# Hi-PACE/hipace

Measured on AMD Instinct MI355X. Metric: transverse slices/s at 1024^2 x 4ppc (explicit solver), higher is better.
Workload: dtype f64

## Files before the change

hipace_amd/_lib.py:

```python
import ctypes as C
import os
import subprocess


def hip_already_started():
    import sys
    if _LIB is not None:
        return True
    t = sys.modules.get("torch")
    try:
        return bool(t is not None and t.cuda.is_initialized())
    except Exception:
        return False


_LIB = None
_HWQ_PRESET = "GPU_MAX_HW_QUEUES" in os.environ
_HIP_STARTED_AT_IMPORT = hip_already_started()
_HERE = os.path.dirname(os.path.abspath(__file__))
CSRC = os.path.join(_HERE, "csrc")
SO = os.environ.get("HPS_LIB") or os.path.join(CSRC, "libhpslice.so")


class Slab(C.Structure):
# ... 54 lines not shown
                ("lo", C.c_double * 3), ("hi", C.c_double * 3),
                ("order", C.c_int), ("deriv_type", C.c_int),
                ("plasma_ppc", C.c_int * 2), ("plasma_density", C.c_double), ("plasma_radius", C.c_double),
                ("plasma_charge", C.c_double), ("plasma_mass", C.c_double), ("max_qsa", C.c_double),
                ("n_subcycles", C.c_int),
                ("beam_profile", C.c_int), ("beam_zmin", C.c_double), ("beam_zmax", C.c_double),
                ("beam_radius", C.c_double), ("beam_density", C.c_double),
                ("beam_umean", C.c_double * 3), ("beam_pos_mean", C.c_double * 3),
                ("beam_pos_std", C.c_double * 3), ("beam_ppc", C.c_int * 3), ("beam_charge", C.c_double),
                ("bc", C.c_int), ("mg_tol_rel", C.c_double), ("mg_tol_abs", C.c_double),
                ("deposit_rho", C.c_int), ("n_steps", C.c_int),
                ("dt", C.c_double), ("beam_n_subcycles", C.c_int), ("beam_mass", C.c_double), ("ext_E_slope", C.c_double * 2),
                ("bxby_solver", C.c_int), ("predcorr_tol", C.c_double), ("predcorr_max_iter", C.c_int),
                ("predcorr_mix", C.c_double), ("field_bc", C.c_int),
                ("laser_on", C.c_int), ("laser_a0", C.c_double), ("laser_w0", C.c_double), ("laser_L0", C.c_double),
                ("laser_lambda0", C.c_double), ("laser_pos", C.c_double * 3),
                ("laser_zfoc", C.c_double), ("laser_solver", C.c_int), ("laser_use_phase", C.c_int), ("si_units", C.c_int),
                ("grid_current_on", C.c_int), ("grid_current_peak", C.c_double), ("grid_current_mean", C.c_double * 3),
                ("grid_current_std", C.c_double * 3), ("laser_mg_tol_rel", C.c_double), ("laser_mg_tol_abs", C.c_double),
                ("beam_radiation_reaction", C.c_int), ("background_density_SI", C.c_double), ("beam_no_z_push", C.c_int),
                ("plasma_no_neutralize", C.c_int), ("ion_on", C.c_int), ("ion_ppc", C.c_int * 2), ("ion_density", C.c_double),
                ("ion_mass", C.c_double), ("ion_charge", C.c_double), ("ion_init_level", C.c_int), ("ion_Z", C.c_int),
                ("ion_energies", C.c_double * 56), ("ion_seed", C.c_ulonglong),
                ("beam_spin_tracking", C.c_int), ("beam_initial_spin", C.c_double * 3), ("beam_spin_anom", C.c_double),
                ("dt_adaptive", C.c_int), ("nt_per_betatron", C.c_double), ("dt_max", C.c_double),
                ("adaptive_threshold_uz", C.c_double), ("adaptive_phase_tolerance", C.c_double),
                ("adaptive_no_predict_step", C.c_int), ("adaptive_no_phase_control", C.c_int), ("adaptive_phase_substeps", C.c_int),
                ("adaptive_density", C.c_double), ("max_time", C.c_double), ("beam_uz_std", C.c_double),
                ("ext_Ez_slope", C.c_double),
                ("beam_do_salame", C.c_int), ("salame_n_iter", C.c_int), ("salame_relative_tolerance", C.c_double),
                ("salame_no_advance", C.c_int), ("salame_Ez_target_slope", C.c_double)]


COMPS = ["N_jx_beam", "N_jy_beam", "chi", "Sy", "Sx", "ExmBy", "EypBx", "Ez", "Bx", "By", "Bz",
         "Psi", "jx_beam", "jy_beam", "jz_beam", "jx", "jy", "rhomjz", "P_jx_beam", "P_jy_beam",
         "Ion_rhomjz", "rho"]
CIDX = {n: i for i, n in enumerate(COMPS)}
COMPS_PC = ["N_jx", "N_jy", "ExmBy", "EypBx", "Ez", "Bx", "By", "Bz", "Psi", "jx", "jy", "jz", "rhomjz",
            "P_Bx", "P_By", "P_jx", "P_jy", "Ion_rhomjz", "It_Bx", "It_By", "PIt_Bx", "PIt_By", "rho"]
CIDX_PC = {n: i for i, n in enumerate(COMPS_PC)}
COMPS_SALAME = ["Ez_target", "Ez_no_salame", "Ez", "jx", "jy", "jz_beam", "Bx", "By", "Sy", "Sx", "Sy_back", "Sx_back"]
ID_VALID = 1 << 63

_SIGS = {
    "hps_last_error": (C.c_char_p, []),
    "hps_version": (C.c_char_p, []),
    "hps_deposit_current": (C.c_int, [Slab, Plasma, Geom, C.c_void_p, C.c_double, C.c_double, C.c_int, C.c_double,
                                      C.c_int, C.c_void_p, C.c_void_p]),
    "hps_explicit_deposit": (C.c_int, [Slab, Plasma, Geom, C.c_void_p, C.c_void_p, C.c_double, C.c_double, C.c_int,
                                       C.c_int, C.c_int, C.c_void_p]),
    "hps_advance_plasma": (C.c_int, [Slab, Plasma, Geom, C.c_void_p, C.c_double, C.c_double, C.c_int, C.c_int,
                                     C.c_int, C.c_int, C.c_void_p]),
    "hps_tiling_create": (C.c_int, [C.c_int, C.c_int, C.c_int, C.c_long, C.POINTER(C.c_void_p)]),
    "hps_reorder_particles": (C.c_int, [C.c_void_p, Plasma, Plasma, Geom, C.c_void_p]),
    "hps_tiling_info": (C.c_int, [C.c_void_p, C.POINTER(C.c_int), C.POINTER(C.c_void_p), C.POINTER(C.c_void_p)]),
    "hps_tiling_destroy": (C.c_int, [C.c_void_p]),
    "hps_deposit_current_tiled": (C.c_int, [Slab, Plasma, Geom, C.c_void_p, C.c_double, C.c_double, C.c_int, C.c_double,
                                            C.c_int, C.c_void_p, C.c_void_p, C.c_void_p, C.c_void_p]),
    "hps_explicit_deposit_tiled": (C.c_int, [Slab, Plasma, Geom, C.c_void_p, C.c_void_p, C.c_double, C.c_double, C.c_int,
                                             C.c_int, C.c_int, C.c_void_p, C.c_void_p, C.c_void_p]),
    "hps_advance_plasma_tiled": (C.c_int, [Slab, Plasma, Geom, C.c_void_p, C.c_double, C.c_double, C.c_int, C.c_int,
                                           C.c_int, C.c_int, C.c_void_p, C.c_void_p, C.c_void_p]),
    "hps_deposit_current_tiled_laser": (C.c_int, [Slab, Plasma, Geom, C.c_void_p, C.c_int, C.c_double, C.c_double, C.c_int,
                                                  C.c_double, C.c_int, C.c_void_p, C.c_void_p, C.c_void_p, C.c_void_p]),
    "hps_explicit_deposit_tiled_laser": (C.c_int, [Slab, Plasma, Geom, C.c_void_p, C.c_int, C.c_void_p, C.c_double, C.c_double,
                                                   C.c_int, C.c_int, C.c_int, C.c_void_p, C.c_void_p, C.c_void_p]),
    "hps_advance_plasma_tiled_laser": (C.c_int, [Slab, Plasma, Geom, C.c_void_p, C.c_int, C.c_double, C.c_double, C.c_int,
                                                 C.c_int, C.c_int, C.c_int, C.c_void_p, C.c_void_p, C.c_void_p]),
    "hps_tiling_set_validity": (C.c_int, [C.c_void_p, C.c_int, C.c_int]),
    "hps_particles_record": (C.c_int, [C.c_int]),
    "hps_particles_recorded": (C.c_int, [C.c_char_p, C.c_long, C.POINTER(C.c_long)]),
    "hps_poisson_create": (C.c_int, [C.c_int, C.c_int, C.c_double, C.c_double, C.POINTER(C.c_void_p)]),
    "hps_poisson_solve": (C.c_int, [C.c_void_p, C.c_void_p, Slab, C.c_int, C.c_void_p]),
    "hps_poisson_solve_batch": (C.c_int, [C.c_void_p, C.c_int, C.c_void_p, Slab, C.c_void_p, C.c_void_p]),
    "hps_poisson_info": (C.c_int, [C.c_void_p, C.POINTER(C.c_int), C.POINTER(C.c_int), C.POINTER(C.c_int)]),
    "hps_poisson_destroy": (C.c_int, [C.c_void_p]),
    "hps_mg_create": (C.c_int, [C.c_int, C.c_int, C.c_double, C.c_double, C.POINTER(C.c_void_p)]),
    "hps_mg_solve1": (C.c_int, [C.c_void_p, Slab, C.c_int, C.c_int, C.c_int, C.c_double, C.c_double, C.c_int,
                                C.POINTER(C.c_int), C.POINTER(C.c_double), C.c_void_p]),
    "hps_mg_solve1_fabs": (C.c_int, [C.c_void_p, Slab, Slab, Slab, C.c_double, C.c_double, C.c_int,
                                     C.POINTER(C.c_int), C.POINTER(C.c_double), C.c_void_p]),
    "hps_mg_info": (C.c_int, [C.c_void_p, C.POINTER(C.c_int), C.POINTER(C.c_int), C.POINTER(C.c_int), C.POINTER(C.c_int),
                              C.POINTER(C.c_long), C.POINTER(C.c_int), C.POINTER(C.c_int), C.POINTER(C.c_int), C.POINTER(C.c_int)]),
    "hps_mg_destroy": (C.c_int, [C.c_void_p]),
    "hps_mg2_create": (C.c_int, [C.c_int, C.c_int, C.c_double, C.c_double, C.POINTER(C.c_void_p)]),
    "hps_mg2_solve2": (C.c_int, [C.c_void_p, C.c_void_p, C.c_void_p, C.c_void_p, C.c_void_p, C.c_double, C.c_double, C.c_int,
                                 C.POINTER(C.c_int), C.POINTER(C.c_double), C.c_void_p]),
    "hps_mg2_info": (C.c_int, [C.c_void_p, C.POINTER(C.c_int), C.POINTER(C.c_int), C.POINTER(C.c_int), C.POINTER(C.c_int)]),
    "hps_mg2_destroy": (C.c_int, [C.c_void_p]),
    "hps_engine_laser_vcycles": (C.c_int, [C.c_void_p, C.POINTER(C.c_long)]),
    "hps_engine_create": (C.c_int, [C.POINTER(Deck), C.c_int, C.POINTER(C.c_void_p)]),
    "hps_engine_destroy": (C.c_int, [C.c_void_p]),
    "hps_engine_begin_step": (C.c_int, [C.c_void_p]),
    "hps_engine_solve_slice": (C.c_int, [C.c_void_p, C.c_int]),
    "hps_engine_solve_slice_begin": (C.c_int, [C.c_void_p, C.c_int]),
    "hps_engine_solve_slice_finish": (C.c_int, [C.c_void_p, C.c_int]),
    "hps_engine_slice_ready": (C.c_int, [C.c_void_p]),
    "hps_engine_run_step": (C.c_int, [C.c_void_p]),
    "hps_engine_sync": (C.c_int, [C.c_void_p]),
    "hps_engine_info": (C.c_int, [C.c_void_p, C.POINTER(C.c_int), C.POINTER(C.c_int), C.POINTER(C.c_long)]),
    "hps_engine_slab": (Slab, [C.c_void_p]),
    "hps_engine_plasma": (Plasma, [C.c_void_p]),
    "hps_engine_stream": (C.c_void_p, [C.c_void_p]),
    "hps_engine_ions": (Plasma, [C.c_void_p]),
    "hps_engine_ion_stats": (C.c_int, [C.c_void_p, C.POINTER(C.c_long), C.POINTER(C.c_long)]),
    "hps_engine_checksums": (C.c_int, [C.c_void_p, C.c_void_p]),
    "hps_beam_sort_by_box": (C.c_int, [C.c_void_p, C.c_long, C.c_double, C.c_double, C.c_int, C.c_void_p, C.c_void_p,
                                       C.c_void_p, C.c_void_p]),
    "hps_engine_stats": (C.c_int, [C.c_void_p, C.POINTER(C.c_long), C.POINTER(C.c_long)]),
    "hps_engine_early_init_slices": (C.c_int, [C.c_void_p, C.POINTER(C.c_long)]),
    "hps_engine_set_insitu_plasma": (C.c_int, [C.c_void_p, C.c_double]),
    "hps_engine_set_insitu_beam": (C.c_int, [C.c_void_p, C.c_double]),
    "hps_engine_insitu_beam": (C.c_int, [C.c_void_p, C.c_void_p]),
    "hps_engine_insitu_plasma": (C.c_int, [C.c_void_p, C.c_void_p]),
    "hps_engine_set_insitu_fields": (C.c_int, [C.c_void_p, C.c_int]),
    "hps_engine_insitu_fields": (C.c_int, [C.c_void_p, C.c_void_p]),
    "hps_engine_set_field_diagnostic": (C.c_int, [C.c_void_p, C.c_int, C.c_void_p, C.c_void_p]),
    "hps_engine_field_diagnostic": (C.c_int, [C.c_void_p, C.c_void_p]),
    "hps_engine_set_field_diagnostic_box": (C.c_int, [C.c_void_p, C.c_int, C.c_void_p, C.c_void_p, C.c_int, C.c_void_p, C.c_void_p]),
    "hps_engine_field_diagnostic_geometry": (C.c_int, [C.c_void_p, C.c_void_p, C.c_void_p, C.c_void_p]),
    "hps_engine_record_event": (C.c_int, [C.c_void_p, C.c_int, C.POINTER(C.c_void_p)]),
    "hps_engine_wait_event": (C.c_int, [C.c_void_p, C.c_void_p]),
    "hps_stream_pool_shared_pairs": (C.c_int, [C.c_int]),
    "hps_engine_copy_async": (C.c_int, [C.c_void_p, C.c_void_p, C.c_void_p, C.c_long]),
    "hps_engine_set_profiling_stride": (C.c_int, [C.c_void_p, C.c_int]),
    "hps_engine_set_laser_import": (C.c_int, [C.c_void_p, C.c_int, C.c_int]),
    "hps_engine_set_step": (C.c_int, [C.c_void_p, C.c_int]),
    "hps_engine_set_time": (C.c_int, [C.c_void_p, C.c_double, C.c_double]),
    "hps_engine_beam_moments": (C.c_int, [C.c_void_p, C.c_void_p]),
    "hps_adaptive_create": (C.c_int, [C.c_void_p, C.POINTER(C.c_void_p)]),
    "hps_adaptive_set_density_profile": (C.c_int, [C.c_void_p, C.c_int, C.c_void_p, C.c_void_p, C.c_int, C.c_void_p, C.c_void_p]),
    "hps_adaptive_initial_dt": (C.c_int, [C.c_void_p, C.c_double, C.c_double, C.c_int, C.POINTER(C.c_double)]),
    "hps_adaptive_before_step": (C.c_int, [C.c_void_p, C.c_double, C.POINTER(C.c_double)]),
    "hps_adaptive_next_time": (C.c_int, [C.c_void_p, C.POINTER(C.c_double)]),
    "hps_adaptive_after_step": (C.c_int, [C.c_void_p, C.c_void_p, C.c_double, C.c_int, C.POINTER(C.c_double)]),
    "hps_adaptive_destroy": (C.c_int, [C.c_void_p]),
    "hps_engine_export_laser_slice": (C.c_int, [C.c_void_p, C.c_int, C.c_void_p]),
    "hps_engine_import_laser_slice": (C.c_int, [C.c_void_p, C.c_int, C.c_void_p]),
    "hps_engine_import_laser_from": (C.c_int, [C.c_void_p, C.c_int, C.c_void_p]),
    "hps_engine_laser_envelope": (C.c_int, [C.c_void_p, C.c_void_p]),
    "hps_engine_laser_info": (C.c_int, [C.c_void_p, C.POINTER(C.c_int), C.POINTER(C.c_double)]),
    "hps_engine_set_laser_grid": (C.c_int, [C.c_void_p, C.POINTER(C.c_int), C.POINTER(C.c_double), C.POINTER(C.c_double), C.c_int]),
    "hps_engine_laser_grid": (C.c_int, [C.c_void_p, C.POINTER(C.c_int), C.POINTER(C.c_int), C.POINTER(C.c_int), C.POINTER(C.c_int)]),
    "hps_engine_laser_chi": (C.c_int, [C.c_void_p, C.c_void_p]),
    "hps_engine_set_laser_pulses": (C.c_int, [C.c_void_p, C.c_int, C.POINTER(LaserPulse)]),
    "hps_engine_add_laser_samples": (C.c_int, [C.c_void_p, C.c_int, C.c_void_p, C.POINTER(C.c_long), C.POINTER(C.c_double),
                                               C.POINTER(C.c_double), C.c_double]),
    "hps_engine_set_insitu_laser": (C.c_int, [C.c_void_p, C.c_int]),
    "hps_engine_insitu_laser": (C.c_int, [C.c_void_p, C.c_void_p]),
    "hps_laser_interp_aabs": (C.c_int, [Slab, C.c_int, C.c_void_p, C.c_int, C.c_int, C.c_double, C.c_double, C.c_double, C.c_double,
                                        Geom, C.c_int, C.c_void_p]),
    "hps_laser_interp_chi": (C.c_int, [Slab, C.c_int, C.c_void_p, C.c_void_p, C.c_int, C.c_int, C.c_double, C.c_double, C.c_double,
                                       C.c_double, Geom, C.c_int, C.c_int, C.c_void_p]),
    "hps_deposit_current_laser": (C.c_int, [Slab, Plasma, Geom, C.c_void_p, C.c_int, C.c_double, C.c_double, C.c_int, C.c_double,
                                            C.c_int, C.c_void_p, C.c_void_p]),
    "hps_explicit_deposit_laser": (C.c_int, [Slab, Plasma, Geom, C.c_void_p, C.c_int, C.c_void_p, C.c_double, C.c_double, C.c_int,
                                             C.c_int, C.c_int, C.c_void_p]),
    "hps_advance_plasma_laser": (C.c_int, [Slab, Plasma, Geom, C.c_void_p, C.c_int, C.c_double, C.c_double, C.c_int, C.c_int,
                                           C.c_int, C.c_int, C.c_void_p]),
    "hps_engine_pc_stats": (C.c_int, [C.c_void_p, C.POINTER(C.c_long), C.POINTER(C.c_double)]),
    "hps_engine_pc_zero_b_slices": (C.c_int, [C.c_void_p, C.POINTER(C.c_long)]),
    "hps_engine_set_diagnostics": (C.c_int, [C.c_void_p, C.c_int]),
    "hps_engine_set_tiling": (C.c_int, [C.c_void_p, C.c_int, C.c_int]),
    "hps_engine_fallbacks": (C.c_int, [C.c_void_p, C.POINTER(C.c_long)]),
    "hps_engine_set_fusion": (C.c_int, [C.c_void_p, C.c_int]),
    "hps_engine_set_density_profile": (C.c_int, [C.c_void_p, C.c_int, C.c_void_p, C.c_void_p, C.c_int, C.c_void_p, C.c_void_p]),
    "hps_engine_set_plasma_init": (C.c_int, [C.c_void_p, C.POINTER(C.c_int), C.POINTER(C.c_int), C.c_double]),
    "hps_engine_set_fine_patch": (C.c_int, [C.c_void_p, C.c_void_p, C.c_int]),
    "hps_engine_set_plasma_momentum": (C.c_int, [C.c_void_p, C.c_int, C.POINTER(C.c_double), C.POINTER(C.c_double), C.c_ulonglong]),
    "hps_engine_set_plasma_symmetry": (C.c_int, [C.c_void_p, C.c_int, C.c_int]),
    "hps_engine_sorts": (C.c_int, [C.c_void_p, C.POINTER(C.c_long)]),
    "hps_engine_assume_initial_beam_support": (C.c_int, [C.c_void_p]),
    "hps_engine_beam_state": (C.c_int, [C.c_void_p, C.c_void_p, C.c_void_p]),
    "hps_engine_beam_capacity": (C.c_int, [C.c_void_p, C.POINTER(C.c_long)]),
    "hps_engine_set_beam_capacity": (C.c_int, [C.c_void_p, C.c_long]),
    "hps_engine_beam_message_rows": (C.c_int, [C.c_void_p, C.POINTER(C.c_int)]),
    "hps_engine_beam_spin": (C.c_int, [C.c_void_p, C.c_void_p]),
    "hps_engine_set_beam_import": (C.c_int, [C.c_void_p, C.c_int]),
    "hps_engine_export_beam_slice": (C.c_int, [C.c_void_p, C.c_int, C.c_void_p]),
    "hps_engine_import_beam_slice": (C.c_int, [C.c_void_p, C.c_int, C.c_void_p]),
    "hps_engine_set_profiling": (C.c_int, [C.c_void_p, C.c_int]),
    "hps_engine_phase_times": (C.c_int, [C.c_void_p, C.c_void_p, C.c_void_p]),
    "hps_engine_beam_info": (C.c_int, [C.c_void_p, C.POINTER(C.c_long), C.c_void_p]),
    "hps_engine_set_beam_particles": (C.c_int, [C.c_void_p, C.c_long, C.c_void_p, C.POINTER(C.c_long)]),
    "hps_engine_set_beam_storage": (C.c_int, [C.c_void_p, C.c_void_p]),
    "hps_engine_initial_beam": (C.c_int, [C.c_void_p, C.c_void_p]),
    "hps_ring_unique_id": (C.c_int, [C.c_char_p]),
    "hps_ring_init": (C.c_int, [C.c_int, C.c_int, C.c_int, C.c_char_p, C.c_char_p, C.POINTER(C.c_void_p)]),
    "hps_ring_send_slice": (C.c_int, [C.c_void_p, C.c_void_p, C.c_long, C.c_void_p, C.c_int, C.POINTER(C.c_void_p)]),
    "hps_ring_recv_slice": (C.c_int, [C.c_void_p, C.c_void_p, C.c_long, C.c_void_p, C.c_int, C.POINTER(C.c_void_p)]),
    "hps_ring_sendrecv_self": (C.c_int, [C.c_void_p, C.c_void_p, C.c_void_p, C.c_long, C.c_void_p, C.c_int, C.POINTER(C.c_void_p)]),
    "hps_ring_stream_wait": (C.c_int, [C.c_void_p, C.c_int, C.c_void_p]),
    "hps_ring_sync_sends": (C.c_int, [C.c_void_p]),
# ... 101 lines not shown
```

hipace_amd/api.py:

```python
import ctypes as C

import numpy as np
import torch

from . import _lib, decks as _decks, expr as _expr
from ._lib import CIDX, COMPS, ID_VALID, PL_REAL, check


def _stream():
    return C.c_void_p(torch.cuda.current_stream().cuda_stream)


def _iarr(vals):
    return (C.c_int * len(vals))(*[int(v) for v in vals])


class Geometry:

    def __init__(self, nx, ny, lo, hi, dz, bc=1, normalized=True, consts=(1., 1., 1., 1., 1.), ng=None):
        self.nx, self.ny = nx, ny
        g = _lib.Geom()
        g.dx = (hi[0] - lo[0]) / nx
        g.dy = (hi[1] - lo[1]) / ny
        g.dz = dz
# ... 248 lines not shown
        check(_lib.lib().hps_laser_interp_chi(fields.struct(), int(chi_comp), self._plane(chi_initial, torch.float64),
                                              C.c_void_p(out.data_ptr()), self.nxl, self.nyl, self.dxl, self.dyl, self.xoffl, self.yoffl,
                                              geom.c, fields.ng if shrink is None else int(shrink), self.order, _stream()))
        return out


def open_boundary(planes, lo, hi, no_monopole_mask=0):
    if not (isinstance(planes, torch.Tensor) and planes.is_cuda and planes.dtype == torch.float64 and planes.dim() == 3
            and planes.is_contiguous()):
        raise ValueError("open_boundary: planes must be a contiguous CUDA float64 tensor (nbatch, ny, nx)")
    nbatch, ny, nx = planes.shape
    check(_lib.lib().hps_open_boundary(C.c_void_p(planes.data_ptr()), nbatch, nx, ny, (C.c_double * 2)(lo[0], lo[1]),
                                       (C.c_double * 2)(hi[0], hi[1]), int(no_monopole_mask), _stream()))
    return planes


class FFTPoissonSolver:

    def __init__(self, nx, ny, dx, dy, device="cuda"):
        self.nx, self.ny = nx, ny
        self._h = C.c_void_p()
        check(_lib.lib().hps_poisson_create(nx, ny, dx, dy, C.byref(self._h)))
        self.staging = torch.zeros((ny, nx), dtype=torch.float64, device=device)

    def StagingArea(self):
        return self.staging

    BACKENDS = ("own-sym", "own-pow2", "dense", "rocfft")

    def info(self):
        b, n, m = C.c_int(), C.c_int(), C.c_int()
        check(_lib.lib().hps_poisson_info(self._h, C.byref(b), C.byref(n), C.byref(m)))
        return self.BACKENDS[b.value], n.value, m.value

    def SolvePoissonEquation(self, lhs_fields, comp):
        check(_lib.lib().hps_poisson_solve(self._h, C.c_void_p(self.staging.data_ptr()), lhs_fields.struct(), comp,
                                           _stream()))

    def __del__(self):
        if getattr(self, "_h", None) and _lib is not None:
            _lib.lib().hps_poisson_destroy(self._h)
            self._h = None


class MultiGrid2:

    def __init__(self, nx, ny, dx, dy):
        self._h = C.c_void_p()
        check(_lib.lib().hps_mg2_create(nx, ny, dx, dy, C.byref(self._h)))

    def solve2(self, sol2, rhs2, acoef_real, acoef_imag, tol_rel=1e-4, tol_abs=0.0, nummaxiter=200):
        it = C.c_int()
        rn = C.c_double()
        for t in (sol2, rhs2, acoef_real, acoef_imag):
            assert t.is_cuda and t.is_contiguous() and t.dtype == torch.float64
        check(_lib.lib().hps_mg2_solve2(self._h, sol2.data_ptr(), rhs2.data_ptr(), acoef_real.data_ptr(), acoef_imag.data_ptr(),
                                        tol_rel, tol_abs, nummaxiter, C.byref(it), C.byref(rn), _stream()))
        return it.value, rn.value

    BOTTOMS = ("lower-v", "single-block", "per-sweep")
    TILES = ("single-block", "32x16", "64x32")

    def info(self):
        nl, top, b, t = C.c_int(), C.c_int(), C.c_int(), (C.c_int * 31)()
        check(_lib.lib().hps_mg2_info(self._h, C.byref(nl), C.byref(top), C.byref(b), t))
        return {"nlev": nl.value, "low_top": top.value, "bottom": self.BOTTOMS[b.value],
                "tiles": tuple(self.TILES[v] for v in t if v >= 0)}

    def __del__(self):
        if getattr(self, "_h", None) and _lib is not None:
            _lib.lib().hps_mg2_destroy(self._h)
            self._h = None


class MultiGrid:

    def __init__(self, nx, ny, dx, dy):
        self._h = C.c_void_p()
        check(_lib.lib().hps_mg_create(nx, ny, dx, dy, C.byref(self._h)))

    LOWV = ("v3", "v-cc", "v-nodal", "bottom")
    TILES = ("TileSmall", "TileBig", "TileSmall-pull", "TileMid-pull")

    def info(self):
        cc, nl, lb, kind, npyr, nres, pull1 = (C.c_int() for _ in range(7))
        lds, t = C.c_long(), (C.c_int * 31)()
        check(_lib.lib().hps_mg_info(self._h, C.byref(cc), C.byref(nl), C.byref(lb), C.byref(kind), C.byref(lds), t,
                                     C.byref(pull1), C.byref(npyr), C.byref(nres)))
        return {"cc": bool(cc.value), "nlev": nl.value, "lowv_begin": lb.value, "lowv": self.LOWV[kind.value],
                "lowv_lds": lds.value, "tiles": tuple(self.TILES[v] for v in t if v >= 0), "nodal_pull1": bool(pull1.value),
                "pyramid": npyr.value, "restricts": nres.value}

    def solve1(self, fields, sol_comp, rhs_comp, acoef_comp, tol_rel=1e-4, tol_abs=2.2250738585072014e-308,
               nummaxiter=200):
        it = C.c_int()
        rn = C.c_double()
        check(_lib.lib().hps_mg_solve1(self._h, fields.struct(), sol_comp, rhs_comp, acoef_comp, tol_rel, tol_abs,
                                       nummaxiter, C.byref(it), C.byref(rn), _stream()))
        return it.value, rn.value

    def solve1_fabs(self, sol, rhs, acoef, tol_rel=1e-4, tol_abs=2.2250738585072014e-308, nummaxiter=200):
        it = C.c_int()
        rn = C.c_double()
        check(_lib.lib().hps_mg_solve1_fabs(self._h, sol.struct(), rhs.struct(), acoef.struct(), tol_rel, tol_abs, nummaxiter,
                                            C.byref(it), C.byref(rn), _stream()))
        return it.value, rn.value

    def __del__(self):
        if getattr(self, "_h", None) and _lib is not None:
            _lib.lib().hps_mg_destroy(self._h)
            self._h = None


class Expression:

    def __init__(self, text, variables=("x", "y", "z", "t"), constants=None):
        self.program = text if isinstance(text, _expr.Program) else _expr.compile_expr(text, variables, constants)
        self._c, self._keep = self.program.c_struct()
        depth = C.c_int()
        check(_lib.lib().hps_expr_check(C.byref(self._c), len(self.program.variables), C.byref(depth)))
        self.depth = depth.value

    def __call__(self, *tensors, out=None):
        nv = len(self.program.variables)
        if len(tensors) != nv:
            raise ValueError(f"Expression: {nv} tensors expected ({', '.join(self.program.variables)}), got {len(tensors)}")
        if out is None and not tensors:
            raise ValueError("Expression: a program without variables needs out=")
        for t in tensors:
            assert t.is_cuda and t.dtype == torch.float64 and t.is_contiguous() and t.shape == tensors[0].shape
        if out is None:
            out = torch.empty_like(tensors[0])
        assert out.is_cuda and out.dtype == torch.float64 and out.is_contiguous() and (not tensors or out.shape == tensors[0].shape)
        ptrs = (C.c_void_p * max(nv, 1))(*[t.data_ptr() if t.numel() else None for t in tensors])
        check(_lib.lib().hps_expr_eval(C.byref(self._c), nv, out.numel(), ptrs, C.c_void_p(out.data_ptr() if out.numel() else None),
                                       _stream()))
        return out

    def evaluate_host(self, *arrays):
        nv = len(self.program.variables)
        if len(arrays) != nv:
            raise ValueError(f"Expression: {nv} arrays expected ({', '.join(self.program.variables)}), got {len(arrays)}")
        a = [np.ascontiguousarray(v, dtype=np.float64) for v in np.broadcast_arrays(*arrays)] if arrays else []
        out = np.empty(a[0].shape if a else (1,), dtype=np.float64)
        ptrs = (C.c_void_p * max(nv, 1))(*[v.ctypes.data for v in a])
        check(_lib.lib().hps_expr_eval_host(C.byref(self._c), nv, out.size, ptrs, out.ctypes.data_as(C.c_void_p)))
        return out


class AdaptiveTimeStep:

    def __init__(self, deck, density_profile=None, density_exprs=None, beams=None):
        self.deck = dict(deck)
        if beams is None:
            more = [s["record"] for s in _decks.beam_species(deck)]
            beams = ([dict(charge=deck.get("beam_charge", -1.0), mass=deck.get("beam_mass", 1.0))] + more) if more else None
        self.beams = None if beams is None or len(beams) < 2 else [dict(b) for b in beams]
        self._dk = _lib.fill_struct(_lib.Deck(), deck)
        self._h = C.c_void_p()
        check(_lib.lib().hps_adaptive_create(C.byref(self._dk), C.byref(self._h)))
        if density_profile is not None:
            self.set_density_profile(*density_profile)
        if density_exprs is None:
            density_exprs = {sp: spec[:2] for sp, spec in _decks.density_exprs(deck).items()}
        for sp, spec in density_exprs.items():
            self.set_density_expr(sp, *spec)

    @classmethod
    def for_engine(cls, engine):
        exprs = {sp: ((progs[0] if pos is None else list(zip(pos, progs))), None)
                 for sp, (progs, pos, _) in getattr(engine, "density_exprs", {}).items()}
        names, _ = engine.beam_species()
        beams = [r for r in engine.beam_species_records] if len(names) > 1 else None
        return cls(engine.deck, getattr(engine, "density_profile", None), exprs, beams)
# ... 703 lines not shown
        assert dst.numel() == src.numel()
        check(_lib.lib().hps_engine_copy_async(self._h, C.c_void_p(dst.data_ptr()), C.c_void_p(src.data_ptr()),
                                               dst.numel() * 8))

    def phase_times(self):
        ms = (C.c_double * 8)()
        n = C.c_long()
        check(_lib.lib().hps_engine_phase_times(self._h, ms, C.byref(n)))
        names = ["deposit_current", "poisson", "explicit_deposit", "mg_solve1", "advance_plasma", "other", "sort", "empty_interval"]
        return {k: ms[i] for i, k in enumerate(names)}, n.value

    def checksums(self):
        out = (C.c_double * self.ncomp)()
        check(_lib.lib().hps_engine_checksums(self._h, out))
        names = self.comp_names()
        cs = {names[i]: out[i] for i in range(self.ncomp)}
        if "aabs" in cs:
            tot = C.c_double()
            check(_lib.lib().hps_engine_laser_info(self._h, None, C.byref(tot)))
            cs["laserEnvelope"] = tot.value
        return cs

    @property
    def has_laser(self):
        return bool(self.deck.get("laser_on", 0))

    def laser_message_doubles(self):
        nxl, nyl, _, _ = self.laser_grid()
        return 4 * nxl * nyl

    def set_step(self, step):
        check(_lib.lib().hps_engine_set_step(self._h, int(step)))

    def set_laser_import(self, on, step=0):
        check(_lib.lib().hps_engine_set_laser_import(self._h, int(on), int(step)))

    def export_laser_slice(self, islice, msg):
        check(_lib.lib().hps_engine_export_laser_slice(self._h, islice, C.c_void_p(msg.data_ptr())))

    def import_laser_slice(self, islice, msg):
        check(_lib.lib().hps_engine_import_laser_slice(self._h, islice, C.c_void_p(msg.data_ptr())))

    def import_laser_from(self, islice, src):
        check(_lib.lib().hps_engine_import_laser_from(self._h, islice, src._h))

    def laser_envelope(self):
        nxl, nyl, zlo, zhi = self.laser_grid()
        out = np.empty((zhi - zlo + 1, nyl, nxl), dtype=np.complex128)
        check(_lib.lib().hps_engine_laser_envelope(self._h, out.ctypes.data_as(C.c_void_p)))
        return out

    def comp_names(self):
        if self.deck.get("bxby_solver", 0):
            return list(_lib.COMPS_PC[:22]) + (["rho"] if self.deck.get("deposit_rho", 0) else [])
        return list(COMPS[:21]) + (["rho"] if self.deck.get("deposit_rho", 0) else []) + \
            (["aabs"] if self.deck.get("laser_on", 0) else []) + \
            (["Salame_" + n for n in _lib.COMPS_SALAME] if self.deck.get("beam_do_salame", 0) else [])

    def salame_stats(self):
        nz = self.deck["nz"]
        out = np.zeros((nz, 4), dtype=np.float64)
        check(_lib.lib().hps_engine_salame_stats(self._h, out.ctypes.data_as(C.c_void_p)))
        flags = out[:, 3].astype(np.int64)
        return {"W": out[:, 0].copy(), "W_total": out[:, 1].copy(), "iterations": out[:, 2].astype(np.int64),
                "converged": (flags & 1) != 0, "overloaded": (flags & 2) != 0, "ran": out[:, 2] > 0}

    def pc_stats(self):
        its, err = C.c_long(), C.c_double()
        check(_lib.lib().hps_engine_pc_stats(self._h, C.byref(its), C.byref(err)))
        return its.value, err.value

    def pc_zero_b_slices(self):
        n = C.c_long()
        check(_lib.lib().hps_engine_pc_zero_b_slices(self._h, C.byref(n)))
        return n.value

    def stats(self):
        vc, sl = C.c_long(), C.c_long()
        check(_lib.lib().hps_engine_stats(self._h, C.byref(vc), C.byref(sl)))
        ei = C.c_long()
        check(_lib.lib().hps_engine_early_init_slices(self._h, C.byref(ei)))
        return dict(vcycles=vc.value, slices=sl.value, early_init=ei.value)

    def slab(self):
        self.sync()
        s = _lib.lib().hps_engine_slab(self._h)
        nx, ny, g = s.nx, s.ny, s.ng
        out = np.empty((s.ncomp, ny + 2 * g, nx + 2 * g), dtype=np.float64)
        check(_lib.lib().hps_memcpy_d2h(out.ctypes.data_as(C.c_void_p), C.c_void_p(s.p), out.nbytes))
        return out

    def ions(self):
        self.sync()
        p = _lib.lib().hps_engine_ions(self._h)
        n = p.n
        real = np.empty((11, n), dtype=np.float64)
        idc = np.empty(n, dtype=np.uint64)
        lev = np.empty(n, dtype=np.int32)
        if n:
            for k, name in enumerate(PL_REAL):
                check(_lib.lib().hps_memcpy_d2h(real[k].ctypes.data_as(C.c_void_p), C.c_void_p(getattr(p, name)), real[k].nbytes))
            check(_lib.lib().hps_memcpy_d2h(idc.ctypes.data_as(C.c_void_p), C.c_void_p(p.idcpu), idc.nbytes))
            check(_lib.lib().hps_memcpy_d2h(lev.ctypes.data_as(C.c_void_p), C.c_void_p(p.ion_lev), lev.nbytes))
        key = ((idc >> np.uint64(24)) & np.uint64((1 << 39) - 1)).astype(np.int64) - 1
        return real, ((idc >> np.uint64(63)) & np.uint64(1)).astype(np.int32), lev, key

    def ion_stats(self):
        a, b = C.c_long(), C.c_long()
        check(_lib.lib().hps_engine_ion_stats(self._h, C.byref(a), C.byref(b)))
        return a.value, b.value

    def particles(self):
        self.sync()
        p = _lib.lib().hps_engine_plasma(self._h)
        n = p.n
        real = np.empty((11, n), dtype=np.float64)
        idc = np.empty(n, dtype=np.uint64)
        if n:
            for k, name in enumerate(PL_REAL):
                check(_lib.lib().hps_memcpy_d2h(real[k].ctypes.data_as(C.c_void_p), C.c_void_p(getattr(p, name)), real[k].nbytes))
            check(_lib.lib().hps_memcpy_d2h(idc.ctypes.data_as(C.c_void_p), C.c_void_p(p.idcpu), idc.nbytes))
        return real, ((idc >> np.uint64(63)) & np.uint64(1)).astype(np.int32)
```

hipace_amd/csrc/engine.h:

```cpp
#ifndef HPS_ENGINE_H_
#define HPS_ENGINE_H_

#include "common.h"
#include "expr.h"
#include <algorithm>
#include <array>
#include <string>
#include <vector>
#include "tiling.h"
#include "mg_gate.h"
#include "particle_math.h"
#include "poisson_src.h"
#include "beam_deposit.h"
#include "slab_ops.h"

void mg_rider (void* mg_handle, int** dev_words, const int** host_words);
namespace hps {

constexpr int PC_MAX_SPEC = 64;

int mg_solve1_begin (void* mg_handle, hps_slab s, int sol_comp, int rhs_comp, int acf_comp, double tol_rel, double tol_abs,
                     int max_iters, hipStream_t st);
void mg_solve1_forget_hierarchy (void* mg_handle);
bool poisson_gateable (void* poisson_handle);
// ... 46 lines not shown
    ~CollScratch ();
};

struct BeamStash { double* blocks = nullptr; unsigned char* tag = nullptr; std::vector<long> off; long n = 0; bool host_beam = false;
                   double charge = 0.0, mass = 0.0; };

struct Engine {
    hps_deck d{};
    hps_geom gm{};
    int g = 0, ncomp = 0;
    hipStream_t st = nullptr;
    bool st_pooled = false; int st_device = 0;
    hps_slab slab{};
    struct Ions { double* d_adk = nullptr; unsigned long long* d_cnt = nullptr; long long* h_cnt = nullptr; long long* h_cnt_dev = nullptr;
                  long long seq = 0; long n_ionized = 0; bool pending = false; int* d_tile_flag = nullptr;
                  double* d_fbound = nullptr;
                } ion;
    std::vector<double> prof_r, prof_t, prof_f_t; double* d_prof_r = nullptr; double prof_ft = 1.0;
    double hollow_core_radius = 0.0;
    bool fine_patch_set = false; int fine_T = 0; long fine_ncells = 0; int* d_fine_level = nullptr; int* d_fine_cells = nullptr;
    struct Thermal { double u_mean[3] = {0.0, 0.0, 0.0}, u_std[3] = {0.0, 0.0, 0.0}; unsigned long long seed = 0;
                     bool warm () const { for (int q = 0; q < 3; ++q) if (u_mean[q] != 0.0 || u_std[q] != 0.0) return true; return false; }
                   };
    bool do_symmetrize = false, prevent_centered = false;
    bool shifted (const int ppc[2], int dir) const { return prevent_centered && (dir == 0 ? d.nx : d.ny) % 2 == 1 && ppc[dir] % 2 == 1; }
    int set_plasma_momentum (int species, const double* u_mean, const double* u_std, unsigned long long seed);
    int set_plasma_symmetry (int symmetrize, int prevent_centered_particle);
    int alloc_sheets ();
    int set_plasma_init (const int* plasma_fine, const int* ion_fine, double hollow_core);
    int set_fine_patch (const unsigned char* mask_host, int transition_cells);
    bool fuse_push_deposit = false; int ahead_for = -2;
    long fallback_div = 256;
    bool gate_push = true;
    int step_index = -1;
    int next_step = -1;
    bool time_set = false; double next_t = 0.0, next_dt = 0.0, step_dt = 0.0;
    double step_time = 0.0;
    struct BeamExt { bool on = false; ExprImage image; int depth = 0; } bext;
    int set_beam_external_fields (const hps_expr* E3, const hps_expr* B3);
    struct DensityExpr { bool on = false; std::vector<std::vector<hps_expr_ins>> ins; std::vector<std::vector<double>> consts;
                         std::vector<double> z_pos; std::vector<int> off; int depth = 0; double min_density = 0.0; int cur = 0; };
    ExprImage dens_image; double dens_z = 0.0;
    int set_density_expr (int species, int n_progs, const hps_expr* progs, const double* z_pos, double min_density);
    void density_begin_step (double ct);
    DensityProgram density_program (int species) const;
    size_t density_lds (int species) const { const DensityExpr& D = sp[species].dens; return D.on ? expr_lds_bytes(D.depth, 256) : 0; }
    struct Species {
        int index = 0;
        hps_plasma pl{}, pl_alt{}; double *real = nullptr, *real_alt = nullptr; Tiling* tiling = nullptr;
        long cap = 0, n_init = 0;
        int ppc[2] = {0, 0}, fine_ppc[2] = {0, 0}; double density = 0.0, charge = 0.0, mass = 0.0;
        int init_level = 0, can_ionize = 0, keyed = 0;
        bool temp_push = false;
        Thermal thermal; DensityExpr dens;
        bool present () const { return density > 0.0; }
        bool alias_prev () const { return !temp_push; }
    } sp[2];
    Species &el = sp[0], &ions = sp[1];
    bool warm_init (const Species& s) const { return s.thermal.warm() || do_symmetrize || shifted(s.ppc, 0) || shifted(s.ppc, 1); }
    long sheet_slots (const Species& s) const;
    int init_sheet (Species& s);
    int sort_sheet (Species& s);
    bool host_beam = false;
    double* d_mom = nullptr;
    struct BeamSpecies { hps_beam_species s{}; long count = 0; bool filled = false; };
    std::vector<BeamSpecies> bsp; int sel_species = 0;
    unsigned char *bm_sp = nullptr, *bm_sp_scr = nullptr, *beam_tag = nullptr; BeamSpeciesRec* d_bsp_tab = nullptr;
    unsigned long beam_launched = 0;
    int n_beam_species () const { return std::max<int>(1, (int)bsp.size()); }
    bool multi_beam () const { return bsp.size() > 1; }
    int add_beam_species (const hps_beam_species* s, int* index_out);
    int alloc_beam_tags ();
    template <class F> int fill_selected_species (const char* fn, F&& set);
    int stash_beam_for_merge (const char* fn, BeamStash& A);
    int merge_stashed_beam (BeamStash& A, int e_setter);
    IonArgs ion_args (int islice);
    int ionize_slice (int islice);
    int ionize_collect ();
    int ion_field_bounds ();
    bool fold_tail = true;
    TailWork fold_tail_of (const Species& s, long margin, long* covered) const;
    int species_deposit (const Species& s, const int comp[6], const BeamPairWork* beam = nullptr, const int* go = nullptr);
    bool valid_by_w = true;
    bool post_in_push = true;
    bool fold_hierarchy = true;
    bool fold_beam = true;
    int species_explicit (const Species& s, const int cache[4], const int depos[2]);
    int species_advance (const Species& s, const int comp[5], int temp_slice, const int* go = nullptr);
    int tile_size = 16, sort_period = 128, since_sort = 0;
    int* d_nfallback = nullptr;
    const int* h_nfallback = nullptr;
    long fb_at_sort = 0; int n_sorts = 0;
    int setup_tiling ();
    int resort ();
    void* ps = nullptr;
    void* mg = nullptr;
    double* staging = nullptr;
    double* d_open_mom = nullptr;
    int open_boundary (int nbatch, unsigned no_monopole_mask);
    double* beam_data = nullptr; double* beam_init = nullptr; double* beam_cur = nullptr;
    long nbeam = 0; std::vector<long> beam_off;
    bool moving = false; int steps_begun = 0; int beam_rows = 7;
    BeamSoA bm{}, bm_scr{}; double* bm_store = nullptr; int* bm_nsub = nullptr; int* bm_nsub_scr = nullptr;
    long* d_B = nullptr; int* d_nfront = nullptr; std::vector<long> h_B;
    bool beam_import = false; long* d_Bimp = nullptr; long beam_cap = 0; int* d_beam_overflow = nullptr;
    long beam_bound (int p) const {
        if (p < 0 || p >= d.nz) return 0;
        if (beam_import) return std::max(nbeam, 1L);
        return h_B[p + 1] - h_B[0];
    }
    struct Box { int ilo, ihi, jlo, jhi; };
    Box beam_box{0, -1, 0, -1}, beam_box_init{0, -1, 0, -1}, full_box{0, -1, 0, -1};
    int* d_nqsa = nullptr;
    double* d_checksum = nullptr;
    bool diagnostics = false;
    bool profiling = false; bool prof_light = false; int prof_stride = 1; bool prof_now = false;
    std::vector<hipEvent_t> ev; size_t ev_used = 0;
    std::vector<hipEvent_t> hand_ev;
    void mark ();
    long total_vcycles = 0, slices_done = 0;
    int* d_pc_dist = nullptr;
    double pc_floor = 0.0;
    int* d_pc_go = nullptr; bool pc_speculate = false; int pc_spec_iters = 1, pc_enqueued = 0, pc_islice = -1; double pc_base_seq = 0.0, pc_last_err = 0.0;
    int solve_slice_pc_begin (int islice); int solve_slice_pc_finish (int islice); int pc_enqueue_iteration (int it); int pc_wait_slot (int slot, double seq);
    bool pc = false; double* d_pc = nullptr; double* d_pc_aux = nullptr; double* h_pc = nullptr; double* h_pc_dev = nullptr; double pc_seq = 0.0; long pc_iterations = 0; double pc_err_sum = 0.0; long pc_zero_b_slices = 0;
    double pc_tol = 4e-2, pc_mix = 0.05; int pc_max_iter = 30;
    int c_aabs = -1; double* d_laser_sum = nullptr;
    LaserState* laser = nullptr;
    struct LaserGrid { bool set = false; int nx = 0, ny = 0, zlo = 0, zhi = -1, order = 1;
                       double lo[3] = {0, 0, 0}, hi[3] = {0, 0, 0}, dx = 0.0, dy = 0.0, xoff = 0.0, yoff = 0.0; } lgrid;
    int set_laser_grid (const int* n_cell, const double* patch_lo, const double* patch_hi, int interp_order);
    struct LaserSamples { int geometry = 0; long extent[3] = {0, 0, 0}; double offset[3] = {0, 0, 0}, spacing[3] = {0, 0, 0}, unit = 1.0;
                          std::vector<double> data; };
    bool laser_pulses_set = false; std::vector<hps_laser_pulse> laser_pulses; std::vector<LaserSamples> laser_samples;
    bool insitu_laser = false;
    bool laser_has_slice (int islice) const { return !lgrid.set || (islice >= lgrid.zlo && islice <= lgrid.zhi); }
    hipStream_t st_laser = nullptr; hipEvent_t ev_lfork = nullptr, ev_ldone = nullptr;
    bool laser_async = true, laser_pending = false;
    hipStream_t st_aux = nullptr; hipEvent_t ev_aux[3] = {nullptr, nullptr, nullptr}; bool aux_on = false, aux_pending = false;
    hipStream_t laser_stream () const { return (laser_async && st_laser) ? st_laser : st; }
    int fork_laser ();
    int laser_done ();
    int join_laser ();
    std::vector<int> fd_comps; int fd_c[3] = {1, 1, 1}; double* d_fd = nullptr; int* d_fd_comps = nullptr;
    int fd_n[3] = {0, 0, 0}; double fd_h[3] = {0, 0, 0}, fd_pos0[3] = {0, 0, 0}, fd_lo[3] = {0, 0, 0}, fd_hi[3] = {0, 0, 0}; int fd_slice_dir = -1;
    size_t fd_cells () const { return (size_t)fd_n[0]*fd_n[1]*fd_n[2]; }
    int fill_field_diagnostic (int islice);
    double* d_insitu_bm = nullptr; double insitu_bm_radius = 0.0;
    void insitu_beam (int islice);
    double* d_insitu_pl = nullptr; double insitu_pl_radius = 0.0;
    double* d_insitu = nullptr;

    ~Engine ();
    int create (const hps_deck& deck, int device);
    int init_beam ();
    int install_beam (std::vector<double> (&h)[7]);
    int set_beam_particles (long n, const double* soa_host, long* n_outside);
    int set_beam_fixed_ppc (const hps_expr* density, double min_density, const double* u_std, const int* random_ppc, unsigned long long seed);
    int set_beam_fixed_weight (const hps_beam_fixed_weight* spec, const hps_expr* mean_x, const hps_expr* mean_y, unsigned long long seed,
                               long* n_left_out);
    int set_beam_fixed_weight_pdf (const hps_beam_fixed_weight_pdf* spec, const hps_expr* pdf, const hps_expr* progs, unsigned long long seed,
                                   long* n_left_out, double* uz_moments);
    int install_beam_device (double* blocks_dev, long n, const double box[4]);
    int begin_device_beam (long* n_left_out = nullptr);
    int finish_device_beam (DevBuf<double>& blocks, long n, long* n_left_out = nullptr);
    int drop_device_beam (int e, long* n_left_out);
// ... 88 lines not shown
```

hipace_amd/csrc/engine.hip:

```cpp
#include "common.h"
#include "engine.h"

#include <cmath>
#include <cstdlib>
#include <cstring>
#include <limits>
#include <atomic>
#include <algorithm>
#include <map>
#include <mutex>
#include <new>

namespace {
std::mutex g_pool_mutex;
std::map<int, std::vector<hipStream_t>> g_stream_pool;
std::map<int, bool> g_pool_made;
}

namespace hps {

int deposit_current_tiled (const hps_slab& slab, const hps_plasma& pl, const hps_geom& g, const int comp[6], double charge,
                           double mass, int order, double max_qsa, int can_ionize, int* n_qsa, Tiling* T, int* n_fallback,
                           hipStream_t st, int aabs_comp = -1, const int* tile_flag = nullptr, TailWork tw = TailWork{},
                           const BeamPairWork* beam = nullptr, const int* go = nullptr, bool valid_by_w = false);
// ... 552 lines not shown
    size_t pos = 0;
    while (pos < e.size()) {
        size_t end = e.find('+', pos); if (end == std::string::npos) end = e.size();
        int lo = 0, hi = -1;
        if (std::sscanf(e.substr(pos, end - pos).c_str(), "%d-%d", &lo, &hi) == 2)
            for (int b = std::max(lo, 0); b <= std::min(hi, 255); ++b) mask[b >> 5] |= 1u << (b & 31);
        pos = end + 1;
    }
    return hipExtStreamCreateWithCUMask(s, 8, mask);
}

long Engine::sheet_slots (const Species& s) const
{
    if (!s.present()) return 0;
    const long cells = (long)d.nx*d.ny, nc = (long)s.ppc[0]*s.ppc[1];
    const long copies = do_symmetrize ? 4 : 1;
    if (!(fine_patch_set && s.fine_ppc[0] > 0)) return copies*nc*cells;
    return copies*(nc*cells + ((long)s.fine_ppc[0]*s.fine_ppc[1] - nc)*fine_ncells);
}

std::array<double**, 11> soa_arrays (hps_plasma& p)
{
    return {&p.x, &p.y, &p.w, &p.ux, &p.uy, &p.psi, &p.x_prev, &p.y_prev, &p.ux_half, &p.uy_half, &p.psi_half};
}
int alloc_soa (hps_plasma& p, double*& real, long cap, bool alias)
{
    HPS_HIP_CHECK(hipMalloc(&real, (size_t)cap*11*sizeof(double)));
    const auto arr = soa_arrays(p);
    for (int k = 0; k < 11; ++k) *arr[k] = real + (size_t)k*cap;
    if (alias) { p.x_prev = p.x; p.y_prev = p.y; }
    HPS_HIP_CHECK(hipMalloc(&p.idcpu, (size_t)cap*sizeof(uint64_t)));
    HPS_HIP_CHECK(hipMalloc(&p.ion_lev, (size_t)cap*sizeof(int32_t)));
    return HPS_OK;
}
void free_soa (hps_plasma& p, double*& real)
{
    (void)hipFree(real); (void)hipFree(p.idcpu); (void)hipFree(p.ion_lev);
    real = nullptr; p = hps_plasma{};
}
static hps_plasma tail_of (const hps_plasma& p, long first, long n)
{
    hps_plasma t = p;
    for (double** a : soa_arrays(t)) *a += first;
    t.idcpu += first; t.ion_lev += first; t.n = n;
    return t;
}

int Engine::alloc_sheets ()
{
    for (Species& s : sp) { free_soa(s.pl, s.real); s.n_init = s.cap = sheet_slots(s); }
    if (ions.present()) el.cap = el.n_init + ions.n_init*(long)(d.ion_Z - d.ion_init_level);
    for (Species& s : sp) {
        s.pl.n = s.n_init;
        if (s.cap > 0) { if (int e = alloc_soa(s.pl, s.real, s.cap, s.alias_prev())) return e; }
    }
    return HPS_OK;
}

int Engine::create (const hps_deck& deck, int device)
{
    d = deck;
    HPS_REQUIRE(d.nx >= 4 && d.ny >= 4 && d.nz >= 1, "hps_engine_create: bad grid");
    HPS_REQUIRE(d.order >= 0 && d.order <= 3, "hps_engine_create: depos_order must be 0..3");
    HPS_REQUIRE(d.n_subcycles >= 0, "hps_engine_create: plasma n_subcycles must be >= 1 (0 = default 1)");
    if (d.n_subcycles == 0) d.n_subcycles = 1;
    if (d.field_bc != 0 && d.field_bc != 1) { set_error("hps_engine_create: boundary.field must be 0 (Dirichlet) or 1 (Open)"); return HPS_ERR_UNSUPPORTED; }
    if (d.field_bc == 1) {
        const double radius = std::min(std::min(std::fabs(d.lo[0]), std::fabs(d.hi[0])), std::min(std::fabs(d.lo[1]), std::fabs(d.hi[1])));
        HPS_REQUIRE(radius > 0.0 && d.lo[0] < 0.0 && d.hi[0] > 0.0 && d.lo[1] < 0.0 && d.hi[1] > 0.0, "hps_engine_create: boundary.field = Open needs x = y = 0 inside the box");
        HPS_HIP_CHECK(hipMalloc(&d_open_mom, (size_t)4*256*2*19*sizeof(double)));
    }
    pc = (d.bxby_solver != 0);
    if (const char* v = std::getenv("HPS_GATED_PUSH")) gate_push = std::atoi(v) != 0;
    if (const char* v = std::getenv("HPS_AUX_STREAM")) aux_on = std::atoi(v) != 0;
    if (aux_on) {
        HPS_HIP_CHECK(hipStreamCreateWithFlags(&st_aux, hipStreamNonBlocking));
        for (hipEvent_t& ev : ev_aux) HPS_HIP_CHECK(hipEventCreateWithFlags(&ev, event_flags(false)));
    }
    if (const char* v = std::getenv("HPS_FOLD_TAIL")) fold_tail = std::atoi(v) != 0;
    if (const char* v = std::getenv("HPS_POST_IN_PUSH")) post_in_push = std::atoi(v) != 0;
    if (const char* v = std::getenv("HPS_FOLD_BEAM")) fold_beam = std::atoi(v) != 0;
    if (const char* v = std::getenv("HPS_FOLD_HIERARCHY")) fold_hierarchy = std::atoi(v) != 0;
    if (const char* v = std::getenv("HPS_VALID_BY_W")) valid_by_w = std::atoi(v) != 0;
    if (const char* v = std::getenv("HPS_GATED_ION_PUSH")) gate_ion_push = std::atoi(v) != 0;
    if (const char* v = std::getenv("HPS_LAZY_SHIFT")) lazy_shift = std::atoi(v) != 0;
    if (const char* v = std::getenv("HPS_FUSE_SOURCES")) fuse_sources = std::atoi(v) != 0;
    if (const char* v = std::getenv("HPS_EARLY_INIT")) early_init = std::atoi(v) != 0;
    if (const char* v = std::getenv("HPS_SORT_FALLBACK_DIV")) { const long q = std::atol(v); if (q >= 1) fallback_div = q; }
    HPS_REQUIRE(!(d.beam_spin_tracking && d.dt == 0.0 && !d.dt_adaptive), "hps_engine_create: spin tracking needs a moving beam (hipace.dt != 0)");
    HPS_REQUIRE(!(d.dt_adaptive && d.laser_on), "hps_engine_create: hipace.dt = adaptive cannot be used with a laser (Hipace.cpp:408)");
    if (d.beam_do_salame) {
        if (pc) { set_error("hps_engine_create: beam_do_salame needs the explicit solver (Hipace.cpp:152), not the predictor-corrector"); return HPS_ERR_UNSUPPORTED; }
        if (d.beam_profile == 0 && !(std::isfinite(d.beam_zmin) && std::isfinite(d.beam_zmax))) {
            set_error("hps_engine_create: beam_do_salame with a gaussian beam profile needs finite beam_zmin and beam_zmax (BeamParticleContainer.cpp:149)"); return HPS_ERR_ARG; }
        if (d.ion_on) { set_error("hps_engine_create: beam_do_salame with the ionisable species (ion_on) is not supported"); return HPS_ERR_UNSUPPORTED; }
        if (d.laser_on) { set_error("hps_engine_create: beam_do_salame with a laser is not supported"); return HPS_ERR_UNSUPPORTED; }
        if (d.dt != 0.0 || d.dt_adaptive) { set_error("hps_engine_create: beam_do_salame needs a static beam (hipace.dt = 0)"); return HPS_ERR_UNSUPPORTED; }
        HPS_REQUIRE(d.salame_n_iter >= 0 && d.salame_relative_tolerance >= 0.0, "hps_engine_create: salame_n_iter and salame_relative_tolerance must not be negative");
        if (d.salame_n_iter == 0) d.salame_n_iter = 5;
        if (d.salame_relative_tolerance == 0.0) d.salame_relative_tolerance = 1.0e-4;
    }
    step_dt = d.dt;
    if (d.predcorr_tol > 0.0) pc_tol = d.predcorr_tol;
    if (d.predcorr_max_iter > 0) pc_max_iter = d.predcorr_max_iter;
    if (d.predcorr_mix > 0.0) pc_mix = d.predcorr_mix;
    HPS_HIP_CHECK(hipSetDevice(device));
    HPS_HIP_CHECK(create_engine_stream(&st, device, &st_pooled));
    st_device = device;
    if (const char* v = std::getenv("HPS_LASER_ASYNC")) laser_async = std::atoi(v) != 0;
    if (laser_async && d.laser_on && d.laser_solver >= 1 && d.dt != 0.0) {
        int lo = 0, hi = 0;
        (void)hipDeviceGetStreamPriorityRange(&lo, &hi);
        HPS_HIP_CHECK(hipStreamCreateWithPriority(&st_laser, hipStreamNonBlocking, lo));
        HPS_HIP_CHECK(hipEventCreateWithFlags(&ev_lfork, event_flags(false)));
        HPS_HIP_CHECK(hipEventCreateWithFlags(&ev_ldone, event_flags(false)));
    }
    g = (d.order + 1)/2 + 1;
    ncomp = pc ? (d.deposit_rho ? HPS_PC_RHO + 1 : HPS_PC_RHO) : (d.deposit_rho ? HPS_C_RHO + 1 : HPS_C_RHO);
    if (d.beam_radiation_reaction && !d.si_units && !(d.background_density_SI > 0.0)) {
        set_error("hps_engine_create: radiation reaction in normalised units needs background_density_SI"); return HPS_ERR_ARG; }
    if (d.laser_on) {
        if (pc) { set_error("hps_engine_create: the laser needs the explicit solver"); return HPS_ERR_UNSUPPORTED; }
        HPS_REQUIRE(d.laser_w0 > 0.0 && d.laser_L0 > 0.0 && d.laser_lambda0 > 0.0, "hps_engine_create: laser w0, L0, lambda0 must be positive");
        if (d.laser_solver < 0 || d.laser_solver > 2) { set_error("hps_engine_create: lasers.solver_type must be 0 (static), 1 (fft) or 2 (multigrid)"); return HPS_ERR_UNSUPPORTED; }
        c_aabs = ncomp++;
    }
    gm.dx = (d.hi[0] - d.lo[0])/d.nx; gm.dy = (d.hi[1] - d.lo[1])/d.ny; gm.dz = (d.hi[2] - d.lo[2])/d.nz;
    gm.xoff = 0.5*(d.lo[0] + d.hi[0] - gm.dx*(d.nx - 1));
    gm.yoff = 0.5*(d.lo[1] + d.hi[1] - gm.dy*(d.ny - 1));
    gm.c = gm.ep0 = gm.mu0 = gm.q_e = gm.m_e = 1.0;
    if (d.si_units) {
        gm.c = 299792458.0; gm.ep0 = 8.8541878128e-12; gm.mu0 = 1.25663706212e-06; gm.q_e = 1.602176634e-19; gm.m_e = 9.1093837015e-31;
    }
    gm.plo[0] = d.lo[0]; gm.plo[1] = d.lo[1]; gm.phi[0] = d.hi[0]; gm.phi[1] = d.hi[1];
    gm.bc = d.bc; gm.normalized = d.si_units ? 0 : 1;

    if (d.beam_do_salame) {
        c_sal = ncomp;
        HPS_HIP_CHECK(hipMalloc(&d_sal, (size_t)4*257*sizeof(double)));
        sal_stats.assign((size_t)4*d.nz, 0.0);
    }
    slab.nx = d.nx; slab.ny = d.ny; slab.ng = g; slab.ncomp = ncomp + (c_sal >= 0 ? (int)HPS_SAL_NCOMP : 0);
    set_canon = set_alt = InitSet{HPS_C_CHI, HPS_C_RHOMJZ, d.deposit_rho ? (int)HPS_C_RHO : -1, HPS_C_JZB, HPS_C_N_JXB, HPS_C_N_JYB};
    if (early_init && !pc && !d.laser_on && !d.ion_on && d.dt == 0.0 && !d.dt_adaptive && d.nx % 2 == 0 && d.ny % 2 == 0) {
        int c = slab.ncomp;
        set_alt.chi = c++; set_alt.rhomjz = c++; if (d.deposit_rho) set_alt.rho = c++;
        set_alt.jzb = c++; set_alt.njxb = c++; set_alt.njyb = c++;
        n_alt = c - slab.ncomp; slab.ncomp = c;
    }
    slab.jstride = d.nx + 2*g; slab.nstride = slab.jstride*(d.ny + 2*g);
    HPS_HIP_CHECK(hipMalloc(&slab.p, (size_t)slab.nstride*slab.ncomp*sizeof(double)));
    HPS_HIP_CHECK(hipMemset(slab.p, 0, (size_t)slab.nstride*slab.ncomp*sizeof(double)));
    HPS_HIP_CHECK(hipMalloc(&staging, (size_t)3*d.nx*d.ny*sizeof(double)));

    if (d.ion_on) {
        HPS_REQUIRE(d.ion_ppc[0] >= 1 && d.ion_ppc[1] >= 1 && d.ion_density > 0.0 && d.ion_mass > 0.0 && d.ion_charge != 0.0,
                    "hps_engine_create: the ion species needs ppc, density, mass and charge");
        if (int e = ion_create(*this)) return e;
    }
    for (int k = 0; k < 2; ++k) { sp[k].index = k; sp[k].can_ionize = k; sp[k].keyed = k; sp[k].temp_push = pc || (k == 0 && c_sal >= 0); }
    std::copy(d.plasma_ppc, d.plasma_ppc + 2, el.ppc); el.density = d.plasma_density; el.charge = d.plasma_charge; el.mass = d.plasma_mass;
    if (d.ion_on) { std::copy(d.ion_ppc, d.ion_ppc + 2, ions.ppc); ions.density = d.ion_density; ions.charge = d.ion_charge; ions.mass = d.ion_mass; ions.init_level = d.ion_init_level; }
    if (int e = alloc_sheets()) return e;
    HPS_HIP_CHECK(hipMalloc(&d_laser_sum, sizeof(double)));
    HPS_HIP_CHECK(hipMemset(d_laser_sum, 0, sizeof(double)));
    HPS_HIP_CHECK(hipMalloc(&d_nqsa, sizeof(int)));
    HPS_HIP_CHECK(hipMemset(d_nqsa, 0, sizeof(int)));
    HPS_HIP_CHECK(hipMalloc(&d_checksum, HPS_PC_NCOMP_MAX*sizeof(double)));
    HPS_HIP_CHECK(hipMemset(d_checksum, 0, HPS_PC_NCOMP_MAX*sizeof(double)));
    if (int e = hps_poisson_create(d.nx, d.ny, gm.dx, gm.dy, &ps)) return e;
    if (int e = hps_mg_create(d.nx, d.ny, gm.dx, gm.dy, &mg)) return e;
    {   int* dw = nullptr; const int* hw = nullptr;
        mg_rider(mg, &dw, &hw);
        d_nfallback = dw; h_nfallback = hw; }
    if (pc) {
        HPS_HIP_CHECK(hipMalloc(&d_pc, 4*sizeof(double)));
        HPS_HIP_CHECK(hipMemset(d_pc, 0, 4*sizeof(double)));
        HPS_HIP_CHECK(hipMalloc(&d_pc_aux, 4*sizeof(double)));
        HPS_HIP_CHECK(hipMemset(d_pc_aux, 0, 4*sizeof(double)));
        HPS_HIP_CHECK(hipHostMalloc(&h_pc, 8*PC_MAX_SPEC*sizeof(double), hipHostMallocMapped));
        std::memset(h_pc, 0, 8*PC_MAX_SPEC*sizeof(double));
        HPS_HIP_CHECK(hipHostGetDevicePointer((void**)&h_pc_dev, h_pc, 0));
        HPS_HIP_CHECK(hipMalloc(&d_pc_go, (PC_MAX_SPEC + 1)*sizeof(int)));
        HPS_HIP_CHECK(hipMemset(d_pc_go, 0, (PC_MAX_SPEC + 1)*sizeof(int)));
        {   const char* v = std::getenv("HPS_PC_EXACT_ZERO");
            if (!(v && std::atoi(v) == 0)) d_pc_dist = d_pc_go + PC_MAX_SPEC; }
        {   double rel = 0.0;
            if (const char* v = std::getenv("HPS_PC_NOISE_FLOOR")) rel = std::atof(v);
            pc_floor = rel*gm.mu0*gm.c*std::fabs(d.plasma_charge*d.plasma_density)*(double)d.nx*d.ny*(d.nx*gm.dx); }
        {   const char* v = std::getenv("HPS_PC_SPECULATE");
            pc_speculate = !(v && std::atoi(v) == 0) && pc_max_iter <= PC_MAX_SPEC - 2 && poisson_gateable(ps)
                           && d.field_bc == 0; }
        d_nfallback = reinterpret_cast<int*>(d_pc + 2); h_nfallback = reinterpret_cast<const int*>(h_pc + 4);
    }
    if (c_aabs >= 0) { if (int e = laser_create(*this)) return e; }
    return init_beam();
}

int Engine::setup_tiling ()
{
    if (tile_size == 0 || el.cap == 0 || el.tiling) return HPS_OK;
    if (int e = tiling_create(d.nx, d.ny, tile_size, el.cap, &el.tiling)) return e;
    {   const char* v = std::getenv("HPS_VALID_BY_PSI");
        el.tiling->valid_by_psi = (v && std::atoi(v) != 0); }
    if (int e = alloc_soa(el.pl_alt, el.real_alt, el.cap, el.alias_prev())) return e;
    if (ions.present()) {
        int ion_ts = tile_size;
        if (const char* v = std::getenv("HPS_ION_TILE")) { const int t = std::atoi(v); if (t == 16 || t == 32) ion_ts = t; }
        if (int e = tiling_create(d.nx, d.ny, ion_ts, ions.cap, &ions.tiling)) return e;
        if (int e = alloc_soa(ions.pl_alt, ions.real_alt, ions.cap, ions.alias_prev())) return e;
        HPS_HIP_CHECK(hipMalloc(&ion.d_tile_flag, (size_t)ions.tiling->g.ntiles*sizeof(int)));
        {   const char* v = std::getenv("HPS_ION_TILE_SKIP");
            if (!(v && std::atoi(v) == 0)) HPS_HIP_CHECK(hipMalloc(&ion.d_fbound, (size_t)5*ions.tiling->g.ntiles*sizeof(double))); }
    }
    return HPS_OK;
}

int Engine::sort_sheet (Species& s)
{
    s.pl_alt.n = s.pl.n;
    if (int e = tiling_sort(s.tiling, s.pl, s.pl_alt, gm, st)) return e;
    std::swap(s.pl, s.pl_alt);
    std::swap(s.real, s.real_alt);
    return HPS_OK;
}

int Engine::resort ()
{
    if (int e = sort_sheet(el)) return e;
    since_sort = 0; ++n_sorts;
    fb_at_sort = h_nfallback ? *h_nfallback : 0;
    return HPS_OK;
}

int Engine::init_sheet (Species& s)
{
    const long n = s.pl.n;
    if (n == 0) return HPS_OK;
    const double radius_sq = d.plasma_radius > 0.0 ? d.plasma_radius*d.plasma_radius : std::numeric_limits<double>::infinity();
    if (warm_init(s)) return init_plasma_warm(*this, s, radius_sq);
    if (hollow_core_radius > 0.0 || (fine_patch_set && s.fine_ppc[0] > 0) || s.dens.on)
        return init_plasma_fine(*this, s, radius_sq);
    const int nppc = s.ppc[0]*s.ppc[1];
    hipLaunchKernelGGL(k_init_plasma, dim3(ceil_div(n, 256)), dim3(256), 0, st, s.pl, n, d.nx, d.ny, s.ppc[0], s.ppc[1], d.lo[0], d.lo[1],
                       gm.dx, gm.dy, s.density*(d.si_units ? gm.dx*gm.dy*gm.dz/nppc : 1.0/nppc),
                       s.init_level, s.keyed, d_prof_r, (int)prof_r.size(), prof_ft, radius_sq);
    return HPS_OK;
}

int Engine::begin_step ()
{
    HPS_REQUIRE(!(d.dt_adaptive && steps_begun == 0 && d.beam_profile < 0 && !host_beam),
                "hps_engine_begin_step: hipace.dt = adaptive needs a beam (beam_profile = -1 and no hps_engine_set_beam_particles: the sum of weights is 0)");
    HPS_REQUIRE(fine_patch_set == (el.fine_ppc[0] > 0 || ions.fine_ppc[0] > 0),
                "hps_engine_begin_step: both fine_ppc (hps_engine_set_plasma_init) and the fine patch (hps_engine_set_fine_patch) must be given to use the fine plasma patch");
    HPS_REQUIRE(!(laser && laser_pulses_set && laser_pulses.empty() && laser_samples.empty() && !step_begun),
                "hps_engine_begin_step: hps_engine_set_laser_pulses with n = 0 needs at least one hps_engine_add_laser_samples");
    if (laser && !step_begun) { for (const LaserSamples& S : laser_samples) { if (int e = laser_check_samples(*this, S)) return e; } }
    if (int e = setup_tiling()) return e;
    el.keyed = coll.empty() ? 0 : 1;
    step_begun = true;
    if (moving && steps_begun > 0) {
        int ov = 0;
        HPS_HIP_CHECK(hipMemcpyAsync(&ov, d_beam_overflow, sizeof(int), hipMemcpyDeviceToHost, st));
        HPS_HIP_CHECK(hipStreamSynchronize(st));
        HPS_REQUIRE(ov == 0, "moving beam: a slice outgrew the hand-off capacity (twice the fullest injected slice) in the previous step");
    }
    if (moving && beam_import) {
        HPS_HIP_CHECK(hipMemsetAsync(d_B, 0, (size_t)(d.nz + 1)*sizeof(long), st));
        HPS_HIP_CHECK(hipMemsetAsync(d_Bimp, 0, (size_t)(d.nz + 1)*sizeof(long), st));
        HPS_HIP_CHECK(hipMemsetAsync(d_nfront, 0, (size_t)(d.nz + 2)*sizeof(int), st));
        ++steps_begun;
    } else if (moving) {
        if (steps_begun > 0) {
            hipLaunchKernelGGL(k_beam_new_step, dim3(ceil_div(std::max(nbeam, 1L), 256)), dim3(256), 0, st, bm_nsub, nbeam);
            HPS_HIP_CHECK(hipMemsetAsync(d_nfront, 0, (size_t)(d.nz + 2)*sizeof(int), st));
        }
        HPS_HIP_CHECK(hipMemcpyAsync(h_B.data(), d_B, (size_t)(d.nz + 1)*sizeof(long), hipMemcpyDeviceToHost, st));
        HPS_HIP_CHECK(hipStreamSynchronize(st));
        ++steps_begun;
    }
    shift_pending = false;
    alt_live = false; init_done = false; pend_rode = false;
    HPS_HIP_CHECK(hipMemsetAsync(slab.p, 0, (size_t)slab.nstride*slab.ncomp*sizeof(double), st));
    if (d_pc_dist) HPS_HIP_CHECK(hipMemsetAsync(d_pc_dist, (d.grid_current_on || d.ion_on || d.plasma_no_neutralize || el.thermal.warm() || ions.thermal.warm()) ? 1 : 0, sizeof(int), st));
    HPS_HIP_CHECK(hipMemsetAsync(d_checksum, 0, HPS_PC_NCOMP_MAX*sizeof(double), st));
    HPS_HIP_CHECK(hipMemsetAsync(d_laser_sum, 0, sizeof(double), st));
// ... 1134 lines not shown
    return HPS_OK;
}

int Engine::run_step ()
{
    if (int e = begin_step()) return e;
    for (int isl = d.nz - 1; isl >= 0; --isl)
        if (int e = solve_slice(isl)) return e;
    return HPS_OK;
}

}

using namespace hps;

extern "C" const char* hps_last_error (void) { return g_err.c_str(); }
extern "C" const char* hps_version (void) { return "hpslice 0.1 (gfx950)"; }

extern "C" int hps_engine_create (const hps_deck* deck, int device, void** handle)
{
    HPS_REQUIRE(deck && handle, "hps_engine_create: null argument");
    Engine* E = new Engine;
    if (int e = E->create(*deck, device)) { delete E; return e; }
    *handle = E;
    return HPS_OK;
}
extern "C" int hps_engine_destroy (void* h) { delete static_cast<Engine*>(h); return HPS_OK; }
extern "C" int hps_engine_begin_step (void* h) { return static_cast<Engine*>(h)->begin_step(); }
extern "C" int hps_engine_solve_slice (void* h, int islice) { return static_cast<Engine*>(h)->solve_slice(islice); }
extern "C" int hps_engine_solve_slice_begin (void* h, int islice) { return static_cast<Engine*>(h)->solve_slice_begin(islice); }
extern "C" int hps_engine_slice_ready (void* h)
{
    Engine* E = static_cast<Engine*>(h);
    if (E->pc) {
        if (!(E->pc_speculate && E->el.tiling && !E->moving && !E->ions.present()) || E->pc_islice < 0 || E->pc_enqueued <= 0) return 1;
        for (int it = 1; it <= E->pc_enqueued; ++it) {
            const volatile double* hp = E->h_pc + 8*it;
            const double seq = E->pc_base_seq + it;
            if (!(hp[1] == seq && hp[3] == seq && hp[5] == seq)) return 0;
            const double err = hp[0] > 0.0 ? hp[2]/hp[0] : 0.0;
            if (!(err > E->pc_tol) || it >= E->pc_max_iter) return 1;
        }
        return 1;
    }
    if (E->pending_slice < 0) return 1;
    return mg_solve1_ready(E->mg) ? 1 : 0;
}
extern "C" int hps_engine_solve_slice_finish (void* h, int islice) { return static_cast<Engine*>(h)->solve_slice_finish(islice); }
extern "C" int hps_engine_run_step (void* h) { return static_cast<Engine*>(h)->run_step(); }
extern "C" int hps_engine_sync (void* h)
{
    Engine* E = static_cast<Engine*>(h);
    E->flush_shift();
    if (int e = E->join_laser()) return e;
    HPS_HIP_CHECK(hipStreamSynchronize(E->st));
    if (E->moving && E->d_beam_overflow) {
        int ov = 0;
        HPS_HIP_CHECK(hipMemcpy(&ov, E->d_beam_overflow, sizeof(int), hipMemcpyDeviceToHost));
        HPS_REQUIRE(ov == 0, "moving beam: a slice outgrew the hand-off capacity (twice the fullest injected slice): particles were lost");
    }
    return HPS_OK;
}
extern "C" int hps_engine_info (void* h, int* ncomp, int* ng, long* np)
{
    Engine* E = static_cast<Engine*>(h);
    if (ncomp) *ncomp = E->ncomp;
    if (ng) *ng = E->g;
    if (np) *np = E->el.pl.n;
    return HPS_OK;
}
extern "C" hps_slab hps_engine_slab (void* h)
{
    Engine* E = static_cast<Engine*>(h);
    E->flush_shift();
    hps_slab s = E->slab; s.ncomp -= E->n_alt;
    return s;
}
extern "C" int hps_engine_early_init_slices (void* h, long* n)
{
    HPS_REQUIRE(h && n, "hps_engine_early_init_slices: null argument");
    *n = static_cast<Engine*>(h)->slices_rode;
    return HPS_OK;
}
extern "C" hps_plasma hps_engine_plasma (void* h) { return static_cast<Engine*>(h)->el.pl; }
extern "C" int hps_engine_tiling (void* h, void** tiling)
{
    HPS_REQUIRE(h && tiling, "hps_engine_tiling: null argument");
    *tiling = static_cast<Engine*>(h)->el.tiling;
    return HPS_OK;
}
extern "C" hps_plasma hps_engine_ions (void* h)
{
    Engine* E = static_cast<Engine*>(h);
    (void)hipStreamSynchronize(E->st);
    return E->ions.pl;
}
extern "C" int hps_engine_ion_stats (void* h, long* n_ionized, long* n_product)
{
    Engine* E = static_cast<Engine*>(h);
    HPS_HIP_CHECK(hipStreamSynchronize(E->st));
    if (int e = E->ionize_collect()) return e;
    if (n_ionized) *n_ionized = E->ion.n_ionized;
    if (n_product) *n_product = E->el.pl.n;
    return HPS_OK;
}
extern "C" hps_stream hps_engine_stream (void* h) { return static_cast<Engine*>(h)->st; }
extern "C" int hps_engine_checksums (void* h, double* out)
{
    Engine* E = static_cast<Engine*>(h);
    HPS_HIP_CHECK(hipStreamSynchronize(E->st));
    HPS_HIP_CHECK(hipMemcpy(out, E->d_checksum, E->ncomp*sizeof(double), hipMemcpyDeviceToHost));
    return HPS_OK;
}
extern "C" int hps_engine_stats (void* h, long* vc, long* sl)
{
    Engine* E = static_cast<Engine*>(h);
    if (vc) *vc = E->total_vcycles;
    if (sl) *sl = E->slices_done;
    return HPS_OK;
}
extern "C" int hps_engine_set_insitu_plasma (void* h, double radius)
{
    Engine* E = static_cast<Engine*>(h);
    HPS_HIP_CHECK(hipStreamSynchronize(E->st));
    (void)hipFree(E->d_insitu_pl); E->d_insitu_pl = nullptr; E->insitu_pl_radius = radius;
    if (!(radius > 0.0)) return HPS_OK;
    HPS_HIP_CHECK(hipMalloc(&E->d_insitu_pl, (size_t)15*E->d.nz*sizeof(double)));
    HPS_HIP_CHECK(hipMemset(E->d_insitu_pl, 0, (size_t)15*E->d.nz*sizeof(double)));
    return HPS_OK;
}
extern "C" int hps_engine_set_insitu_beam (void* h, double radius)
{
    Engine* E = static_cast<Engine*>(h);
    HPS_HIP_CHECK(hipStreamSynchronize(E->st));
    (void)hipFree(E->d_insitu_bm); E->d_insitu_bm = nullptr; E->insitu_bm_radius = radius;
    if (!(radius > 0.0)) return HPS_OK;
    HPS_HIP_CHECK(hipMalloc(&E->d_insitu_bm, (size_t)23*E->d.nz*HPS_MAX_BEAM_SPECIES*sizeof(double)));
    HPS_HIP_CHECK(hipMemset(E->d_insitu_bm, 0, (size_t)23*E->d.nz*HPS_MAX_BEAM_SPECIES*sizeof(double)));
    return HPS_OK;
}
extern "C" int hps_engine_insitu_beam (void* h, double* out)
{
    Engine* E = static_cast<Engine*>(h);
    HPS_REQUIRE(E && !E->multi_beam(), "hps_engine_insitu_beam: the engine holds several beam species: hps_engine_insitu_beam_species returns one of them");
    return hps_engine_insitu_beam_species(h, 0, out);
}
extern "C" int hps_engine_insitu_beam_species (void* h, int species, double* out)
{
    Engine* E = static_cast<Engine*>(h);
    HPS_REQUIRE(E && E->d_insitu_bm && out, "hps_engine_insitu_beam: not switched on");
    HPS_REQUIRE(species >= 0 && species < E->n_beam_species(), "hps_engine_insitu_beam_species: no such beam species");
    HPS_HIP_CHECK(hipStreamSynchronize(E->st));
    const int nz = E->d.nz;
    HPS_HIP_CHECK(hipMemcpy(out, E->d_insitu_bm + (size_t)species*23*nz, (size_t)23*nz*sizeof(double), hipMemcpyDeviceToHost));
    for (int k = 0; k < nz; ++k) {
        const double sw = out[k], inv = sw <= 0.0 ? 0.0 : 1.0/sw;
        for (int q = 1; q <= 21; ++q) out[(size_t)q*nz + k] *= inv;
    }
    return HPS_OK;
}
extern "C" int hps_engine_insitu_plasma (void* h, double* out)
{
    Engine* E = static_cast<Engine*>(h);
    HPS_REQUIRE(E->d_insitu_pl && out, "hps_engine_insitu_plasma: not switched on");
    HPS_HIP_CHECK(hipStreamSynchronize(E->st));
    const int nz = E->d.nz;
// ... 653 lines not shown
```

hipace_amd/csrc/multigrid.hip:

```cpp
#include "common.h"
#include <type_traits>
#include "mg_gate.h"
#include "slab_ops.h"

#include <vector>
#include <algorithm>
#include <cmath>
#include <cstring>

namespace hps {

struct FView {
    double* p; long js, ns; int oi, oj;
    __device__ __forceinline__ double& operator() (int i, int j, int n) const {
        const unsigned o = (unsigned)((i + oi) + (j + oj)*(int)js + n*(int)ns)*8u;
        return *reinterpret_cast<double*>(reinterpret_cast<char*>(p) + o);
    }
};

struct LevBox { int lox, loy, hix, hiy;
                int vlx, vly, vhx, vhy; };

enum { SRC_ZERO = 0, SRC_DIRECT = 1, SRC_PROLONG = 2 };

#define HPS_KEEP(x) asm volatile("" :: "v"(x))

#ifdef HPS_STAMPS
__device__ long long* g_mg_dbg = nullptr;
#define MG_STAMP(i) do { if (g_mg_dbg && blockIdx.x == 0 && threadIdx.x == 0) g_mg_dbg[i] = __builtin_amdgcn_s_memtime(); } while (0)
#else
#define MG_STAMP(i) do { } while (0)
#endif

template <int TX_, int TY_, int NT_>
struct TileShape {
    static constexpr int TX = TX_, TY = TY_, NT = NT_;
    static constexpr int AX = TX + 2, AY = TY + 2;
    static constexpr int PR = TX/2;
    static constexpr int GPAIRS = TX*TY/2/NT;
    static_assert(TX*TY/2 % NT == 0 && NT % 64 == 0 && (PR == 16 || PR == 32), "tile shape");
};
using TileBig = TileShape<64, 32, 512>;
using TileMid = TileShape<32, 32, 256>;
using TileHuge = TileShape<64, 48, 512>;
using TileHugeNodal = TileShape<64, 32, 512>;
template <bool CC> struct HugeTileOf { using type = TileHuge; };
template <> struct HugeTileOf<false> { using type = TileHugeNodal; };
using TileSmall = TileShape<32, 16, 256>;

template <bool CC>
__device__ __forceinline__ double diag_c0 (int i, int j, const LevBox& b, double acf, double facx, double facy)
{
    double c0 = -(acf + 2.0*(facx + facy));
    if (CC && (i == b.lox || i == b.hix)) c0 -= 2.0*facx;
    if (CC && (j == b.loy || j == b.hiy)) c0 -= 2.0*facy;
    return c0;
}

template <bool CC, bool INTERIOR = false, class P>
__device__ __forceinline__ double offdiag (P c, int sy, int i, int j, const LevBox& b, double facx, double facy)
{
    const double w = c[-1], e = c[1], s = c[-sy], n = c[sy];
    double lx = facx*(w + e), ly = facy*(s + n);
    if (CC && !INTERIOR) {
        const double fx43 = facx*(4./3.), fy43 = facy*(4./3.);
        lx = (i == b.lox) ? fx43*e : ((i == b.hix) ? fx43*w : lx);
        ly = (j == b.loy) ? fy43*n : ((j == b.hiy) ? fy43*s : ly);
    }
    return lx + ly;
}

template <class P>
__device__ __forceinline__ double offdiag_m (P c, int sy, double fxm, double fym)
{
    return fxm*(c[-1] + c[1]) + fym*(c[-sy] + c[sy]);
}
template <bool CC>
__device__ __forceinline__ double wall_mult (int i, int lo, int hi, double fac)
{
    return (CC && (i == lo || i == hi)) ? fac*(4./3.) : fac;
}

template <bool INTERIOR = false>
__device__ __forceinline__ double residual_v (double p0, double w, double e, double s, double n, int i, int j, const LevBox& b,
                                              double rhs, double acf, double facx, double facy);

template <bool INTERIOR = false, class P>
__device__ __forceinline__ double residual_at (P c, int sy, int i, int j, const LevBox& b,
                                               double rhs, double acf, double facx, double facy)
{
    return residual_v<INTERIOR>(c[0], c[-1], c[1], c[-sy], c[sy], i, j, b, rhs, acf, facx, facy);
}

template <bool INTERIOR>
__device__ __forceinline__ double residual_v (double p0, double w, double e, double s, double n, int i, int j, const LevBox& b,
                                              double rhs, double acf, double facx, double facy)
{
    double lap = -2.0*(facx + facy)*p0;
    double tx = facx*(w + e), ty = facy*(s + n);
    if (!INTERIOR) {
        tx = (i == b.lox) ? facx*((4./3.)*e - 2.0*p0) : ((i == b.hix) ? facx*((4./3.)*w - 2.0*p0) : tx);
        ty = (j == b.loy) ? facy*((4./3.)*n - 2.0*p0) : ((j == b.hiy) ? facy*((4./3.)*s - 2.0*p0) : ty);
    }
    lap += tx;
    lap += ty;
    return rhs + acf*p0 - lap;
}

template <bool CC>
__device__ __forceinline__ double prolong_at (const FView& crse, int i, int j, int n)
{
    const int ic = i >> 1, jc = j >> 1;
    if (CC) return crse(ic, jc, n);
    const bool io = (i & 1), jo = (j & 1);
    if (io && jo)  return (crse(ic, jc, n) + crse(ic+1, jc, n) + crse(ic, jc+1, n) + crse(ic+1, jc+1, n))*0.25;
    if (io)        return (crse(ic, jc, n) + crse(ic+1, jc, n))*0.5;
    if (jo)        return (crse(ic, jc, n) + crse(ic, jc+1, n))*0.5;
    return crse(ic, jc, n);
}

constexpr int MG_MAX_VCYCLES = 1024;
template <int NT>
__device__ __forceinline__ void block_max_to (unsigned long long* slot, double v, double* s_red)
{
    for (int o = 32; o > 0; o >>= 1) v = fmax(v, __shfl_xor(v, o));
    if ((threadIdx.x & 63) == 0) s_red[threadIdx.x >> 6] = v;
    __syncthreads();
    if (threadIdx.x == 0) {
        double m = 0.0;
        for (int w = 0; w < NT/64; ++w) m = fmax(m, s_red[w]);
        if (m > 0.0) atomicMax(slot + (blockIdx.x & (MG_NSUB - 1)), (unsigned long long)__double_as_longlong(m));
// ... 210 lines not shown
                }
                if (fin[p]) {
                    if constexpr (RPULL) { rhs(i, j, 0) = r0[m][p]; rhs(i, j, 1) = r1[m][p]; }
                    if (DO_RES && !FUSE_R) { res_out(i, j, 0) = q0[p]; res_out(i, j, 1) = q1[p]; }
                    phi_out(i, j, 0) = f0;
                    phi_out(i, j, 1) = f1;
                    if (phi_out2.p) { phi_out2(i, j, 0) = f0; phi_out2(i, j, 1) = f1; }
                }
            }
            const bool sw = (hx[m] != 0);
            la0[m] = sw ? q0[1] : q0[0]; ra0[m] = sw ? q0[0] : q0[1];
            la1[m] = sw ? q1[1] : q1[0]; ra1[m] = sw ? q1[0] : q1[1];
            finr[m] = fin[0];
        }
        if (FUSE_R) {
            const double c0 = __shfl_down(la0[0], PR), d0 = __shfl_down(ra0[0], PR);
            const double c1 = __shfl_down(la1[0], PR), d1 = __shfl_down(ra1[0], PR);
#pragma unroll
            for (int m = 0; m < GPAIRS; ++m) {
                MG_ROWPK(m);
                if (finr[m] && ((jj & 1) == 0)) {
                    const bool own = (m + 1 < GPAIRS);
                    const int mu = own ? m + 1 : m;
                    const double ua0 = own ? la0[mu] : c0, ub0 = own ? ra0[mu] : d0, ua1 = own ? la1[mu] : c1, ub1 = own ? ra1[mu] : d1;
                    const int ic = (gi0 + 2*pk) >> 1, jc = (gj0 + jj) >> 1;
                    cres_out(ic, jc, 0) = 0.25*(la0[m] + ra0[m] + ua0 + ub0);
                    cres_out(ic, jc, 1) = 0.25*(la1[m] + ra1[m] + ua1 + ub1);
                }
            }
        }
    } else {
#pragma unroll
        for (int m = 0; m < GPAIRS; ++m) {
            MG_ROWPK(m);
            const int j = gj0 + jj;
            const bool rowok = (jj >= E && jj < GT_Y - E);
            double q0[2], q1[2];
            bool fin[2];
#pragma unroll
            for (int p = 0; p < 2; ++p) {
                const int h = hx[m] ^ p;
                const int ii = 2*pk + h;
                fin[p] = rowok && ii >= E && ii < GT_X - E && in[m][p];
                const int i = gi0 + ii;
                const int row = (jj + 1)*AXH + pk;
                const double f0 = s_phi[0][p*CH + row + h], f1 = s_phi[1][p*CH + row + h];
                q0[p] = 0.0; q1[p] = 0.0;
                if (DO_RES) {
                    const double* nb0 = &s_phi[0][(1 - p)*CH + row];
                    const double* nb1 = &s_phi[1][(1 - p)*CH + row];
                    const double t0 = residual_v<INTERIOR>(f0, nb0[0], nb0[1], nb0[h - AXH], nb0[h + AXH], i, j, b, r0[m][p], ac[m][p], facx, facy);
                    const double t1 = residual_v<INTERIOR>(f1, nb1[0], nb1[1], nb1[h - AXH], nb1[h + AXH], i, j, b, r1[m][p], ac[m][p], facx, facy);
                    q0[p] = fin[p] ? t0 : 0.0; q1[p] = fin[p] ? t1 : 0.0;
                    resmax = fmax(resmax, fmax(fabs(q0[p]), fabs(q1[p])));
                }
                if (fin[p]) {
                    if constexpr (RPULL) { rhs(i, j, 0) = r0[m][p]; rhs(i, j, 1) = r1[m][p]; }
                    if (DO_RES && !FUSE_R) { res_out(i, j, 0) = q0[p]; res_out(i, j, 1) = q1[p]; }
                    phi_out(i, j, 0) = f0;
                    phi_out(i, j, 1) = f1;
                    if (phi_out2.p) { phi_out2(i, j, 0) = f0; phi_out2(i, j, 1) = f1; }
                }
            }
            if (FUSE_R) {
                const bool sw = (hx[m] != 0);
                const double la0 = sw ? q0[1] : q0[0], ra0 = sw ? q0[0] : q0[1];
                const double la1 = sw ? q1[1] : q1[0], ra1 = sw ? q1[0] : q1[1];
                const double c0 = __shfl_down(la0, PR), d0 = __shfl_down(ra0, PR);
                const double c1 = __shfl_down(la1, PR), d1 = __shfl_down(ra1, PR);
                if (fin[0] && ((tid & PR) == 0)) {
                    const int ic = (gi0 + 2*pk) >> 1, jc = j >> 1;
                    cres_out(ic, jc, 0) = 0.25*(la0 + ra0 + c0 + d0);
                    cres_out(ic, jc, 1) = 0.25*(la1 + ra1 + c1 + d1);
                }
            }
        }
    }
    MG_STAMP(4);
    if (DO_RES && resnorm) block_max_to<MG_NT>(resnorm, resmax, s_red);
    if (rhsnorm) block_max_to<MG_NT>(rhsnorm, rmax, s_red);
    MG_STAMP(5);
}

template <class TS, bool CC, int SRC, bool DO_RES, bool FUSE_R, int NSW = 4, bool RPULL = false>
__global__ __launch_bounds__(TS::NT, (RPULL && TS::GPAIRS > 1) ? 2 : 4)
void k_smooth (LevBox b, FView phi_out, FView phi_out2, FView rhs, FView acf, FView phi_in, FView crse, FView res_out,
               FView cres_out, double facx, double facy, int ntx, unsigned long long* resnorm,
               unsigned long long* rhsnorm, StopRule sr)
{
    static_assert(!FUSE_R || (CC && DO_RES), "fused restriction is cell-centred only");
    if (NSW != 4 && !vcycle_active(sr)) return;
    constexpr int GT_X = TS::TX, GT_Y = TS::TY;
    __shared__ double s_phi[2][TS::AY*TS::AX];
    __shared__ double s_red[TS::NT/64];
    constexpr bool PLDS = !CC && SRC == SRC_PROLONG;
    __shared__ double s_crs[PLDS ? 2*(TS::AX/2 + 2)*(TS::AY/2 + 2) : 1];
    constexpr int E = DO_RES ? NSW : NSW - 1;
    constexpr int FX = GT_X - 2*E, FY = GT_Y - 2*E;
    const int nb = gridDim.x, q8 = nb >> 3, r8 = nb & 7, xcd = blockIdx.x & 7;
    const int tile = xcd*q8 + min(xcd, r8) + (blockIdx.x >> 3);
    const int bx = tile % ntx, by = tile / ntx;
    const int gi0 = b.vlx + bx*FX - E;
    const int gj0 = b.vly + by*FY - E;
    const bool interior = (gi0 - 1 >= b.vlx) && (gi0 + GT_X <= b.vhx) && (gj0 - 1 >= b.vly) && (gj0 + GT_Y <= b.vhy)
                       && (gi0 > b.lox) && (gi0 + GT_X - 1 < b.hix) && (gj0 > b.loy) && (gj0 + GT_Y - 1 < b.hiy);
    constexpr bool GATE_IN = (NSW == 4);
    if (interior) smooth_tile<TS, CC, SRC, DO_RES, FUSE_R, true, NSW, GATE_IN, RPULL>(s_phi, s_red, s_crs, b, phi_out, phi_out2, rhs, acf, phi_in, crse, res_out, cres_out,
                                                             facx, facy, gi0, gj0, resnorm, rhsnorm, sr);
    else          smooth_tile<TS, CC, SRC, DO_RES, FUSE_R, false, NSW, GATE_IN, RPULL>(s_phi, s_red, s_crs, b, phi_out, phi_out2, rhs, acf, phi_in, crse, res_out, cres_out,
                                                              facx, facy, gi0, gj0, resnorm, rhsnorm, sr);
}

template <bool CC>
__device__ __forceinline__ double restrict_at (const FView& fine, int i, int j, int n)
{
    if (CC) return 0.25*(fine(2*i, 2*j, n) + fine(2*i+1, 2*j, n) + fine(2*i, 2*j+1, n) + fine(2*i+1, 2*j+1, n));
    return (1./16.)*(fine(2*i-1, 2*j-1, n) + 2.*fine(2*i, 2*j-1, n) + fine(2*i+1, 2*j-1, n)
                   + 2.*fine(2*i-1, 2*j, n) + 4.*fine(2*i, 2*j, n) + 2.*fine(2*i+1, 2*j, n)
                   + fine(2*i-1, 2*j+1, n) + 2.*fine(2*i, 2*j+1, n) + fine(2*i+1, 2*j+1, n));
}

template <bool CC>
__global__ __launch_bounds__(256)
void k_restrict (LevBox cb, FView crse, FView fine, int ncomp, StopRule sr)
{
    if (!vcycle_active(sr)) return;
    const int i = cb.vlx + blockIdx.x*blockDim.x + threadIdx.x;
    const int j = cb.vly + blockIdx.y;
    if (i > cb.vhx || j > cb.vhy) return;
    for (int n = 0; n < ncomp; ++n) crse(i, j, n) = restrict_at<CC>(fine, i, j, n);
}

typedef __attribute__((address_space(3))) double lds_double;

struct LowLev { LevBox b; int nxb; int cells; int off; };

struct LView {
    lds_double* p; int nxb; int lox, loy;
    __device__ __forceinline__ lds_double& operator() (int i, int j) const { return p[(i - lox) + (j - loy)*nxb]; }
};
__device__ __forceinline__ LView lplane (lds_double* base, const LowLev& l, int plane)
{
    return LView{base + l.off + plane*l.cells, l.nxb, l.b.lox, l.b.loy};
}

template <bool CC>
__device__ __forceinline__ double lrestrict (const LView& f, int i, int j)
{
    if (CC) return 0.25*(f(2*i, 2*j) + f(2*i+1, 2*j) + f(2*i, 2*j+1) + f(2*i+1, 2*j+1));
    return (1./16.)*(f(2*i-1, 2*j-1) + 2.*f(2*i, 2*j-1) + f(2*i+1, 2*j-1)
                   + 2.*f(2*i-1, 2*j) + 4.*f(2*i, 2*j) + 2.*f(2*i+1, 2*j)
                   + f(2*i-1, 2*j+1) + 2.*f(2*i, 2*j+1) + f(2*i+1, 2*j+1));
}

template <bool CC>
__device__ __forceinline__ double lprolong (const LView& c, int i, int j)
{
    const int ic = i >> 1, jc = j >> 1;
    if (CC) return c(ic, jc);
    const bool io = (i & 1), jo = (j & 1);
    if (io && jo)  return (c(ic, jc) + c(ic+1, jc) + c(ic, jc+1) + c(ic+1, jc+1))*0.25;
    if (io)        return (c(ic, jc) + c(ic+1, jc))*0.5;
    if (jo)        return (c(ic, jc) + c(ic, jc+1))*0.5;
    return c(ic, jc);
}

#define HPS_LOW_FOR_VALID(l, i, j)                                                          \
    for (int j = (l).b.vly + (int)(threadIdx.x >> 5); j <= (l).b.vhy; j += (int)(blockDim.x >> 5))   \
        for (int i = (l).b.vlx + (int)(threadIdx.x & 31); i <= (l).b.vhx; i += 32)

__device__ __forceinline__ double low_fac (double f0, int l) { for (int k = 0; k < l; ++k) f0 *= 0.25; return f0; }

template <bool CC>
__device__ void low_sweeps (lds_double* base, const LowLev& l, double facx, double facy, int nsweeps, int n0 = 0, int n1 = 2)
{
    const int ti = (int)(threadIdx.x & 15), tj = (int)(threadIdx.x >> 4);
    const int si = 16, sj = (int)(blockDim.x >> 4);
    const LView cinv = lplane(base, l, 7);
    if (!CC && l.b.vhy - l.b.vly < sj && l.b.vhx - l.b.vlx < 2*si) {
        const int j = l.b.vly + tj;
        const bool rowok = j <= l.b.vhy;
        const int jc = rowok ? j : l.b.vly;
        int off[2]; bool ok[2]; double ci[2], r0[2], r1[2];
// ... 343 lines not shown
            base[d.off[l+1] + psn + ((j >> 1) + 1)*pn + (i >> 1) + 1] = 0.25*(q0[0] + q0[1] + q0[2] + q0[3]);
        }
        lvl_sync<WAVE>();
    }
}

template <bool WAVE>
__device__ __forceinline__ void low_up_s (lds_double* base, const Low2& d, int l, int t, double fx, double fy)
{
    const int nx = d.nx[l], ny = d.ny[l];
    Blk B; int i, j;
    blk_geometry(B, base + d.off[l], nx, ny, t, fx, fy, i, j);
    const int ps = B.pitch*(ny + 2);
    const lds_double* r = B.c0 + ps;
    const lds_double* cf = base + d.coff[l] + (B.c0 - (base + d.off[l]));
    const int ok[4] = {0, 1, B.pitch, B.pitch + 1};
    const int pn = d.nx[l+1] + 2;
    const lds_double* kc = base + d.off[l+1] + ((j >> 1) + 1)*pn + (i >> 1) + 1;
    const double k0 = B.act ? kc[0] : 0.0;
#pragma unroll
    for (int k = 0; k < 4; ++k) {
        const int o = B.ok[k] ? ok[k] : 0;
        B.r0[k] = r[o]; B.ci[k] = cf[ps + o];
        const double c0 = B.c0[o];
        B.v0[k] = B.ok[k] ? c0 + k0 : 0.0;
        if (B.ok[k]) B.c0[o] = B.v0[k];
    }
    lvl_sync<WAVE>();
    blk_sweep<0, WAVE>(B); blk_sweep<1, WAVE>(B); blk_sweep<0, WAVE>(B); blk_sweep<1, WAVE>(B);
}

__device__ __forceinline__ void tiny_down_s (lds_double* base, const Low2& d, int l, int t, double fx, double fy)
{
    const int nx = d.nx[l], ny = d.ny[l], pitch = nx + 2, ps = pitch*(ny + 2);
    const int i = t & 7, j = t >> 3;
    const bool ok = (i < nx) && (j < ny);
    const int o = ok ? (j + 1)*pitch + i + 1 : pitch + 1;
    lds_double* c0 = base + d.off[l] + o;
    const lds_double* cf = base + d.coff[l] + o;
    const double r0 = c0[ps], a = cf[0], ci = cf[ps];
    const double fxm = wall_mult<true>(i, 0, nx - 1, fx), fym = wall_mult<true>(j, 0, ny - 1, fy);
    if (ok && (((i + j) & 1) == 0)) c0[0] = r0*ci;
    lvl_sync<true>();
    for (int s = 1; s < 4; ++s) {
        if (ok && (((i + j + s) & 1) == 0)) c0[0] = (r0 - offdiag_m((const lds_double*)c0, pitch, fxm, fym))*ci;
        lvl_sync<true>();
    }
    const LevBox b = cc_box(nx, ny);
    const double u0 = residual_at<false>((const lds_double*)c0, pitch, i, j, b, r0, a, fx, fy);
    const double q0 = ok ? u0 : 0.0;
    const double b0 = __shfl_down(q0, 1), g0 = __shfl_down(q0, 8), e0 = __shfl_down(q0, 9);
    if (ok && !(i & 1) && !(j & 1)) {
        const int pn = d.nx[l+1] + 2, psn = pn*(d.ny[l+1] + 2);
        base[d.off[l+1] + psn + ((j >> 1) + 1)*pn + (i >> 1) + 1] = 0.25*(q0 + b0 + g0 + e0);
    }
    lvl_sync<true>();
}

__device__ __forceinline__ void tiny_up_s (lds_double* base, const Low2& d, int l, int t, double fx, double fy)
{
    const int nx = d.nx[l], ny = d.ny[l], pitch = nx + 2, ps = pitch*(ny + 2);
    const int i = t & 7, j = t >> 3;
    const bool ok = (i < nx) && (j < ny);
    const int o = ok ? (j + 1)*pitch + i + 1 : pitch + 1;
    lds_double* c0 = base + d.off[l] + o;
    const double r0 = c0[ps], ci = base[d.coff[l] + ps + o];
    const double fxm = wall_mult<true>(i, 0, nx - 1, fx), fym = wall_mult<true>(j, 0, ny - 1, fy);
    if (ok) {
        const int pn = d.nx[l+1] + 2;
        c0[0] = c0[0] + base[d.off[l+1] + ((j >> 1) + 1)*pn + (i >> 1) + 1];
    }
    lvl_sync<true>();
    for (int s = 0; s < 4; ++s) {
        if (ok && (((i + j + s) & 1) == 0)) c0[0] = (r0 - offdiag_m((const lds_double*)c0, pitch, fxm, fym))*ci;
        lvl_sync<true>();
    }
}

__device__ __forceinline__ void lower_v_guest (const ShiftInit& a, int guest, int nguests)
{
    for (long s = (long)guest*1024 + threadIdx.x; s < a.plane; s += (long)nguests*1024) shift_init_cell(a, s);
}

__global__ __launch_bounds__(1024)
void k_lower_v3 (const Low2* __restrict__ dp, const double* __restrict__ acf_g, const double* __restrict__ cinv_g,
                 const double* __restrict__ res_g, double* __restrict__ cor_g, double* __restrict__ coef_g, int nxA, int nyA, int ctot,
                 double facx0, double facy0, int nsweeps_bottom, StopRule sr, ShiftInit guest)
{
    if (blockIdx.x >= 2) { lower_v_guest(guest, (int)blockIdx.x - 2, (int)gridDim.x - 2); return; }
    extern __shared__ __attribute__((aligned(16))) double lds_raw[];
    lds_double* base = (lds_double*)lds_raw;
    const int t = threadIdx.x;
    const Low2& d = *dp;
    const int nl = d.nl;
    const int cellsA = nxA*nyA;
    res_g += (long)blockIdx.x*cellsA; cor_g += (long)blockIdx.x*cellsA;
    const LevBox bA = cc_box(nxA, nyA);
    Blk A; int iA, jA;
    blk_geometry(A, base, nxA, nyA, t, facx0, facy0, iA, jA);
    double aA[4], rA[4];
#pragma unroll
    for (int k = 0; k < 4; ++k) {
        const int i = iA + (k & 1), j = jA + (k >> 1);
        const int g = min(i, nxA - 1) + min(j, nyA - 1)*nxA;
        const double v0 = res_g[g], v2 = acf_g[g], v3 = cinv_g[g];
        rA[k] = A.ok[k] ? v0 : 0.0; aA[k] = A.ok[k] ? v2 : 0.0; A.ci[k] = A.ok[k] ? v3 : 0.0;
        A.r0[k] = rA[k];
    }
    const bool derive = (sr.k <= 0);
    constexpr int NIMG = 4;
    double img[NIMG];
#pragma unroll
    for (int m = 0; m < NIMG; ++m) { const int q = min(t + 1024*m, ctot - 1); img[m] = derive ? 0.0 : coef_g[q]; }
    const bool active = vcycle_active(sr);
#pragma unroll
    for (int k = 0; k < 4; ++k) { HPS_KEEP(rA[k]); HPS_KEEP(aA[k]); HPS_KEEP(A.ci[k]); }
#pragma unroll
    for (int m = 0; m < NIMG; ++m) HPS_KEEP(img[m]);
    if (!active) return;
    MG_STAMP(8);
    for (int l = 0; l < nl; ++l) {
        const int n1 = (d.nx[l] + 2)*(d.ny[l] + 2);
        lds_double* c = base + d.off[l];
        for (int s = t; s < n1; s += 1024) c[s] = 0.0;
    }
    if (!derive) {
#pragma unroll
        for (int m = 0; m < NIMG; ++m) if (t + 1024*m < ctot) base[d.cbase + t + 1024*m] = img[m];
        for (int q = t + 1024*NIMG; q < ctot; q += 1024) base[d.cbase + q] = coef_g[q];
    }
    __syncthreads();
    if (derive) {
        if (nl > 1 && A.act) {
            const int p1 = d.nx[1] + 2;
            base[d.coff[1] + ((jA >> 1) + 1)*p1 + (iA >> 1) + 1] = 0.25*(aA[0] + aA[1] + aA[2] + aA[3]);
        }
        __syncthreads();
        for (int l = 1; l < nl; ++l) {
            const double fx = lvl_fac(facx0, l), fy = lvl_fac(facy0, l);
            const int nx = d.nx[l], ny = d.ny[l];
            Blk B; int i, j;
            blk_geometry(B, base + d.coff[l], nx, ny, t, fx, fy, i, j);
            const int ps = B.pitch*(ny + 2);
            lds_double* acf = B.c0;
            const int ok[4] = {0, 1, B.pitch, B.pitch + 1};
            if (B.act) {
                double a[4];
#pragma unroll
                for (int k = 0; k < 4; ++k) a[k] = B.ok[k] ? acf[ok[k]] : 0.0;
                if (l + 1 < nl) {
                    const int pn = d.nx[l+1] + 2;
                    base[d.coff[l+1] + ((j >> 1) + 1)*pn + (i >> 1) + 1] = 0.25*(a[0] + a[1] + a[2] + a[3]);
                }
#pragma unroll
                for (int k = 0; k < 4; ++k)
                    if (B.ok[k]) acf[ps + ok[k]] = 1.0/diag_c0<true>(i + (k & 1), j + (k >> 1), cc_box(nx, ny), a[k], fx, fy);
            }
            __syncthreads();
        }
        if (blockIdx.x == 0) for (int q = t; q < ctot; q += 1024) coef_g[q] = base[d.cbase + q];
    }
    MG_STAMP(9);
    const bool bottomA = (nl == 1);
    blk_down_sweeps<false>(A, bottomA ? nsweeps_bottom : 4);
    if (!bottomA) {
        double q0[4];
        blk_residual(A, iA, jA, bA, aA, facx0, facy0, q0);
        if (A.act) {
            const int p1 = d.nx[1] + 2, ps1 = p1*(d.ny[1] + 2);
            base[d.off[1] + ps1 + ((jA >> 1) + 1)*p1 + (iA >> 1) + 1] = 0.25*(q0[0] + q0[1] + q0[2] + q0[3]);
        }
        __syncthreads();
    }
    MG_STAMP(10);
    if (!bottomA) {
        int lw = 1;
        for (; lw < nl; ++lw) {
            const int nbx = (d.nx[lw] + 1) >> 1, nby = (d.ny[lw] + 1) >> 1;
            int lg = 0; while ((1 << lg) < nbx) ++lg;
            if ((nby << lg) <= 64) break;
        }
        for (int l = 1; l < lw; ++l)
            low_down_s<false>(base, d, l, t, lvl_fac(facx0, l), lvl_fac(facy0, l), (l == nl - 1) ? nsweeps_bottom : 4, l == nl - 1);
        MG_STAMP(11);
        if (lw < nl) {
            if (t < 64) {
                for (int l = lw; l < nl; ++l) {
                    MG_STAMP(16 + l);
                    const bool tiny = (d.nx[l] <= 8 && d.ny[l] <= 8 && l < nl - 1);
                    if (tiny) tiny_down_s(base, d, l, t, lvl_fac(facx0, l), lvl_fac(facy0, l));
                    else low_down_s<true>(base, d, l, t, lvl_fac(facx0, l), lvl_fac(facy0, l), (l == nl - 1) ? nsweeps_bottom : 4, l == nl - 1);
                }
// ... 139 lines not shown
                            + 2.*f[w] + 4.*f[w + 1] + 2.*f[w + 2]
                            + f[2*w] + 2.*f[2*w + 1] + f[2*w + 2]);
                if (i >= ox && j >= oy) out(i, j, 0) = v;
            }
            if (l < np) nxt[e] = v;
        }
        __syncthreads();
        cur = nxt; w = wl;
    }
}
static size_t nodal_pyramid_lds (int np)
{
    size_t n = 0;
    for (int l = 0; l < np; ++l) { const int s = np - l; const size_t w = (size_t)NPYR_NB*(1 << s) + (1 << s) - 1; n += w*w; }
    return n*sizeof(double);
}

__global__ void k_level_cinv (const double* __restrict__ acf, double* __restrict__ cinv, int nx, int ny, double fx, double fy)
{
    const int i = blockIdx.x*blockDim.x + threadIdx.x, j = blockIdx.y;
    if (i < nx && j < ny) cinv[i + (long)j*nx] = 1.0/diag_c0<true>(i, j, cc_box(nx, ny), acf[i + (long)j*nx], fx, fy);
}

__global__ void k_copy2 (LevBox b, FView dst, FView src)
{
    const int i = b.vlx + blockIdx.x*blockDim.x + threadIdx.x;
    const int j = b.vly + blockIdx.y;
    if (i > b.vhx || j > b.vhy) return;
    dst(i, j, 0) = src(i, j, 0); dst(i, j, 1) = src(i, j, 1);
}

template <bool CC>
__global__ __launch_bounds__(256)
void k_bottom_sweep (LevBox b, FView cor, FView rhs, FView acf, double facx, double facy, int is, StopRule sr)
{
    if (!vcycle_active(sr)) return;
    const int i = b.vlx + blockIdx.x*blockDim.x + threadIdx.x;
    const int j = b.vly + blockIdx.y;
    if (i > b.vhx || j > b.vhy) return;
    if (is < 0) { cor(i, j, 0) = 0.0; cor(i, j, 1) = 0.0; return; }
    if ((i + j + is) & 1) return;
    const double ci = 1.0/diag_c0<CC>(i, j, b, acf(i, j, 0), facx, facy);
    for (int n = 0; n < 2; ++n) {
        const double w = (i > b.lox) ? cor(i-1, j, n) : 0.0, e = (i < b.hix) ? cor(i+1, j, n) : 0.0;
        const double s = (j > b.loy) ? cor(i, j-1, n) : 0.0, no = (j < b.hiy) ? cor(i, j+1, n) : 0.0;
        double lx = facx*(w + e), ly = facy*(s + no);
        if (CC) {
            lx = (i == b.lox) ? facx*(4./3.)*e : ((i == b.hix) ? facx*(4./3.)*w : lx);
            ly = (j == b.loy) ? facy*(4./3.)*no : ((j == b.hiy) ? facy*(4./3.)*s : ly);
        }
        cor(i, j, n) = (rhs(i, j, n) - (lx + ly))*ci;
    }
}

struct MGLevelDev { LevBox b; long cells; double *acf, *res, *cor, *rescor; };

constexpr long LOWV_MAX_CELLS = 34*34;
constexpr long SMALL_TILE_CELLS = 300L*300L;

constexpr int MG_GO_WORD = 8;
struct SolveRun { int enq, nspec, nzeroed, max_iters; double tol_rel, tol_abs; bool cc; };

struct Multigrid {
    bool cc; int nx, ny; double dx, dy;
    bool hierarchy_ready = false;
    bool nodal_pull1 = false;
    std::vector<MGLevelDev> L;
    int lowv_begin = 1;
    LowLev* d_low = nullptr; size_t low_lds = 0;
    bool bottom = false;
    unsigned long long *d_buf = nullptr, *h_buf = nullptr;
    unsigned long long* h_buf_dev = nullptr;
    long dbg_trips = 0, dbg_solves = 0, dbg_hist[8] = {0,0,0,0,0,0,0,0};
    unsigned long long* h_seq = nullptr; unsigned long long* h_seq_dev = nullptr; unsigned long long seq = 0;
    unsigned long long* d_norms = nullptr;
    unsigned long long* h_norms = nullptr;
    int last_iters = 1;
    SolveRun run{};
    bool defer_post = false; bool deferred_valid = false; MgPost deferred{};
    bool use_low3 = false; Low2 low3{}; Low2* d_low3 = nullptr; size_t low3_lds = 0;
    bool ride_on = false; ShiftInit ride{}; int ride_guests = 0;
    double* cinvA = nullptr;
    double* coef_img = nullptr;
    double* tmp0 = nullptr;
    bool cor_in_tmp = false;
    FView sol, rhs, acf0;

    ~Multigrid () {
        for (auto& l : L) { (void)hipFree(l.acf); (void)hipFree(l.res); (void)hipFree(l.cor); (void)hipFree(l.rescor); }
        if (getenv("HPS_MG_DEBUG")) fprintf(stderr, "mg: solves %ld trips %ld hist %ld %ld %ld %ld %ld %ld\n", dbg_solves, dbg_trips, dbg_hist[0], dbg_hist[1], dbg_hist[2], dbg_hist[3], dbg_hist[4], dbg_hist[5]);
        (void)hipFree(d_buf); (void)hipFree(d_low); (void)hipFree(tmp0); (void)hipFree(d_low3); (void)hipFree(cinvA); (void)hipFree(coef_img);
        if (h_buf) (void)hipHostFree(h_buf);
    }
    FView lv (int il, double* p) const {
        const MGLevelDev& l = L[il];
        const long nxb = l.b.hix - l.b.lox + 1;
        return FView{p, nxb, l.cells, -l.b.lox, -l.b.loy};
    }
    int nlev () const { return (int)L.size(); }
    bool pulls (int il) const {
        return !cc && ((il >= 2 && ((il < lowv_begin && L[il].cells <= SMALL_TILE_CELLS) ||
                                    (il == lowv_begin && !use_low3 && !bottom))) ||
                       (il == 1 && nodal_pull1));
    }
};

static size_t device_max_lds ()
{
    static const size_t lim = [] {
        int dev = 0, a = 0, b = 0;
        if (hipGetDevice(&dev) != hipSuccess) return (size_t)0;
        if (hipDeviceGetAttribute(&a, hipDeviceAttributeMaxSharedMemoryPerBlock, dev) != hipSuccess) a = 0;
        if (hipDeviceGetAttribute(&b, hipDeviceAttributeSharedMemPerBlockOptin, dev) != hipSuccess) b = 0;
        return (size_t)std::max(a, b);
    }();
    return lim;
}

int mg_create (int nx, int ny, double dx, double dy, Multigrid** out)
{
    if (nx % 2 != ny % 2) { set_error("hps_mg_create: nx and ny must have the same parity"); return HPS_ERR_ARG; }
    HPS_REQUIRE((long)(nx + 16)*(ny + 16) < (1L << 27), "hps_mg_create: the kernels address a two-component plane pair by 32-bit byte offsets (at most 2^27 cells per plane)");
    Multigrid* M = new Multigrid;
    M->cc = (nx % 2 == 0); M->nx = nx; M->ny = ny; M->dx = dx; M->dy = dy;
    int hx = M->cc ? nx - 1 : nx + 1, hy = M->cc ? ny - 1 : ny + 1;
    for (int il = 0; il < 31; ++il) {
        MGLevelDev l{};
        l.b.lox = 0; l.b.loy = 0; l.b.hix = hx; l.b.hiy = hy;
        if (M->cc) { l.b.vlx = 0; l.b.vly = 0; l.b.vhx = hx; l.b.vhy = hy; }
        else       { l.b.vlx = 1; l.b.vly = 1; l.b.vhx = hx - 1; l.b.vhy = hy - 1; }
        l.cells = (long)(hx + 1)*(hy + 1);
        HPS_HIP_CHECK(hipMalloc(&l.acf, l.cells*sizeof(double)));
        HPS_HIP_CHECK(hipMalloc(&l.res, 2*l.cells*sizeof(double)));
        HPS_HIP_CHECK(hipMalloc(&l.cor, 2*l.cells*sizeof(double)));
        HPS_HIP_CHECK(hipMalloc(&l.rescor, 2*l.cells*sizeof(double)));
        HPS_HIP_CHECK(hipMemset(l.acf, 0, l.cells*sizeof(double)));
        HPS_HIP_CHECK(hipMemset(l.res, 0, 2*l.cells*sizeof(double)));
        HPS_HIP_CHECK(hipMemset(l.cor, 0, 2*l.cells*sizeof(double)));
        HPS_HIP_CHECK(hipMemset(l.rescor, 0, 2*l.cells*sizeof(double)));
        M->L.push_back(l);
        bool ok;
        const int nxl = hx + 1, nyl = hy + 1;
        if (M->cc) { ok = nxl >= 4 && nyl >= 4 && nxl % 2 == 0 && nyl % 2 == 0; if (ok) { hx = nxl/2 - 1; hy = nyl/2 - 1; } }
        else       { ok = nxl >= 8 && nyl >= 8 && hx % 2 == 0 && hy % 2 == 0;   if (ok) { hx /= 2; hy /= 2; } }
        if (!ok) break;
    }
    if (M->nlev() < 2) { delete M; set_error("hps_mg_create: grid too small to coarsen"); return HPS_ERR_ARG; }
    if (!M->cc)
        HPS_HIP_CHECK(hipFuncSetAttribute((const void*)k_nodal_acf_pyramid<5>, hipFuncAttributeMaxDynamicSharedMemorySize, (int)nodal_pyramid_lds(NPYR_MAX)));
    const int nl = M->nlev();
    M->lowv_begin = nl - 1;
    for (int il = nl - 1; il >= 1; --il) if (M->L[il].cells <= LOWV_MAX_CELLS) M->lowv_begin = il;
    if (M->cc) {
        for (int il = 1; il < nl; ++il) {
            const LevBox& b = M->L[il].b;
            const bool fits = (b.hix + 1 <= 64) && (b.hiy + 1 <= 64) && (nl - il <= LOW2_MAXLEV)
                           && (il + 1 >= nl || (M->L[il+1].b.hix + 1 <= 32 && M->L[il+1].b.hiy + 1 <= 32));
            if (!fits) continue;
            M->use_low3 = true; M->lowv_begin = il;
            Low2& e = M->low3;
            e.nl = nl - il;
            int off3 = 0;
            for (int k = 0; k < e.nl; ++k) {
                const LevBox& bk = M->L[il + k].b;
                e.nx[k] = bk.hix + 1; e.ny[k] = bk.hiy + 1; e.off[k] = off3;
                off3 += (k == 0 ? 1 : 2)*(e.nx[k] + 2)*(e.ny[k] + 2);
            }
            e.cbase = off3; e.coff[0] = off3;
            for (int k = 1; k < e.nl; ++k) { e.coff[k] = off3; off3 += 2*(e.nx[k] + 2)*(e.ny[k] + 2); }
            e.ctot = std::max(off3 - e.cbase, 1);
            e.total = off3;
            HPS_HIP_CHECK(hipMalloc(&M->coef_img, (size_t)e.ctot*sizeof(double)));
            HPS_HIP_CHECK(hipMemset(M->coef_img, 0, (size_t)e.ctot*sizeof(double)));
            M->low3_lds = (size_t)off3*sizeof(double);
            if (M->low3_lds > 64*1024)
                HPS_HIP_CHECK(hipFuncSetAttribute((const void*)k_lower_v3, hipFuncAttributeMaxDynamicSharedMemorySize, (int)M->low3_lds));
            HPS_HIP_CHECK(hipMalloc(&M->d_low3, sizeof(Low2)));
            HPS_HIP_CHECK(hipMemcpy(M->d_low3, &e, sizeof(Low2), hipMemcpyHostToDevice));
            HPS_HIP_CHECK(hipMalloc(&M->cinvA, (size_t)e.nx[0]*e.ny[0]*sizeof(double)));
            int dev = 0, ncu = 0;
            HPS_HIP_CHECK(hipGetDevice(&dev));
            HPS_HIP_CHECK(hipDeviceGetAttribute(&ncu, hipDeviceAttributeMultiprocessorCount, dev));
            M->ride_guests = std::max(ncu - 2, 1);
            break;
        }
    }
    if (!M->use_low3) {
        long cells = 0;
        for (int il = M->lowv_begin; il < nl; ++il) cells += M->L[il].cells;
        M->low_lds = (size_t)(8*cells)*sizeof(double);
        hipFuncAttributes fa{};
        HPS_HIP_CHECK(hipFuncGetAttributes(&fa, M->cc ? (const void*)k_lower_v<true> : (const void*)k_lower_v<false>));
        if (M->low_lds + fa.sharedSizeBytes > device_max_lds()) { M->bottom = true; M->lowv_begin = nl - 1; M->low_lds = 0; }
    }
    M->nodal_pull1 = !M->cc && M->lowv_begin > 1;
    if (!M->use_low3 && !M->bottom) {
        std::vector<LowLev> low;
        int off = 0;
        for (int il = M->lowv_begin; il < nl; ++il) {
            const MGLevelDev& l = M->L[il];
            low.push_back(LowLev{l.b, l.b.hix - l.b.lox + 1, (int)l.cells, off});
            off += 8*(int)l.cells;
        }
        if (M->low_lds > 64*1024) {
            HPS_HIP_CHECK(hipFuncSetAttribute((const void*)k_lower_v<true>, hipFuncAttributeMaxDynamicSharedMemorySize, (int)M->low_lds));
            HPS_HIP_CHECK(hipFuncSetAttribute((const void*)k_lower_v<false>, hipFuncAttributeMaxDynamicSharedMemorySize, (int)M->low_lds));
        }
        HPS_HIP_CHECK(hipMalloc(&M->d_low, low.size()*sizeof(LowLev)));
        HPS_HIP_CHECK(hipMemcpy(M->d_low, low.data(), low.size()*sizeof(LowLev), hipMemcpyHostToDevice));
    }
    HPS_HIP_CHECK(hipMalloc(&M->d_buf, (3 + MG_MAX_VCYCLES)*MG_NSUB*sizeof(unsigned long long)));
    HPS_HIP_CHECK(hipHostMalloc(&M->h_buf, ((3 + MG_MAX_VCYCLES)*MG_NSUB + 8)*sizeof(unsigned long long), hipHostMallocMapped));
    HPS_HIP_CHECK(hipHostGetDevicePointer((void**)&M->h_buf_dev, M->h_buf, 0));
    M->h_seq = M->h_buf + (3 + MG_MAX_VCYCLES)*MG_NSUB; M->h_seq_dev = M->h_buf_dev + (3 + MG_MAX_VCYCLES)*MG_NSUB;
    *M->h_seq = 0ULL;
    HPS_HIP_CHECK(hipMemset(M->d_buf, 0, (3 + MG_MAX_VCYCLES)*MG_NSUB*sizeof(unsigned long long)));
    memset(M->h_buf, 0, (3 + MG_MAX_VCYCLES)*MG_NSUB*sizeof(unsigned long long));
    M->d_norms = M->d_buf + MG_NSUB; M->h_norms = M->h_buf + MG_NSUB;
    HPS_HIP_CHECK(hipMalloc(&M->tmp0, 2*M->L[0].cells*sizeof(double)));
    HPS_HIP_CHECK(hipMemset(M->tmp0, 0, 2*M->L[0].cells*sizeof(double)));
    *out = M;
    return HPS_OK;
}

template <class TS, bool CC, int SRC, bool DO_RES, int NSW = 4, bool RPULL = false>
static void launch_smooth_ts (Multigrid* M, int il, FView phi_out, FView phi_out2, FView rhs, FView acf, FView phi_in, FView crse,
                              FView res_out, FView cres_out, unsigned long long* resnorm, unsigned long long* rhsnorm,
                              const StopRule& sr, hipStream_t st)
{
    const LevBox& b = M->L[il].b;
    constexpr int E = DO_RES ? NSW : NSW - 1;
    constexpr int FX = TS::TX - 2*E, FY = TS::TY - 2*E;
    const int ntx = ceil_div(b.vhx - b.vlx + 1, FX), nty = ceil_div(b.vhy - b.vly + 1, FY);
    const double fac = (double)(1 << il);
    const double ldx = M->dx*fac, ldy = M->dy*fac;
    const double facx = 1.0/(ldx*ldx), facy = 1.0/(ldy*ldy);
    constexpr bool FUSE = CC && DO_RES;
    hipLaunchKernelGGL((k_smooth<TS, CC, SRC, DO_RES, FUSE, NSW, RPULL>), dim3(ntx*nty), dim3(TS::NT), 0, st, b, phi_out, phi_out2, rhs, acf,
                       phi_in, crse, res_out, cres_out, facx, facy, ntx, resnorm, rhsnorm, sr);
}

template <bool CC, int SRC, bool DO_RES>
static void launch_smooth (Multigrid* M, int il, FView phi_out, FView phi_out2, FView rhs, FView acf, FView phi_in, FView crse,
                           FView res_out, FView cres_out, unsigned long long* resnorm, unsigned long long* rhsnorm,
                           const StopRule& sr, hipStream_t st)
{
    if (M->L[il].cells <= SMALL_TILE_CELLS)
        launch_smooth_ts<TileSmall, CC, SRC, DO_RES>(M, il, phi_out, phi_out2, rhs, acf, phi_in, crse, res_out, cres_out, resnorm, rhsnorm, sr, st);
    else
        launch_smooth_ts<TileBig, CC, SRC, DO_RES>(M, il, phi_out, phi_out2, rhs, acf, phi_in, crse, res_out, cres_out, resnorm, rhsnorm, sr, st);
}

template <bool CC>
static void restrict_residual_if_nodal (Multigrid* M, int il, const StopRule& sr, hipStream_t st)
{
    if (CC) return;
    const LevBox& cb = M->L[il+1].b;
    hipLaunchKernelGGL(k_restrict<CC>, dim3(ceil_div(cb.vhx - cb.vlx + 1, 64), cb.vhy - cb.vly + 1), dim3(64), 0, st,
                       cb, M->lv(il+1, M->L[il+1].res), M->lv(il, M->L[il].rescor), 2, sr);
}

template <bool CC>
static void vcycle (Multigrid* M, int k, double tol_rel, double tol_abs, hipStream_t st)
{
    const int nl = M->nlev();
    const int lb = M->lowv_begin;
    const FView none{};
    const StopRule sr{M->d_norms, k, tol_rel, tol_abs};
    for (int il = 1; il < lb; ++il) {
        if (!M->pulls(il))
            launch_smooth<CC, SRC_ZERO, true>(M, il, M->lv(il, M->L[il].cor), none, M->lv(il, M->L[il].res), M->lv(il, M->L[il].acf), none,
                                              none, M->lv(il, M->L[il].rescor), M->lv(il+1, M->L[il+1].res), nullptr, nullptr, sr, st);
        else if constexpr (!CC) {
            if (M->L[il].cells > SMALL_TILE_CELLS)
                launch_smooth_ts<TileMid, CC, SRC_ZERO, true, 4, true>(M, il, M->lv(il, M->L[il].cor), none, M->lv(il, M->L[il].res), M->lv(il, M->L[il].acf), none,
                                                                       M->lv(il-1, M->L[il-1].rescor), M->lv(il, M->L[il].rescor), M->lv(il+1, M->L[il+1].res), nullptr, nullptr, sr, st);
            else
                launch_smooth_ts<TileSmall, CC, SRC_ZERO, true, 4, true>(M, il, M->lv(il, M->L[il].cor), none, M->lv(il, M->L[il].res), M->lv(il, M->L[il].acf), none,
                                                                         M->lv(il-1, M->L[il-1].rescor), M->lv(il, M->L[il].rescor), M->lv(il+1, M->L[il+1].res), nullptr, nullptr, sr, st);
        }
        if (!M->pulls(il + 1)) restrict_residual_if_nodal<CC>(M, il, sr, st);
    }
    {
        const double fac = (double)(1 << lb);
        const double ldx = M->dx*fac, ldy = M->dy*fac;
        const LevBox& bb = M->L[nl-1].b;
        const int nsweeps = std::max(16, (std::max(bb.hix - bb.lox + 1, bb.hiy - bb.loy + 1) + 1)/2*2);
        if (M->bottom) {
            const FView cor = M->lv(lb, M->L[lb].cor), rhs = M->lv(lb, M->L[lb].res), acf = M->lv(lb, M->L[lb].acf);
            const dim3 grid(ceil_div(bb.vhx - bb.vlx + 1, 64), bb.vhy - bb.vly + 1);
            for (int is = -1; is < nsweeps; ++is)
                hipLaunchKernelGGL(k_bottom_sweep<CC>, grid, dim3(64), 0, st, bb, cor, rhs, acf, 1.0/(ldx*ldx), 1.0/(ldy*ldy), is, sr);
        } else if (M->use_low3) {
            const int guests = (k == 0 && M->ride_on) ? M->ride_guests : 0;
            M->ride_on = false;
            hipLaunchKernelGGL(k_lower_v3, dim3(2 + guests), dim3(1024), M->low3_lds, st, M->d_low3, M->L[lb].acf, M->cinvA, M->L[lb].res, M->L[lb].cor,
                               M->coef_img, M->low3.nx[0], M->low3.ny[0], M->low3.ctot, 1.0/(ldx*ldx), 1.0/(ldy*ldy), nsweeps, sr, M->ride);
        } else
            hipLaunchKernelGGL(k_lower_v<CC>, dim3(CC ? 1 : 2), dim3(1024), M->low_lds, st, M->d_low, nl - lb, M->L[lb].acf, M->L[lb].res,
                               M->L[lb].cor, 1.0/(ldx*ldx), 1.0/(ldy*ldy), nsweeps, sr, M->pulls(lb) ? M->lv(lb-1, M->L[lb-1].rescor) : FView{});
    }
    for (int il = lb - 1; il >= 1; --il) {
        double* crse = (il + 1 == lb) ? M->L[il+1].cor : M->L[il+1].rescor;
        launch_smooth<CC, SRC_PROLONG, false>(M, il, M->lv(il, M->L[il].rescor), none, M->lv(il, M->L[il].res), M->lv(il, M->L[il].acf),
                                              M->lv(il, M->L[il].cor), M->lv(il+1, crse), none, none, nullptr, nullptr, sr, st);
    }
    {
        double* crse = (1 == lb) ? M->L[1].cor : M->L[1].rescor;
        double* in = M->cor_in_tmp ? M->tmp0 : M->L[0].cor;
        double* out = M->cor_in_tmp ? M->L[0].cor : M->tmp0;
        launch_smooth_ts<typename HugeTileOf<CC>::type, CC, SRC_PROLONG, true, 8>(M, 0, M->lv(0, out), M->sol, M->rhs, M->acf0, M->lv(0, in), M->lv(1, crse),
                                                             M->lv(0, M->L[0].rescor), M->lv(1, M->L[1].res), M->d_norms + (2 + k)*MG_NSUB,
                                                             nullptr, sr, st);
        M->cor_in_tmp = !M->cor_in_tmp;
    }
    if (!M->nodal_pull1) restrict_residual_if_nodal<CC>(M, 0, sr, st);
}

__global__ __launch_bounds__(256)
void k_post_norms (const unsigned long long* __restrict__ src, volatile unsigned long long* dst, int nwords,
                   volatile unsigned long long* seq_slot, unsigned long long seq, int* go_word, StopRule after)
{
    {   const bool act = vcycle_active(after);
        if (threadIdx.x == 0) *go_word = act ? 0 : 1; }
    for (int w = threadIdx.x; w < nwords; w += blockDim.x) dst[w] = src[w];
    HPS_HOST_STORES_ACKNOWLEDGED();
    __syncthreads();
    if (threadIdx.x == 0) { *seq_slot = seq; }
}

template <bool CC>
static void enqueue_cycles (Multigrid* M, hipStream_t st)
{
    SolveRun& r = M->run;
    for (int v = 0; v < r.nspec && r.enq < r.max_iters; ++v, ++r.enq) {
        if (r.enq >= r.nzeroed) {
            const int more = std::min(r.max_iters - r.nzeroed, 64);
            (void)hipMemsetAsync(M->d_norms + (2 + r.nzeroed)*MG_NSUB, 0, more*MG_NSUB*sizeof(unsigned long long), st);
            r.nzeroed += more;
        }
        vcycle<CC>(M, r.enq, r.tol_rel, r.tol_abs, st);
    }
    ++M->seq; ++M->dbg_trips;
    if (M->defer_post) {
        M->defer_post = false; M->deferred_valid = true;
        M->deferred = MgPost{M->d_buf, (volatile unsigned long long*)M->h_buf_dev, (3 + r.enq)*MG_NSUB, (volatile unsigned long long*)M->h_seq_dev, M->seq,
                             StopRule{M->d_norms, r.enq, r.tol_rel, r.tol_abs}};
        return;
    }
    hipLaunchKernelGGL(k_post_norms, dim3(1), dim3(256), 0, st, M->d_buf, (volatile unsigned long long*)M->h_buf_dev,
                       (3 + r.enq)*MG_NSUB, (volatile unsigned long long*)M->h_seq_dev, M->seq,
                       reinterpret_cast<int*>(M->d_buf) + MG_GO_WORD, StopRule{M->d_norms, r.enq, r.tol_rel, r.tol_abs});
}

struct GuestPass { bool on = false; SlabView f{hps_slab{}}; GradPsiSxSy ga{}; };

template <bool CC>
static int solve1_hierarchy (Multigrid* M, int max_iters, hipStream_t st, const GuestPass* guest = nullptr)
{
    const int lb = M->lowv_begin;
    max_iters = std::min(max_iters, MG_MAX_VCYCLES);
    const StopRule always{nullptr, -1, 0.0, 0.0};
    int nspec = std::min(std::max(M->last_iters, 1), std::max(max_iters, 1));
    int nzeroed = std::min(max_iters, nspec + 8);
    const int nzero_words = (2 + nzeroed)*MG_NSUB;
    int first = 1;
    if (CC) {
        PyrOut po{};
        const int np = std::min(lb, 5);
        for (int il = 1; il <= np; ++il) { po.p[il-1] = M->L[il].acf; po.nx[il-1] = M->L[il].b.hix + 1; po.ny[il-1] = M->L[il].b.hiy + 1; }
        const double lfac = (double)(1 << lb), lfx = 1.0/(M->dx*lfac*M->dx*lfac), lfy = 1.0/(M->dy*lfac*M->dy*lfac);
        if (M->use_low3 && lb <= np) { po.cinv = M->cinvA; po.cinv_l = lb - 1; po.cfx = lfx; po.cfy = lfy; }
        if (guest) {
            const int gx = ceil_div(M->nx, 32), gy = ceil_div(M->ny, 32);
            const SlabView& f = guest->f;
            const int nbx = ceil_div(f.js, 256), rows = f.ny + 2*f.ng;
            hipLaunchKernelGGL(k_hierarchy_gradpsi, dim3(gx*gy + nbx*rows), dim3(256), 0, st, M->acf0, M->nx, M->ny, po, np, M->d_norms, nzero_words,
                               gx, gy, f, guest->ga, nbx);
        } else
        hipLaunchKernelGGL(k_acf_pyramid, dim3(ceil_div(M->nx, 32), ceil_div(M->ny, 32)), dim3(256), 0, st, M->acf0, M->nx, M->ny, po, np,
                           M->d_norms, nzero_words);
        first = np + 1;
    } else {
        NodalPyr o{};
        const int np = std::min(lb, NPYR_MAX);
        o.np = np;
        o.vhx[0] = M->L[0].b.vhx; o.vhy[0] = M->L[0].b.vhy;
        for (int il = 1; il <= np; ++il) { o.lev[il-1] = M->lv(il, M->L[il].acf); o.vhx[il] = M->L[il].b.vhx; o.vhy[il] = M->L[il].b.vhy; }
        const int tx = ceil_div(M->L[np].b.hix, NPYR_NB), ty = ceil_div(M->L[np].b.hiy, NPYR_NB);
        switch (np) {
            case 1: hipLaunchKernelGGL(k_nodal_acf_pyramid<1>, dim3(tx, ty), dim3(256), nodal_pyramid_lds(np), st, M->acf0, o, M->d_norms, nzero_words); break;
            case 2: hipLaunchKernelGGL(k_nodal_acf_pyramid<2>, dim3(tx, ty), dim3(256), nodal_pyramid_lds(np), st, M->acf0, o, M->d_norms, nzero_words); break;
            case 3: hipLaunchKernelGGL(k_nodal_acf_pyramid<3>, dim3(tx, ty), dim3(256), nodal_pyramid_lds(np), st, M->acf0, o, M->d_norms, nzero_words); break;
            case 4: hipLaunchKernelGGL(k_nodal_acf_pyramid<4>, dim3(tx, ty), dim3(256), nodal_pyramid_lds(np), st, M->acf0, o, M->d_norms, nzero_words); break;
            default: hipLaunchKernelGGL(k_nodal_acf_pyramid<5>, dim3(tx, ty), dim3(256), nodal_pyramid_lds(np), st, M->acf0, o, M->d_norms, nzero_words); break;
        }
        first = np + 1;
    }
    for (int il = first; il <= lb; ++il) {
        const LevBox& cb = M->L[il].b;
        FView fine = (il == 1) ? M->acf0 : M->lv(il-1, M->L[il-1].acf);
        hipLaunchKernelGGL(k_restrict<CC>, dim3(ceil_div(cb.vhx - cb.vlx + 1, 64), cb.vhy - cb.vly + 1), dim3(64), 0, st,
                           cb, M->lv(il, M->L[il].acf), fine, 1, always);
    }
    if (CC && M->use_low3 && lb > 5) {
        const double lfac = (double)(1 << lb);
        const int lnx = M->L[lb].b.hix + 1, lny = M->L[lb].b.hiy + 1;
        hipLaunchKernelGGL(k_level_cinv, dim3(ceil_div(lnx, 64), lny), dim3(64), 0, st, M->L[lb].acf, M->cinvA, lnx, lny,
                           1.0/(M->dx*lfac*M->dx*lfac), 1.0/(M->dy*lfac*M->dy*lfac));
    }
    HPS_HIP_CHECK(hipGetLastError());
    return HPS_OK;
}

template <bool CC>
static int solve1_begin (Multigrid* M, double tol_rel, double tol_abs, int max_iters, hipStream_t st)
{
    max_iters = std::min(max_iters, MG_MAX_VCYCLES);
    M->cor_in_tmp = false;
    const StopRule always{nullptr, -1, 0.0, 0.0};
    int nspec = std::min(std::max(M->last_iters, 1), std::max(max_iters, 1));
    int nzeroed = std::min(max_iters, nspec + 8);
    if (M->hierarchy_ready) M->hierarchy_ready = false;
    else if (int e = solve1_hierarchy<CC>(M, max_iters, st)) return e;
    launch_smooth<CC, SRC_DIRECT, true>(M, 0, M->lv(0, M->L[0].cor), FView{}, M->rhs, M->acf0, M->sol, FView{}, M->lv(0, M->L[0].rescor),
                                        M->lv(1, M->L[1].res), M->d_norms, M->d_norms + MG_NSUB, always, st);
    if (!M->nodal_pull1) restrict_residual_if_nodal<CC>(M, 0, always, st);
    M->run = SolveRun{0, nspec, nzeroed, max_iters, tol_rel, tol_abs, CC};
    enqueue_cycles<CC>(M, st);
    HPS_HIP_CHECK(hipGetLastError());
    return HPS_OK;
}

template <bool CC>
static int solve1_finish (Multigrid* M, int* iters_out, double* resnorm_out, int* extra, hipStream_t st)
{
    SolveRun& r = M->run;
    int status = HPS_OK;
    int iters = 0;
    double last_norm = 0.0;
    bool converged = false, diverged = false, first_trip = true;
    if (extra) *extra = 0;
    auto slot_value = [M] (int slot) {
        unsigned long long m = 0ULL;
        for (int q = 0; q < MG_NSUB; ++q) m = std::max(m, M->h_norms[slot*MG_NSUB + q]);
        double dd; memcpy(&dd, &m, 8); return dd;
    };
    while (true) {
        {   volatile unsigned long long* hs = M->h_seq;
            long spins = 0;
            while (*hs != M->seq) {
                if ((++spins & 0xfffff) == 0 && hipStreamQuery(st) != hipErrorNotReady) {
                    if (*hs == M->seq) break;
                    HPS_HIP_CHECK(hipStreamSynchronize(st));
                    if (*hs != M->seq) { set_error("hps_mg_solve1: the norm read-back never arrived"); return HPS_ERR_HIP; }
                }
            }
            __atomic_thread_fence(__ATOMIC_ACQUIRE); }
        const double res0 = slot_value(0), rhs0 = slot_value(1);
        const double max_norm = (rhs0 >= res0) ? rhs0 : res0;
        const double target = std::max(r.tol_abs, std::max(r.tol_rel, 1.e-16)*max_norm);
        last_norm = res0; iters = 0;
        converged = (res0 <= target); diverged = false;
        for (int k = 0; k < r.enq && !converged && !diverged; ++k) {
            last_norm = slot_value(2 + k); ++iters;
            if (last_norm <= target) converged = true;
            else if (!(last_norm <= 1.e20*max_norm)) diverged = true;
        }
        if (first_trip) {
            const double prev = (r.enq == 0) ? res0 : slot_value(2 + r.enq - 1);
            const bool gate_active = prev > target && prev <= 1.e20*max_norm;
            if (gate_active != !(converged || diverged)) { set_error("hps_mg_solve1: host and device stopping rules disagree"); return HPS_ERR_HIP; }
            if (extra) *extra = gate_active ? 1 : 0;
            first_trip = false;
        }
        if (converged || diverged) break;
        if (r.enq >= r.max_iters) { set_error("hps_mg_solve1: not converged after max_iters V-cycles"); status = HPS_ERR_MG_MAXITER; break; }
        r.nspec = 1;
        enqueue_cycles<CC>(M, st);
    }
    if (diverged) { set_error("hps_mg_solve1: diverging"); status = HPS_ERR_MG_DIVERGED; }
    M->last_iters = std::max(1, iters); ++M->dbg_solves; ++M->dbg_hist[std::min(iters, 7)];
    if (iters == 0) {
        const LevBox& b0 = M->L[0].b;
        hipLaunchKernelGGL(k_copy2, dim3(ceil_div(b0.vhx - b0.vlx + 1, 64), b0.vhy - b0.vly + 1), dim3(64), 0, st,
                           b0, M->sol, M->lv(0, M->L[0].cor));
    }
    HPS_HIP_CHECK(hipGetLastError());
    if (iters_out) *iters_out = iters;
    if (resnorm_out) *resnorm_out = last_norm;
    return status;
}

static void set_views (Multigrid* M, const hps_slab& s, int sol_comp, int rhs_comp, int acf_comp)
{
    const int sh = M->cc ? 0 : 1;
    const int o = s.ng - sh;
    M->sol  = FView{s.p + (long)sol_comp*s.nstride, s.jstride, s.nstride, o, o};
    M->rhs  = FView{s.p + (long)rhs_comp*s.nstride, s.jstride, s.nstride, o, o};
    M->acf0 = FView{s.p + (long)acf_comp*s.nstride, s.jstride, s.nstride, o, o};
}

int mg_solve1_begin (void* handle, hps_slab s, int sol_comp, int rhs_comp, int acf_comp, double tol_rel, double tol_abs,
                     int max_iters, hipStream_t st)
{
    Multigrid* M = static_cast<Multigrid*>(handle);
    HPS_REQUIRE(s.nstride < (1L << 27) && s.ng <= 8, "mg_solve1_begin: planes of at most 2^27 doubles and at most 8 guard cells (32-bit byte offsets in the kernels)");
// ... 25 lines not shown
{
    if (!handle) return;
    Multigrid* M = static_cast<Multigrid*>(handle);
    M->hierarchy_ready = false; M->ride_on = false;
}
void mg_defer_post (void* handle) { Multigrid* M = static_cast<Multigrid*>(handle); M->defer_post = true; M->deferred_valid = false; }
bool mg_take_deferred_post (void* handle, MgPost* out)
{
    Multigrid* M = static_cast<Multigrid*>(handle);
    M->defer_post = false;
    if (!M->deferred_valid) return false;
    M->deferred_valid = false; *out = M->deferred;
    return true;
}
bool mg_ride_shift_init (void* handle, const ShiftInit& pass)
{
    Multigrid* M = static_cast<Multigrid*>(handle);
    if (!M->cc || !M->use_low3 || M->bottom) return false;
    M->ride = pass; M->ride_on = true;
    return true;
}
const int* mg_gate_after_enqueued (void* handle)
{
    return reinterpret_cast<const int*>(static_cast<Multigrid*>(handle)->d_buf) + MG_GO_WORD;
}
bool mg_solve1_ready (void* handle)
{
    Multigrid* M = static_cast<Multigrid*>(handle);
    return *(volatile unsigned long long*)M->h_seq == M->seq;
}
int mg_solve1_finish (void* handle, int* iters_out, double* resnorm_out, int* extra, hipStream_t st)
{
    Multigrid* M = static_cast<Multigrid*>(handle);
    return M->cc ? solve1_finish<true>(M, iters_out, resnorm_out, extra, st) : solve1_finish<false>(M, iters_out, resnorm_out, extra, st);
}

int mg_solve1 (Multigrid* M, hps_slab s, int sol_comp, int rhs_comp, int acf_comp, double tol_rel, double tol_abs,
               int max_iters, int* iters_out, double* resnorm_out, hipStream_t st)
{
    if (int e = mg_solve1_begin(M, s, sol_comp, rhs_comp, acf_comp, tol_rel, tol_abs, max_iters, st)) return e;
    return mg_solve1_finish(M, iters_out, resnorm_out, nullptr, st);
}

}

using namespace hps;

extern "C" int hps_mg_create (int nx, int ny, double dx, double dy, void** handle)
{
    HPS_REQUIRE(nx >= 2 && ny >= 2 && handle, "hps_mg_create: bad size");
    Multigrid* M = nullptr;
    if (int e = mg_create(nx, ny, dx, dy, &M)) return e;
    *handle = M;
    return HPS_OK;
}

extern "C" int hps_mg_info (void* handle, int* cc, int* nlev, int* lowv_begin, int* lowv_kind, long* lowv_lds, int* tiles,
                            int* nodal_pull1, int* pyr_levels, int* pyr_restricts)
{
    HPS_REQUIRE(handle, "hps_mg_info: null handle");
    const Multigrid* M = static_cast<const Multigrid*>(handle);
    const int lb = M->lowv_begin;
    if (cc) *cc = M->cc;
    if (nlev) *nlev = M->nlev();
    if (lowv_begin) *lowv_begin = lb;
    if (lowv_kind) *lowv_kind = M->bottom ? HPS_MG_LOWV_BOTTOM : M->use_low3 ? HPS_MG_LOWV_V3 : M->cc ? HPS_MG_LOWV_CC : HPS_MG_LOWV_NODAL;
    if (lowv_lds) *lowv_lds = (long)(M->use_low3 ? M->low3_lds : M->low_lds);
    if (tiles) {
        for (int il = 0; il < HPS_MG_MAXLEV; ++il) {
            int t = -1;
            if (il < lb) {
                const bool small = M->L[il].cells <= SMALL_TILE_CELLS;
                t = M->pulls(il) ? (small ? HPS_MG_TILE_SMALL_PULL : HPS_MG_TILE_MID_PULL) : (small ? HPS_MG_TILE_SMALL : HPS_MG_TILE_BIG);
            }
            tiles[il] = t;
        }
    }
    if (nodal_pull1) *nodal_pull1 = M->nodal_pull1;
    if (pyr_levels) *pyr_levels = std::min(lb, M->cc ? 5 : NPYR_MAX);
    if (pyr_restricts) *pyr_restricts = lb - std::min(lb, M->cc ? 5 : NPYR_MAX);
    return HPS_OK;
}

extern "C" int hps_mg_solve1 (void* handle, hps_slab slab, int sol_comp, int rhs_comp, int acoef_comp, double tol_rel,
                              double tol_abs, int max_iters, int* iters_host, double* resnorm_host, hps_stream stream)
{
    HPS_REQUIRE(handle && slab.p, "hps_mg_solve1: null argument");
    Multigrid* M = static_cast<Multigrid*>(handle);
    HPS_REQUIRE(slab.nx == M->nx && slab.ny == M->ny, "hps_mg_solve1: slab size does not match the solver");
    HPS_REQUIRE(sol_comp >= 0 && sol_comp + 1 < slab.ncomp && rhs_comp >= 0 && rhs_comp + 1 < slab.ncomp &&
                acoef_comp >= 0 && acoef_comp < slab.ncomp, "hps_mg_solve1: bad component");
    HPS_REQUIRE(M->cc || slab.ng >= 1, "hps_mg_solve1: node-centred solve needs >= 1 guard cell");
    HPS_REQUIRE(slab.nstride < (1L << 27) && slab.ng <= 8, "hps_mg_solve1: planes of at most 2^27 doubles and at most 8 guard cells (32-bit byte offsets in the kernels)");
    return mg_solve1(M, slab, sol_comp, rhs_comp, acoef_comp, tol_rel, tol_abs, max_iters, iters_host, resnorm_host,
                     (hipStream_t)stream);
}

extern "C" int hps_mg_solve1_fabs (void* handle, hps_slab sol2, hps_slab rhs2, hps_slab acoef1, double tol_rel, double tol_abs,
                                   int max_iters, int* iters_host, double* resnorm_host, hps_stream stream)
{
    HPS_REQUIRE(handle && sol2.p && rhs2.p && acoef1.p, "hps_mg_solve1_fabs: null argument");
    Multigrid* M = static_cast<Multigrid*>(handle);
    for (const hps_slab* s : {&sol2, &rhs2, &acoef1}) {
        HPS_REQUIRE(s->nx == M->nx && s->ny == M->ny, "hps_mg_solve1_fabs: view size does not match the solver");
        HPS_REQUIRE(M->cc || s->ng >= 1, "hps_mg_solve1_fabs: node-centred solve needs >= 1 guard cell in every view");
    }
    HPS_REQUIRE(sol2.ncomp >= 2 && rhs2.ncomp >= 2 && acoef1.ncomp >= 1, "hps_mg_solve1_fabs: sol and rhs need two components, acoef one");
    const int sh = M->cc ? 0 : 1;
    HPS_REQUIRE(sol2.nstride < (1L << 27) && rhs2.nstride < (1L << 27) && acoef1.nstride < (1L << 27), "hps_mg_solve1_fabs: planes of at most 2^27 doubles (32-bit byte offsets in the kernels)");
    M->sol  = FView{sol2.p, sol2.jstride, sol2.nstride, sol2.ng - sh, sol2.ng - sh};
    M->rhs  = FView{rhs2.p, rhs2.jstride, rhs2.nstride, rhs2.ng - sh, rhs2.ng - sh};
    M->acf0 = FView{acoef1.p, acoef1.jstride, acoef1.nstride, acoef1.ng - sh, acoef1.ng - sh};
    hipStream_t st = (hipStream_t)stream;
    if (int e = M->cc ? solve1_begin<true>(M, tol_rel, tol_abs, max_iters, st) : solve1_begin<false>(M, tol_rel, tol_abs, max_iters, st)) return e;
    return mg_solve1_finish(M, iters_host, resnorm_host, nullptr, st);
}

void mg_rider (void* handle, int** dev_words, const int** host_words)
{
    Multigrid* M = static_cast<Multigrid*>(handle);
    *dev_words = reinterpret_cast<int*>(M->d_buf);
    *host_words = reinterpret_cast<const int*>(M->h_buf);
}

extern "C" int hps_mg_debug_stamps (long long* stamps16_host)
{
#ifndef HPS_STAMPS
    (void)stamps16_host; set_error("hps_mg_debug_stamps: the library was built without -DHPS_STAMPS (make stamps)"); return HPS_ERR_UNSUPPORTED;
#else
    static long long* d = nullptr;
    if (!d) {
        HPS_HIP_CHECK(hipMalloc(&d, 48*sizeof(long long)));
        HPS_HIP_CHECK(hipMemset(d, 0, 48*sizeof(long long)));
        HPS_HIP_CHECK(hipMemcpyToSymbol(HIP_SYMBOL(g_mg_dbg), &d, sizeof(d)));
        return HPS_OK;
    }
    HPS_HIP_CHECK(hipDeviceSynchronize());
    HPS_HIP_CHECK(hipMemcpy(stamps16_host, d, 48*sizeof(long long), hipMemcpyDeviceToHost));
    return HPS_OK;
#endif
}

extern "C" int hps_mg_destroy (void* handle)
{
    delete static_cast<Multigrid*>(handle);
    return HPS_OK;
}
```

hipace_amd/csrc/particles_tiled.hip:

```cpp
#include "common.h"
#include <type_traits>
#include "particle_math.h"
#include "tiling.h"
#include "mg_gate.h"
#include "beam_deposit.h"

#include <algorithm>
#include <atomic>
#include <cstdio>
#include <cstdlib>
#include <cstring>
#include <mutex>
#include <set>
#include <string>

namespace hps {

static std::atomic<bool> g_record{false};
static std::mutex g_record_mu;
static std::set<std::string> g_recorded;
static void record_launch (const char* kernel, std::initializer_list<int> args)
{
    std::string n(kernel);
    char sep = '<';
// ... 37 lines not shown

__device__ __forceinline__ void vm_wait_all () { __builtin_amdgcn_s_waitcnt(0x0F70); }

template <int ORDER>
__device__ __forceinline__ double laser_gather_lds (const double* a, int pitch, int li, int lj, const double* lx, const double* ly)
{
    double A = 0.0;
#pragma unroll
    for (int iy = 0; iy <= ORDER; ++iy)
#pragma unroll
        for (int ix = 0; ix <= ORDER; ++ix) A += lx[ix]*ly[iy]*lds_get(a + (lj + iy)*pitch + li + ix);
    return A;
}
template <int ORDER>
__device__ __forceinline__ void laser_gather_grad_lds (const double* a, int pitch, int li, int lj, const double* lx, const double* ly,
                                                       double dx_inv, double dy_inv, double& A, double& ADx, double& ADy)
{
    A = 0.0; ADx = 0.0; ADy = 0.0;
#pragma unroll
    for (int iy = 0; iy <= ORDER; ++iy)
#pragma unroll
        for (int ix = 0; ix <= ORDER; ++ix) {
            const double* c = a + (lj + iy)*pitch + li + ix;
            const double w = lx[ix]*ly[iy];
            A += w*lds_get(c);
            ADx += w*0.5*dx_inv*(lds_get(c + 1) - lds_get(c - 1));
            ADy += w*0.5*dy_inv*(lds_get(c + pitch) - lds_get(c - pitch));
        }
}

__device__ __forceinline__ int4 tile_record (const int* __restrict__ offsets, const TailWork& tw, long n, bool& tail)
{
    const int b0 = (int)blockIdx.x - tw.extra;
    const int b = b0 - tw.nwg;
    tail = b < 0;
    if (tail) {
        const long nn = tw.live_n ? (long)*tw.live_n : n;
        const long first = (long)tw.first + 256L*b0;
        return make_int4(0, (int)min(first, nn), (int)min(first + 256, nn), 0);
    }
    return reinterpret_cast<const int4*>(offsets + tile_launch_offset(gridDim.x - tw.nwg - tw.extra))[b];
}
constexpr int TAIL_ORIGIN = -(1 << 24);

template <int R, int RP = R, int NT = 256, int NC = 6>
__device__ __forceinline__ void load_region (double* img, const SlabView& f, const int* comps, int nc, int ox, int oy, int tid);

template <int ORDER, int TS, int MASK, bool LASER = false, bool VBW = false>
__global__ __launch_bounds__(256)
void k_deposit_tiled (SlabView f, hps_plasma pl, const int* __restrict__ offsets, int ntx, DepComps cm,
                      PartConsts k, int* n_qsa, int* n_fallback, const int* __restrict__ tile_flag, TailWork tw, BeamPairWork bw,
                      const int* go)
{
    if (go && *go == 0) return;
    if ((int)blockIdx.x < bw.nwg) {
        beam_pair_block<ORDER>(f, bw, (int)blockIdx.x, k.dx_inv, k.dy_inv, k.xoff, k.yoff);
        return;
    }
    constexpr int R = TS + 2*TILE_HALO;
    constexpr int RP = R, PL = RP*R;
    if (tile_flag && !tile_flag[offsets[gridDim.x + 2 + blockIdx.x]]) return;
    extern __shared__ __attribute__((aligned(16))) double acc[];
    const int gc[6] = {cm.jx, cm.jy, cm.jz, cm.rho, cm.chi, cm.rhomjz};
    int slot[6]; int na = 0;
#pragma unroll
    for (int c = 0; c < 6; ++c) {
        const bool on = (MASK >= 0) ? ((MASK >> c) & 1) : (gc[c] >= 0);
        slot[c] = on ? na++ : -1;
    }

    bool tail;
    const int4 lrec = tile_record(offsets, tw, pl.n, tail);
    const int tile = lrec.x;
    const int ox = tail ? TAIL_ORIGIN : (tile % ntx)*TS - TILE_HALO, oy = tail ? TAIL_ORIGIN : (tile / ntx)*TS - TILE_HALO;
    const int tid = threadIdx.x;
    PT_STAMP(0);
    const int pend = lrec.z;
    int nfb = 0;
    struct Rec { double x, y, w, ux, uy, psi; uint64_t id; int ion; };
    auto fetch = [&] (int ip) {
        Rec r;
        r.x = pl.x[ip]; r.y = pl.y[ip]; r.w = pl.w[ip];
        r.ux = pl.ux[ip]; r.uy = pl.uy[ip]; r.psi = pl.psi[ip];
        if constexpr (VBW) r.id = (r.w != 0.0) ? HPS_ID_VALID : 0ULL;
        else r.id = pl.idcpu[ip];
        r.ion = k.can_ionize ? pl.ion_lev[ip] : 1;
        return r;
    };
    constexpr int NB = 4;
    Rec rec[NB];
    const int ipb = lrec.y + tid;
    if (ipb < pend) {
#pragma unroll
        for (int u = 0; u < NB; ++u) rec[u] = fetch(min(ipb + 256*u, pend - 1));
    }
    {
        double2* z = (double2*)acc;
        for (int s = tid; s < na*PL/2; s += 256) z[s] = make_double2(0.0, 0.0);
    }
    double* aimg = acc + na*PL;
    if constexpr (LASER) { const int ca[1] = {k.aabs}; load_region<R, R, 256, 1>(aimg, f, ca, 1, ox, oy, tid); }
    __syncthreads();
    PT_STAMP(1);

    for (int ip0 = ipb; ip0 < pend; ip0 += 256*NB) {
      if (ip0 != ipb) {
#pragma unroll
        for (int u = 0; u < NB; ++u) rec[u] = fetch(min(ip0 + 256*u, pend - 1));
      }
#pragma unroll
      for (int u = 0; u < NB; ++u) {
        const int ip = ip0 + 256*u;
        if (ip >= pend) break;
        const Rec cur = rec[u];
        const uint64_t id = cur.id;
        if (!(id & HPS_ID_VALID)) continue;
        const double psi_inv = 1.0/cur.psi;
        const double vx_c = cur.ux*psi_inv;
        const double vy_c = cur.uy*psi_inv;
        double q_invvol = k.a*cur.w;
        double q_mu0_mass = k.b;
        if (k.can_ionize) { const double il = (double)cur.ion; q_invvol *= il; q_mu0_mass *= il; }
        double sx[ORDER + 1], sy[ORDER + 1];
        const int i0 = shape_weights<ORDER>((cur.x - k.xoff)*k.dx_inv, sx);
        const int j0 = shape_weights<ORDER>((cur.y - k.yoff)*k.dy_inv, sy);
        const int li = i0 - ox, lj = j0 - oy;
        const bool local = (li >= 0 && li + ORDER < R && lj >= 0 && lj + ORDER < R);
        double gamma_psi;
        if constexpr (LASER) {
            double A = (local ? laser_gather_lds<ORDER>(aimg, R, li, lj, sx, sy)
                              : laser_gather<ORDER>(f, k.aabs, (cur.x - k.xoff)*k.dx_inv, (cur.y - k.yoff)*k.dy_inv))*k.laser_fac;
            if (k.can_ionize) A *= (double)cur.ion*(double)cur.ion;
            gamma_psi = 0.5*((1.0 + 0.5*A)*psi_inv*psi_inv + vx_c*vx_c*k.c_inv*k.c_inv + vy_c*vy_c*k.c_inv*k.c_inv + 1.0);
        } else {
            gamma_psi = 0.5*(psi_inv*psi_inv + vx_c*vx_c*k.c_inv*k.c_inv + vy_c*vy_c*k.c_inv*k.c_inv + 1.0);
        }
        if (gamma_psi < 0.0 || gamma_psi > k.max_qsa || psi_inv < 0.0) {
            if (n_qsa) atomicAdd(n_qsa, 1);
            pl.w[ip] = 0.0;
            pl.idcpu[ip] = (VBW ? pl.idcpu[ip] : id) & ~HPS_ID_VALID;
            if (pl.psi_half) pl.psi_half[ip] = 0.0;
            continue;
        }
        if (k.can_ionize && cur.ion == 0) continue;
        const double wv[6] = {vx_c, vy_c, (gamma_psi - 1.0)*k.c, gamma_psi, q_mu0_mass*psi_inv, 1.0};
        if (local) {
#pragma unroll
            for (int iy = 0; iy <= ORDER; ++iy) {
#pragma unroll
                for (int ix = 0; ix <= ORDER; ++ix) {
                    const double cd = q_invvol*sx[ix]*sy[iy];
                    double* p = acc + (lj + iy)*RP + li + ix;
#pragma unroll
                    for (int c = 0; c < 6; ++c) if (slot[c] >= 0) lds_add(p + slot[c]*PL, cd*wv[c]);
                }
            }
        } else {
            nfb += !tail;
#pragma unroll
            for (int iy = 0; iy <= ORDER; ++iy) {
#pragma unroll
                for (int ix = 0; ix <= ORDER; ++ix) {
                    const double cd = q_invvol*sx[ix]*sy[iy];
                    double* p = f.p + f.off(i0 + ix, j0 + iy);
#pragma unroll
                    for (int c = 0; c < 6; ++c) if (slot[c] >= 0) atomic_add_f64(p + gc[c]*f.ns, cd*wv[c]);
                }
            }
        }
      }
    }
    if (n_fallback && nfb) atomicAdd(n_fallback, nfb);
    PT_STAMP(2);
    __syncthreads();
    PT_STAMP(3);

    for (int s = tid; s < R*R; s += 256) {
        const int lj = s / R, li = s - lj*R;
        const int i = ox + li, j = oy + lj;
        if (i < -f.ng || i >= f.nx + f.ng || j < -f.ng || j >= f.ny + f.ng) continue;
        double* p = f.p + f.off(i, j);
#pragma unroll
        for (int c = 0; c < 6; ++c) {
            if (slot[c] >= 0) {
                const double v = acc[slot[c]*PL + lj*RP + li];
                if (v != 0.0) atomic_add_f64(p + gc[c]*f.ns, v);
            }
        }
    }
    PT_STAMP(4);
}

template <int R, int RP, int NT, int NC>
__device__ __forceinline__ void load_region (double* img, const SlabView& f, const int* comps, int nc, int ox, int oy, int tid)
{
    constexpr int NIT = (R*R + NT - 1)/NT;
    double v[NIT][NC];
#pragma unroll
    for (int it = 0; it < NIT; ++it) {
// ... 946 lines not shown
```

include/hpslice.h:

```cpp
#ifndef HPSLICE_H_
#define HPSLICE_H_

#include <stdint.h>

#ifdef __cplusplus
extern "C" {
#endif

typedef void* hps_stream;

enum { HPS_OK = 0, HPS_ERR_ARG = 1, HPS_ERR_HIP = 2, HPS_ERR_FFT = 3, HPS_ERR_MG_DIVERGED = 4,
       HPS_ERR_MG_MAXITER = 5, HPS_ERR_COMM = 6, HPS_ERR_UNSUPPORTED = 7 };

enum { HPS_BC_REFLECTING = 0, HPS_BC_PERIODIC = 1, HPS_BC_ABSORBING = 2 };

typedef struct {
    double* p;
    int nx, ny, ng, ncomp;
    long jstride, nstride;
} hps_slab;

typedef struct {
    double *x, *y, *w, *ux, *uy, *psi, *x_prev, *y_prev, *ux_half, *uy_half, *psi_half;
    uint64_t* idcpu;
// ... 18 lines not shown
int hps_deposit_current (hps_slab slab, hps_plasma plasma, hps_geom geom, const int comp[6],
                         double charge, double mass, int depos_order, double max_qsa_weighting,
                         int can_ionize, int* n_qsa_violation, hps_stream stream);

int hps_explicit_deposit (hps_slab slab, hps_plasma plasma, hps_geom geom, const int cache[4],
                          const int depos[2], double charge, double mass, int depos_order,
                          int derivative_type, int can_ionize, hps_stream stream);

int hps_advance_plasma (hps_slab slab, hps_plasma plasma, hps_geom geom, const int comp[5],
                        double charge, double mass, int depos_order, int temp_slice,
                        int n_subcycles, int can_ionize, hps_stream stream);

int hps_deposit_current_laser (hps_slab slab, hps_plasma plasma, hps_geom geom, const int comp[6], int aabs_comp,
                               double charge, double mass, int depos_order, double max_qsa_weighting,
                               int can_ionize, int* n_qsa_violation, hps_stream stream);
int hps_explicit_deposit_laser (hps_slab slab, hps_plasma plasma, hps_geom geom, const int cache[4], int aabs_comp,
                                const int depos[2], double charge, double mass, int depos_order,
                                int derivative_type, int can_ionize, hps_stream stream);
int hps_advance_plasma_laser (hps_slab slab, hps_plasma plasma, hps_geom geom, const int comp[5], int aabs_comp,
                              double charge, double mass, int depos_order, int temp_slice,
                              int n_subcycles, int can_ionize, hps_stream stream);


int hps_tiling_create (int nx, int ny, int tile_size, long max_particles, void** handle);
int hps_reorder_particles (void* tiling, hps_plasma src, hps_plasma dst, hps_geom geom,
                           hps_stream stream);
int hps_tiling_info (void* tiling, int* ntiles, const int** offsets_dev, const unsigned int** perm_dev);
int hps_tiling_destroy (void* tiling);

int hps_beam_sort_by_box (const double* z_dev, long n, double plo_z, double dz, int num_boxes,
                          unsigned long long* counts_dev, unsigned long long* offsets_dev,
                          unsigned long long* perm_dev, hps_stream stream);

int hps_deposit_current_tiled (hps_slab slab, hps_plasma plasma, hps_geom geom, const int comp[6],
                               double charge, double mass, int depos_order, double max_qsa_weighting,
                               int can_ionize, int* n_qsa_violation, void* tiling, int* n_fallback,
                               hps_stream stream);
int hps_explicit_deposit_tiled (hps_slab slab, hps_plasma plasma, hps_geom geom, const int cache[4],
                                const int depos[2], double charge, double mass, int depos_order,
                                int derivative_type, int can_ionize, void* tiling, int* n_fallback,
                                hps_stream stream);
int hps_advance_plasma_tiled (hps_slab slab, hps_plasma plasma, hps_geom geom, const int comp[5],
                              double charge, double mass, int depos_order, int temp_slice,
                              int n_subcycles, int can_ionize, void* tiling, int* n_fallback,
                              hps_stream stream);
int hps_deposit_current_tiled_laser (hps_slab slab, hps_plasma plasma, hps_geom geom, const int comp[6], int aabs_comp,
                                     double charge, double mass, int depos_order, double max_qsa_weighting,
                                     int can_ionize, int* n_qsa_violation, void* tiling, int* n_fallback,
                                     hps_stream stream);
int hps_explicit_deposit_tiled_laser (hps_slab slab, hps_plasma plasma, hps_geom geom, const int cache[4], int aabs_comp,
                                      const int depos[2], double charge, double mass, int depos_order,
                                      int derivative_type, int can_ionize, void* tiling, int* n_fallback,
                                      hps_stream stream);
int hps_advance_plasma_tiled_laser (hps_slab slab, hps_plasma plasma, hps_geom geom, const int comp[5], int aabs_comp,
                                    double charge, double mass, int depos_order, int temp_slice,
                                    int n_subcycles, int can_ionize, void* tiling, int* n_fallback,
                                    hps_stream stream);
int hps_tiling_set_validity (void* tiling, int by_weight, int by_psi_half);

int hps_particles_record (int on);
int hps_particles_recorded (char* buf, long cap, long* len);


int hps_poisson_create (int nx, int ny, double dx, double dy, void** handle);
int hps_poisson_solve (void* handle, const double* staging, hps_slab dst, int dst_comp,
                       hps_stream stream);
int hps_poisson_solve_batch (void* handle, int nbatch, const double* staging, hps_slab dst,
                             const int* dst_comps, hps_stream stream);
enum { HPS_POISSON_OWN_SYM = 0, HPS_POISSON_OWN_POW2 = 1, HPS_POISSON_DENSE = 2, HPS_POISSON_ROCFFT = 3 };
int hps_poisson_info (void* handle, int* backend, int* x_len, int* tri_rows);
int hps_poisson_destroy (void* handle);

int hps_mg_create (int nx, int ny, double dx, double dy, void** handle);
int hps_mg_solve1 (void* handle, hps_slab slab, int sol_comp, int rhs_comp, int acoef_comp,
                   double tol_rel, double tol_abs, int max_iters, int* iters_host,
                   double* resnorm_host, hps_stream stream);
int hps_mg_solve1_fabs (void* handle, hps_slab sol2, hps_slab rhs2, hps_slab acoef1, double tol_rel, double tol_abs,
                        int max_iters, int* iters_host, double* resnorm_host, hps_stream stream);
enum { HPS_MG_LOWV_V3 = 0, HPS_MG_LOWV_CC = 1, HPS_MG_LOWV_NODAL = 2, HPS_MG_LOWV_BOTTOM = 3 };
enum { HPS_MG_TILE_SMALL = 0, HPS_MG_TILE_BIG = 1, HPS_MG_TILE_SMALL_PULL = 2, HPS_MG_TILE_MID_PULL = 3 };
enum { HPS_MG_MAXLEV = 31 };
int hps_mg_info (void* handle, int* cc, int* nlev, int* lowv_begin, int* lowv_kind, long* lowv_lds, int* tiles,
                 int* nodal_pull1, int* pyr_levels, int* pyr_restricts);
int hps_mg_destroy (void* handle);

int hps_mg2_create (int nx, int ny, double dx, double dy, void** handle);
int hps_mg2_solve2 (void* handle, double* sol2_dev, const double* rhs2_dev, const double* acoef_real_dev,
                    const double* acoef_imag_dev, double tol_rel, double tol_abs, int max_iters, int* iters_host,
                    double* resnorm_host, hps_stream stream);
enum { HPS_MG2_BOTTOM_LOWER_V = 0, HPS_MG2_BOTTOM_SINGLE_BLOCK = 1, HPS_MG2_BOTTOM_PER_SWEEP = 2 };
enum { HPS_MG2_TILE_SINGLE_BLOCK = 0, HPS_MG2_TILE_SMALL = 1, HPS_MG2_TILE_BIG = 2 };
int hps_mg2_info (void* handle, int* nlev, int* low_top, int* bottom, int* tiles);
int hps_mg2_destroy (void* handle);


#define HPS_MAX_ION_LEVELS 56
typedef struct {
    int nx, ny, nz; double lo[3], hi[3];
    int order; int deriv_type;
    int plasma_ppc[2]; double plasma_density; double plasma_radius;
    double plasma_charge, plasma_mass; double max_qsa; int n_subcycles;
    int beam_profile;
    double beam_zmin, beam_zmax, beam_radius, beam_density;
    double beam_umean[3], beam_pos_mean[3], beam_pos_std[3]; int beam_ppc[3]; double beam_charge;
    int bc; double mg_tol_rel, mg_tol_abs; int deposit_rho; int n_steps;
    double dt; int beam_n_subcycles; double beam_mass; double ext_E_slope[2];
    int bxby_solver; double predcorr_tol; int predcorr_max_iter; double predcorr_mix; int field_bc;
    int laser_on; double laser_a0, laser_w0, laser_L0, laser_lambda0, laser_pos[3];
    double laser_zfoc; int laser_solver; int laser_use_phase;
    int si_units;
    int grid_current_on; double grid_current_peak, grid_current_mean[3], grid_current_std[3];
    double laser_mg_tol_rel, laser_mg_tol_abs;
    int beam_radiation_reaction; double background_density_SI; int beam_no_z_push;
    int plasma_no_neutralize;
    int ion_on; int ion_ppc[2]; double ion_density, ion_mass, ion_charge; int ion_init_level, ion_Z;
    double ion_energies[HPS_MAX_ION_LEVELS]; unsigned long long ion_seed;
    int beam_spin_tracking; double beam_initial_spin[3]; double beam_spin_anom;
    int dt_adaptive; double nt_per_betatron, dt_max, adaptive_threshold_uz, adaptive_phase_tolerance;
    int adaptive_no_predict_step, adaptive_no_phase_control, adaptive_phase_substeps;
    double adaptive_density, max_time, beam_uz_std;
    double ext_Ez_slope;
    int beam_do_salame; int salame_n_iter; double salame_relative_tolerance; int salame_no_advance;
    double salame_Ez_target_slope;
} hps_deck;

enum { HPS_SAL_EZ_TARGET = 0, HPS_SAL_EZ_NO_SALAME, HPS_SAL_EZ, HPS_SAL_JX, HPS_SAL_JY, HPS_SAL_JZB, HPS_SAL_BX, HPS_SAL_BY,
       HPS_SAL_SY, HPS_SAL_SX, HPS_SAL_SY_BACK, HPS_SAL_SX_BACK, HPS_SAL_NCOMP };

enum { HPS_C_N_JXB = 0, HPS_C_N_JYB, HPS_C_CHI, HPS_C_SY, HPS_C_SX, HPS_C_EXMBY, HPS_C_EYPBX,
       HPS_C_EZ, HPS_C_BX, HPS_C_BY, HPS_C_BZ, HPS_C_PSI, HPS_C_JXB, HPS_C_JYB, HPS_C_JZB,
       HPS_C_JX, HPS_C_JY, HPS_C_RHOMJZ, HPS_C_P_JXB, HPS_C_P_JYB, HPS_C_ION_RHOMJZ, HPS_C_RHO,
       HPS_NCOMP_MAX };

enum { HPS_PC_N_JX = 0, HPS_PC_N_JY, HPS_PC_EXMBY, HPS_PC_EYPBX, HPS_PC_EZ, HPS_PC_BX, HPS_PC_BY, HPS_PC_BZ,
       HPS_PC_PSI, HPS_PC_JX, HPS_PC_JY, HPS_PC_JZ, HPS_PC_RHOMJZ, HPS_PC_P_BX, HPS_PC_P_BY, HPS_PC_P_JX,
       HPS_PC_P_JY, HPS_PC_ION_RHOMJZ, HPS_PC_IT_BX, HPS_PC_IT_BY, HPS_PC_PIT_BX, HPS_PC_PIT_BY, HPS_PC_RHO,
       HPS_PC_NCOMP_MAX };

int hps_engine_create (const hps_deck* deck, int device, void** handle);
int hps_engine_destroy (void* handle);
int hps_engine_begin_step (void* handle);
int hps_engine_set_step (void* handle, int step);
int hps_engine_set_time (void* handle, double t, double dt);
int hps_engine_beam_moments (void* handle, double* out4_host);
int hps_engine_solve_slice (void* handle, int islice);
int hps_engine_solve_slice_begin (void* handle, int islice);
int hps_engine_solve_slice_finish (void* handle, int islice);
int hps_engine_slice_ready (void* handle);
int hps_engine_run_step (void* handle);
int hps_engine_sync (void* handle);
int hps_engine_info (void* handle, int* ncomp, int* nguards, long* nparticles);
hps_slab hps_engine_slab (void* handle);
hps_plasma hps_engine_plasma (void* handle);
int hps_engine_tiling (void* handle, void** tiling);
hps_plasma hps_engine_ions (void* handle);
int hps_engine_ion_stats (void* handle, long* n_ionized_host, long* n_product_host);
hps_stream hps_engine_stream (void* handle);
int hps_engine_checksums (void* handle, double* out_host);
int hps_engine_stats (void* handle, long* total_vcycles, long* slices_done);
int hps_engine_early_init_slices (void* handle, long* n_slices);
int hps_engine_pc_stats (void* handle, long* iterations, double* error_sum);
int hps_engine_pc_zero_b_slices (void* handle, long* slices);
int hps_engine_laser_info (void* handle, int* aabs_comp, double* envelope_abs_sum_host);
int hps_engine_laser_envelope (void* handle, double* out_host);
int hps_engine_set_laser_import (void* handle, int on, int step);
int hps_engine_export_laser_slice (void* handle, int islice, double* msg_dev);
int hps_engine_import_laser_slice (void* handle, int islice, const double* msg_dev);
int hps_engine_import_laser_from (void* handle, int islice, void* src_engine);
int hps_engine_set_laser_grid (void* handle, const int* n_cell , const double* patch_lo ,
                               const double* patch_hi , int interp_order);
int hps_engine_laser_grid (void* handle, int* nxl, int* nyl, int* zeta_lo, int* zeta_hi);
int hps_engine_laser_chi (void* handle, double* out_host);
int hps_laser_interp_aabs (hps_slab slab, int c_aabs, const double* a_plane, int nxl, int nyl, double dxl, double dyl,
                           double xoffl, double yoffl, hps_geom geom, int order, void* stream);
int hps_laser_interp_chi (hps_slab slab, int c_chi, const double* chi_initial, double* chi_out, int nxl, int nyl, double dxl,
                          double dyl, double xoffl, double yoffl, hps_geom geom, int shrink, int order, void* stream);
typedef struct { double a0, w0, L0, pos[3], zfoc, cep, propagation_angle_yz, pft_yz; } hps_laser_pulse;
int hps_engine_set_laser_pulses (void* handle, int n, const hps_laser_pulse* pulses);
int hps_engine_add_laser_samples (void* handle, int geometry, const double* data_host, const long extent[3],
                                  const double offset[3], const double spacing[3], double unit);
int hps_engine_set_insitu_laser (void* handle, int on);
int hps_engine_insitu_laser (void* handle, double* out_host );
int hps_engine_set_diagnostics (void* handle, int on);
int hps_engine_set_field_diagnostic (void* handle, int ncomps, const int* comps, const int coarsening[3]);
int hps_engine_field_diagnostic (void* handle, double* out_host);
int hps_engine_set_field_diagnostic_box (void* handle, int ncomps, const int* comps, const int coarsening[3], int slice_dir,
                                         const double* patch_lo , const double* patch_hi );
int hps_engine_field_diagnostic_geometry (void* handle, int* n3, double* lo3, double* hi3);

int hps_engine_set_insitu_fields (void* handle, int on);
int hps_engine_insitu_fields (void* handle, double* out_host );

int hps_engine_set_insitu_plasma (void* handle, double radius);
int hps_engine_laser_vcycles (void* handle, long* vcycles);
int hps_engine_set_insitu_beam (void* handle, double radius);
int hps_engine_insitu_beam (void* handle, double* out_host );
int hps_engine_insitu_plasma (void* handle, double* out_host );

int hps_engine_set_tiling (void* handle, int tile_size, int sort_period);
int hps_engine_fallbacks (void* handle, long* n_fallback_host);
int hps_engine_set_density_profile (void* handle, int nr, const double* r_host, const double* fr_host, int nt,
                                    const double* ct_host, const double* ft_host);
int hps_engine_set_plasma_init (void* handle, const int* plasma_fine_ppc, const int* ion_fine_ppc, double hollow_core_radius);
int hps_engine_set_fine_patch (void* handle, const unsigned char* mask_host, int transition_cells);
int hps_engine_set_plasma_momentum (void* handle, int species, const double u_mean[3], const double u_std[3], unsigned long long seed);
int hps_engine_set_plasma_symmetry (void* handle, int do_symmetrize, int prevent_centered_particle);
int hps_engine_set_fusion (void* handle, int on);
int hps_engine_sorts (void* handle, long* n_sorts_host);
int hps_engine_set_profiling (void* handle, int on);
int hps_engine_set_profiling_stride (void* handle, int stride);
int hps_engine_phase_times (void* handle, double* ms_host, long* nslices_host);

int hps_engine_beam_info (void* handle, long* nbeam_host, long* offsets_host );
int hps_engine_set_beam_particles (void* handle, long n, const double* soa_host, long* n_outside);
int hps_engine_set_beam_storage (void* handle, double* storage_dev );
int hps_engine_initial_beam (void* handle, double* dst_dev);
int hps_engine_beam_state (void* handle, long* boundaries_host, double* soa_host);
int hps_engine_beam_capacity (void* handle, long* cap_host);
int hps_engine_set_beam_capacity (void* handle, long cap);
int hps_engine_beam_message_rows (void* handle, int* rows_host);
int hps_engine_beam_spin (void* handle, double* soa_host);
int hps_engine_set_beam_import (void* handle, int on);
int hps_engine_export_beam_slice (void* handle, int islice, double* msg_dev);
int hps_engine_import_beam_slice (void* handle, int islice, const double* msg_dev);
int hps_engine_assume_initial_beam_support (void* handle);

int hps_engine_record_event (void* handle, int slot, void** event_out);
int hps_stream_pool_shared_pairs (int device);
int hps_engine_wait_event (void* handle, void* event);
int hps_engine_copy_async (void* handle, void* dst_dev, const void* src_dev, long bytes);

int hps_open_boundary (double* staging_dev, int nbatch, int nx, int ny, const double lo[2], const double hi[2],
                       unsigned no_monopole_mask, void* stream);

int hps_engine_salame_stats (void* handle, double* out_host );
int hps_salame_only_advance (hps_slab slab, hps_plasma plasma, hps_geom geom, int bx_comp, int by_comp, double charge,
                             double mass, int depos_order, int can_ionize, hps_stream stream);
int hps_salame_jxjy_from_bxby (hps_slab slab, hps_geom geom, int bx_comp, int by_comp, int chi_comp, int jx_comp, int jy_comp,
                               hps_stream stream);
int hps_salame_sxsy_from_jz (hps_slab slab, hps_geom geom, int jz_comp, int sy_comp, int sx_comp, hps_stream stream);
int hps_salame_get_w (hps_slab slab, int ez_target_comp, int ez_no_salame_comp, int ez_comp, int jz_comp, double* scratch_dev,
                      double* out4_host, hps_stream stream);
int hps_salame_scale_beam_slice (double* w_dev, long n, double W, hps_stream stream);
// ... 127 lines not shown
```

Baseline: 1717.

## Derive low-level MG coefficient image in a guest block of initial smooth

```diff
diff --git a/hipace_amd/_lib.py b/hipace_amd/_lib.py
--- a/hipace_amd/_lib.py
+++ b/hipace_amd/_lib.py
@@ -160,6 +160,7 @@
                                      C.POINTER(C.c_int), C.POINTER(C.c_double), C.c_void_p]),
     "hps_mg_info": (C.c_int, [C.c_void_p, C.POINTER(C.c_int), C.POINTER(C.c_int), C.POINTER(C.c_int), C.POINTER(C.c_int),
                               C.POINTER(C.c_long), C.POINTER(C.c_int), C.POINTER(C.c_int), C.POINTER(C.c_int), C.POINTER(C.c_int)]),
+    "hps_mg_info_schedule": (C.c_int, [C.c_void_p, C.POINTER(C.c_int)]),
     "hps_mg_destroy": (C.c_int, [C.c_void_p]),
     "hps_mg2_create": (C.c_int, [C.c_int, C.c_int, C.c_double, C.c_double, C.POINTER(C.c_void_p)]),
     "hps_mg2_solve2": (C.c_int, [C.c_void_p, C.c_void_p, C.c_void_p, C.c_void_p, C.c_void_p, C.c_double, C.c_double, C.c_int,
@@ -187,6 +188,8 @@
                                        C.c_void_p, C.c_void_p]),
     "hps_engine_stats": (C.c_int, [C.c_void_p, C.POINTER(C.c_long), C.POINTER(C.c_long)]),
     "hps_engine_early_init_slices": (C.c_int, [C.c_void_p, C.POINTER(C.c_long)]),
+    "hps_engine_schedule": (C.c_int, [C.c_void_p, C.POINTER(C.c_int), C.POINTER(C.c_int)]),
+    "hps_engine_qsa_drops": (C.c_int, [C.c_void_p, C.POINTER(C.c_long)]),
     "hps_engine_set_insitu_plasma": (C.c_int, [C.c_void_p, C.c_double]),
     "hps_engine_set_insitu_beam": (C.c_int, [C.c_void_p, C.c_double]),
     "hps_engine_insitu_beam": (C.c_int, [C.c_void_p, C.c_void_p]),
diff --git a/hipace_amd/api.py b/hipace_amd/api.py
--- a/hipace_amd/api.py
+++ b/hipace_amd/api.py
@@ -354,14 +354,19 @@
     LOWV = ("v3", "v-cc", "v-nodal", "bottom")
     TILES = ("TileSmall", "TileBig", "TileSmall-pull", "TileMid-pull")
 
-    def info(self):
+    def info(self, schedule=False):
         cc, nl, lb, kind, npyr, nres, pull1 = (C.c_int() for _ in range(7))
         lds, t = C.c_long(), (C.c_int * 31)()
         check(_lib.lib().hps_mg_info(self._h, C.byref(cc), C.byref(nl), C.byref(lb), C.byref(kind), C.byref(lds), t,
                                      C.byref(pull1), C.byref(npyr), C.byref(nres)))
-        return {"cc": bool(cc.value), "nlev": nl.value, "lowv_begin": lb.value, "lowv": self.LOWV[kind.value],
-                "lowv_lds": lds.value, "tiles": tuple(self.TILES[v] for v in t if v >= 0), "nodal_pull1": bool(pull1.value),
-                "pyramid": npyr.value, "restricts": nres.value}
+        out = {"cc": bool(cc.value), "nlev": nl.value, "lowv_begin": lb.value, "lowv": self.LOWV[kind.value],
+               "lowv_lds": lds.value, "tiles": tuple(self.TILES[v] for v in t if v >= 0), "nodal_pull1": bool(pull1.value),
+               "pyramid": npyr.value, "restricts": nres.value}
+        if schedule:
+            guest = C.c_int()
+            check(_lib.lib().hps_mg_info_schedule(self._h, C.byref(guest)))
+            out["coef_guest"] = bool(guest.value)
+        return out
 
     def solve1(self, fields, sol_comp, rhs_comp, acoef_comp, tol_rel=1e-4, tol_abs=2.2250738585072014e-308,
                nummaxiter=200):
@@ -1231,6 +1236,16 @@
         check(_lib.lib().hps_engine_early_init_slices(self._h, C.byref(ei)))
         return dict(vcycles=vc.value, slices=sl.value, early_init=ei.value)
 
+    def schedule(self):
+        g, v = C.c_int(), C.c_int()
+        check(_lib.lib().hps_engine_schedule(self._h, C.byref(g), C.byref(v)))
+        return dict(mg_coef_guest=bool(g.value), valid_by_psi=bool(v.value))
+
+    def qsa_drops(self):
+        n = C.c_long()
+        check(_lib.lib().hps_engine_qsa_drops(self._h, C.byref(n)))
+        return n.value
+
     def slab(self):
         self.sync()
         s = _lib.lib().hps_engine_slab(self._h)
diff --git a/hipace_amd/csrc/engine.h b/hipace_amd/csrc/engine.h
--- a/hipace_amd/csrc/engine.h
+++ b/hipace_amd/csrc/engine.h
@@ -152,6 +152,7 @@
     TailWork fold_tail_of (const Species& s, long margin, long* covered) const;
     int species_deposit (const Species& s, const int comp[6], const BeamPairWork* beam = nullptr, const int* go = nullptr);
     bool valid_by_w = true;
+    bool valid_by_psi = true;
     bool post_in_push = true;
     bool fold_hierarchy = true;
     bool fold_beam = true;
diff --git a/hipace_amd/csrc/engine.hip b/hipace_amd/csrc/engine.hip
--- a/hipace_amd/csrc/engine.hip
+++ b/hipace_amd/csrc/engine.hip
@@ -658,6 +658,7 @@
     if (const char* v = std::getenv("HPS_FOLD_BEAM")) fold_beam = std::atoi(v) != 0;
     if (const char* v = std::getenv("HPS_FOLD_HIERARCHY")) fold_hierarchy = std::atoi(v) != 0;
     if (const char* v = std::getenv("HPS_VALID_BY_W")) valid_by_w = std::atoi(v) != 0;
+    if (const char* v = std::getenv("HPS_VALID_BY_PSI")) valid_by_psi = std::atoi(v) != 0;
     if (const char* v = std::getenv("HPS_GATED_ION_PUSH")) gate_ion_push = std::atoi(v) != 0;
     if (const char* v = std::getenv("HPS_LAZY_SHIFT")) lazy_shift = std::atoi(v) != 0;
     if (const char* v = std::getenv("HPS_FUSE_SOURCES")) fuse_sources = std::atoi(v) != 0;
@@ -777,8 +778,7 @@
 {
     if (tile_size == 0 || el.cap == 0 || el.tiling) return HPS_OK;
     if (int e = tiling_create(d.nx, d.ny, tile_size, el.cap, &el.tiling)) return e;
-    {   const char* v = std::getenv("HPS_VALID_BY_PSI");
-        el.tiling->valid_by_psi = (v && std::atoi(v) != 0); }
+    el.tiling->valid_by_psi = valid_by_psi;
     if (int e = alloc_soa(el.pl_alt, el.real_alt, el.cap, el.alias_prev())) return e;
     if (ions.present()) {
         int ion_ts = tile_size;
@@ -2079,6 +2079,24 @@
     *n = static_cast<Engine*>(h)->slices_rode;
     return HPS_OK;
 }
+extern "C" int hps_engine_schedule (void* h, int* mg_coef_guest, int* valid_by_psi)
+{
+    HPS_REQUIRE(h, "hps_engine_schedule: null handle");
+    Engine* E = static_cast<Engine*>(h);
+    if (mg_coef_guest) { *mg_coef_guest = 0; if (E->mg) { if (int e = hps_mg_info_schedule(E->mg, mg_coef_guest)) return e; } }
+    if (valid_by_psi) *valid_by_psi = (E->tile_size != 0 && E->valid_by_psi) ? 1 : 0;
+    return HPS_OK;
+}
+extern "C" int hps_engine_qsa_drops (void* h, long* n)
+{
+    HPS_REQUIRE(h && n, "hps_engine_qsa_drops: null argument");
+    Engine* E = static_cast<Engine*>(h);
+    int v = 0;
+    HPS_HIP_CHECK(hipStreamSynchronize(E->st));
+    HPS_HIP_CHECK(hipMemcpy(&v, E->d_nqsa, sizeof(int), hipMemcpyDeviceToHost));
+    *n = v;
+    return HPS_OK;
+}
 extern "C" hps_plasma hps_engine_plasma (void* h) { return static_cast<Engine*>(h)->el.pl; }
 extern "C" int hps_engine_tiling (void* h, void** tiling)
 {
diff --git a/hipace_amd/csrc/multigrid.hip b/hipace_amd/csrc/multigrid.hip
--- a/hipace_amd/csrc/multigrid.hip
+++ b/hipace_amd/csrc/multigrid.hip
@@ -47,6 +47,7 @@
 template <bool CC> struct HugeTileOf { using type = TileHuge; };
 template <> struct HugeTileOf<false> { using type = TileHugeNodal; };
 using TileSmall = TileShape<32, 16, 256>;
+constexpr int COEF_GUEST_MAX_IMG = 2*(34*34 + 18*18 + 10*10 + 6*6 + 4*4);
 
 template <bool CC>
 __device__ __forceinline__ double diag_c0 (int i, int j, const LevBox& b, double acf, double facx, double facy)
@@ -423,23 +424,33 @@
     MG_STAMP(5);
 }
 
-template <class TS, bool CC, int SRC, bool DO_RES, bool FUSE_R, int NSW = 4, bool RPULL = false>
+struct CoefGuest;
+__device__ void coef_guest_derive (double* s_img, const CoefGuest& g, int nt);
+
+template <class TS, bool CC, int SRC, bool DO_RES, bool FUSE_R, int NSW = 4, bool RPULL = false, class... GUEST>
 __global__ __launch_bounds__(TS::NT, (RPULL && TS::GPAIRS > 1) ? 2 : 4)
 void k_smooth (LevBox b, FView phi_out, FView phi_out2, FView rhs, FView acf, FView phi_in, FView crse, FView res_out,
                FView cres_out, double facx, double facy, int ntx, unsigned long long* resnorm,
-               unsigned long long* rhsnorm, StopRule sr)
+               unsigned long long* rhsnorm, StopRule sr, GUEST... guest)
 {
     static_assert(!FUSE_R || (CC && DO_RES), "fused restriction is cell-centred only");
+    constexpr int HOST = (int)sizeof...(GUEST);
+    static_assert(HOST <= 1 && (HOST == 0 || (CC && NSW == 4)), "the guest rides in the cell-centred initial pass");
     if (NSW != 4 && !vcycle_active(sr)) return;
     constexpr int GT_X = TS::TX, GT_Y = TS::TY;
     __shared__ double s_phi[2][TS::AY*TS::AX];
     __shared__ double s_red[TS::NT/64];
+    if constexpr (HOST > 0) {
+        static_assert(2*TS::AY*TS::AX >= COEF_GUEST_MAX_IMG, "the image is staged in the tile's static LDS");
+        if (blockIdx.x == 0) { coef_guest_derive(&s_phi[0][0], guest..., TS::NT); return; }
+    }
     constexpr bool PLDS = !CC && SRC == SRC_PROLONG;
     __shared__ double s_crs[PLDS ? 2*(TS::AX/2 + 2)*(TS::AY/2 + 2) : 1];
     constexpr int E = DO_RES ? NSW : NSW - 1;
     constexpr int FX = GT_X - 2*E, FY = GT_Y - 2*E;
-    const int nb = gridDim.x, q8 = nb >> 3, r8 = nb & 7, xcd = blockIdx.x & 7;
-    const int tile = xcd*q8 + min(xcd, r8) + (blockIdx.x >> 3);
+    const unsigned wg = blockIdx.x - HOST;
+    const int nb = gridDim.x - HOST, q8 = nb >> 3, r8 = nb & 7, xcd = wg & 7;
+    const int tile = xcd*q8 + min(xcd, r8) + (wg >> 3);
     const int bx = tile % ntx, by = tile / ntx;
     const int gi0 = b.vlx + bx*FX - E;
     const int gj0 = b.vly + by*FY - E;
@@ -949,10 +960,60 @@
     for (long s = (long)guest*1024 + threadIdx.x; s < a.plane; s += (long)nguests*1024) shift_init_cell(a, s);
 }
 
+struct CoefGuest { const Low2* low; const double* acfA; double* img; double facx0, facy0; };
+
+__device__ void coef_guest_derive (double* s_img, const CoefGuest& g, int nt)
+{
+    lds_double* img = (lds_double*)s_img;
+    const Low2& d = *g.low;
+    const int t = threadIdx.x;
+    const int nl = d.nl, ctot = d.ctot, cbase = d.cbase;
+    for (int q = t; q < ctot; q += nt) img[q] = 0.0;
+    __syncthreads();
+    if (nl > 1) {
+        const int nxA = d.nx[0], nyA = d.ny[0], nbx = (nxA + 1) >> 1, nby = (nyA + 1) >> 1, p1 = d.nx[1] + 2;
+        for (int q = t; q < nbx*nby; q += nt) {
+            const int bj = q / nbx, i = 2*(q - bj*nbx), j = 2*bj;
+            double a[4];
+#pragma unroll
+            for (int k = 0; k < 4; ++k) {
+                const int ik = i + (k & 1), jk = j + (k >> 1);
+                const double v = g.acfA[min(ik, nxA - 1) + min(jk, nyA - 1)*nxA];
+                a[k] = (ik < nxA && jk < nyA) ? v : 0.0;
+            }
+            img[d.coff[1] - cbase + ((j >> 1) + 1)*p1 + (i >> 1) + 1] = 0.25*(a[0] + a[1] + a[2] + a[3]);
+        }
+    }
+    __syncthreads();
+    for (int l = 1; l < nl; ++l) {
+        const double fx = lvl_fac(g.facx0, l), fy = lvl_fac(g.facy0, l);
+        const int nx = d.nx[l], ny = d.ny[l], nbx = (nx + 1) >> 1, nby = (ny + 1) >> 1, pitch = nx + 2, ps = pitch*(ny + 2);
+        lds_double* lev = img + (d.coff[l] - cbase);
+        const int ok[4] = {0, 1, pitch, pitch + 1};
+        for (int q = t; q < nbx*nby; q += nt) {
+            const int bj = q / nbx, i = 2*(q - bj*nbx), j = 2*bj;
+            lds_double* acf = lev + (j + 1)*pitch + i + 1;
+            const bool in[4] = {true, i + 1 < nx, j + 1 < ny, i + 1 < nx && j + 1 < ny};
+            double a[4];
+#pragma unroll
+            for (int k = 0; k < 4; ++k) a[k] = in[k] ? acf[ok[k]] : 0.0;
+            if (l + 1 < nl) {
+                const int pn = d.nx[l+1] + 2;
+                img[d.coff[l+1] - cbase + ((j >> 1) + 1)*pn + (i >> 1) + 1] = 0.25*(a[0] + a[1] + a[2] + a[3]);
+            }
+#pragma unroll
+            for (int k = 0; k < 4; ++k)
+                if (in[k]) acf[ps + ok[k]] = 1.0/diag_c0<true>(i + (k & 1), j + (k >> 1), cc_box(nx, ny), a[k], fx, fy);
+        }
+        __syncthreads();
+    }
+    for (int q = t; q < ctot; q += nt) g.img[q] = img[q];
+}
+
 __global__ __launch_bounds__(1024)
 void k_lower_v3 (const Low2* __restrict__ dp, const double* __restrict__ acf_g, const double* __restrict__ cinv_g,
                  const double* __restrict__ res_g, double* __restrict__ cor_g, double* __restrict__ coef_g, int nxA, int nyA, int ctot,
-                 double facx0, double facy0, int nsweeps_bottom, StopRule sr, ShiftInit guest)
+                 double facx0, double facy0, int nsweeps_bottom, StopRule sr, ShiftInit guest, int derive_first)
 {
     if (blockIdx.x >= 2) { lower_v_guest(guest, (int)blockIdx.x - 2, (int)gridDim.x - 2); return; }
     extern __shared__ __attribute__((aligned(16))) double lds_raw[];
@@ -974,7 +1035,7 @@
         rA[k] = A.ok[k] ? v0 : 0.0; aA[k] = A.ok[k] ? v2 : 0.0; A.ci[k] = A.ok[k] ? v3 : 0.0;
         A.r0[k] = rA[k];
     }
-    const bool derive = (sr.k <= 0);
+    const bool derive = derive_first && (sr.k <= 0);
     constexpr int NIMG = 4;
     double img[NIMG];
 #pragma unroll
@@ -1280,6 +1341,7 @@
     bool ride_on = false; ShiftInit ride{}; int ride_guests = 0;
     double* cinvA = nullptr;
     double* coef_img = nullptr;
+    bool coef_guest = false;
     double* tmp0 = nullptr;
     bool cor_in_tmp = false;
     FView sol, rhs, acf0;
@@ -1380,6 +1442,8 @@
             HPS_HIP_CHECK(hipGetDevice(&dev));
             HPS_HIP_CHECK(hipDeviceGetAttribute(&ncu, hipDeviceAttributeMultiprocessorCount, dev));
             M->ride_guests = std::max(ncu - 2, 1);
+            const char* sw = getenv("HPS_MG_COEF_GUEST");
+            M->coef_guest = !(sw && atoi(sw) == 0) && M->L[0].cells > SMALL_TILE_CELLS && e.nl > 1 && e.ctot <= COEF_GUEST_MAX_IMG;
             break;
         }
     }
@@ -1493,7 +1557,8 @@
             const int guests = (k == 0 && M->ride_on) ? M->ride_guests : 0;
             M->ride_on = false;
             hipLaunchKernelGGL(k_lower_v3, dim3(2 + guests), dim3(1024), M->low3_lds, st, M->d_low3, M->L[lb].acf, M->cinvA, M->L[lb].res, M->L[lb].cor,
-                               M->coef_img, M->low3.nx[0], M->low3.ny[0], M->low3.ctot, 1.0/(ldx*ldx), 1.0/(ldy*ldy), nsweeps, sr, M->ride);
+                               M->coef_img, M->low3.nx[0], M->low3.ny[0], M->low3.ctot, 1.0/(ldx*ldx), 1.0/(ldy*ldy), nsweeps, sr, M->ride,
+                               M->coef_guest ? 0 : 1);
         } else
             hipLaunchKernelGGL(k_lower_v<CC>, dim3(CC ? 1 : 2), dim3(1024), M->low_lds, st, M->d_low, nl - lb, M->L[lb].acf, M->L[lb].res,
                                M->L[lb].cor, 1.0/(ldx*ldx), 1.0/(ldy*ldy), nsweeps, sr, M->pulls(lb) ? M->lv(lb-1, M->L[lb-1].rescor) : FView{});
@@ -1611,6 +1676,20 @@
     return HPS_OK;
 }
 
+static void launch_initial_with_guest (Multigrid* M, const StopRule& sr, hipStream_t st)
+{
+    using TS = TileBig;
+    const LevBox& b = M->L[0].b;
+    constexpr int FX = TS::TX - 2*4, FY = TS::TY - 2*4;
+    const int ntx = ceil_div(b.vhx - b.vlx + 1, FX), nty = ceil_div(b.vhy - b.vly + 1, FY);
+    const int lb = M->lowv_begin;
+    const double lfac = (double)(1 << lb), ldx = M->dx*lfac, ldy = M->dy*lfac;
+    const CoefGuest g{M->d_low3, M->L[lb].acf, M->coef_img, 1.0/(ldx*ldx), 1.0/(ldy*ldy)};
+    hipLaunchKernelGGL((k_smooth<TS, true, SRC_DIRECT, true, true, 4, false, CoefGuest>), dim3(ntx*nty + 1), dim3(TS::NT), 0, st, b,
+                       M->lv(0, M->L[0].cor), FView{}, M->rhs, M->acf0, M->sol, FView{}, M->lv(0, M->L[0].rescor), M->lv(1, M->L[1].res),
+                       1.0/(M->dx*M->dx), 1.0/(M->dy*M->dy), ntx, M->d_norms, M->d_norms + MG_NSUB, sr, g);
+}
+
 template <bool CC>
 static int solve1_begin (Multigrid* M, double tol_rel, double tol_abs, int max_iters, hipStream_t st)
 {
@@ -1621,6 +1700,9 @@
     int nzeroed = std::min(max_iters, nspec + 8);
     if (M->hierarchy_ready) M->hierarchy_ready = false;
     else if (int e = solve1_hierarchy<CC>(M, max_iters, st)) return e;
+    if (CC && M->coef_guest)
+        launch_initial_with_guest(M, always, st);
+    else
     launch_smooth<CC, SRC_DIRECT, true>(M, 0, M->lv(0, M->L[0].cor), FView{}, M->rhs, M->acf0, M->sol, FView{}, M->lv(0, M->L[0].rescor),
                                         M->lv(1, M->L[1].res), M->d_norms, M->d_norms + MG_NSUB, always, st);
     if (!M->nodal_pull1) restrict_residual_if_nodal<CC>(M, 0, always, st);
@@ -1812,6 +1894,13 @@
     return HPS_OK;
 }
 
+extern "C" int hps_mg_info_schedule (void* handle, int* coef_guest)
+{
+    HPS_REQUIRE(handle, "hps_mg_info_schedule: null handle");
+    if (coef_guest) *coef_guest = static_cast<const Multigrid*>(handle)->coef_guest ? 1 : 0;
+    return HPS_OK;
+}
+
 extern "C" int hps_mg_solve1 (void* handle, hps_slab slab, int sol_comp, int rhs_comp, int acoef_comp, double tol_rel,
                               double tol_abs, int max_iters, int* iters_host, double* resnorm_host, hps_stream stream)
 {
diff --git a/hipace_amd/csrc/particles_tiled.hip b/hipace_amd/csrc/particles_tiled.hip
--- a/hipace_amd/csrc/particles_tiled.hip
+++ b/hipace_amd/csrc/particles_tiled.hip
@@ -143,7 +143,7 @@
         Rec r;
         r.x = pl.x[ip]; r.y = pl.y[ip]; r.w = pl.w[ip];
         r.ux = pl.ux[ip]; r.uy = pl.uy[ip]; r.psi = pl.psi[ip];
-        if constexpr (VBW) r.id = (r.w != 0.0) ? HPS_ID_VALID : 0ULL;
+        if constexpr (VBW) r.id = 0ULL;
         else r.id = pl.idcpu[ip];
         r.ion = k.can_ionize ? pl.ion_lev[ip] : 1;
         return r;
@@ -175,7 +175,7 @@
         if (ip >= pend) break;
         const Rec cur = rec[u];
         const uint64_t id = cur.id;
-        if (!(id & HPS_ID_VALID)) continue;
+        if (VBW ? (cur.w == 0.0) : !(id & HPS_ID_VALID)) continue;
         const double psi_inv = 1.0/cur.psi;
         const double vx_c = cur.ux*psi_inv;
         const double vy_c = cur.uy*psi_inv;
diff --git a/include/hpslice.h b/include/hpslice.h
--- a/include/hpslice.h
+++ b/include/hpslice.h
@@ -124,6 +124,7 @@
 enum { HPS_MG_MAXLEV = 31 };
 int hps_mg_info (void* handle, int* cc, int* nlev, int* lowv_begin, int* lowv_kind, long* lowv_lds, int* tiles,
                  int* nodal_pull1, int* pyr_levels, int* pyr_restricts);
+int hps_mg_info_schedule (void* handle, int* coef_guest);
 int hps_mg_destroy (void* handle);
 
 int hps_mg2_create (int nx, int ny, double dx, double dy, void** handle);
@@ -201,6 +202,8 @@
 int hps_engine_checksums (void* handle, double* out_host);
 int hps_engine_stats (void* handle, long* total_vcycles, long* slices_done);
 int hps_engine_early_init_slices (void* handle, long* n_slices);
+int hps_engine_schedule (void* handle, int* mg_coef_guest, int* valid_by_psi);
+int hps_engine_qsa_drops (void* handle, long* n);
 int hps_engine_pc_stats (void* handle, long* iterations, double* error_sum);
 int hps_engine_pc_zero_b_slices (void* handle, long* slices);
 int hps_engine_laser_info (void* handle, int* aabs_comp, double* envelope_abs_sum_host);
```

New measurement: 1739, median of 6. 1.2% higher.
